# adamgreig/basebandboard

Hardware: AMD Instinct MI355X
Metric: awgn_clt_gsamples_per_s (higher is better)
Workload: dtype u32 bit-sliced GF(2) / int8 out

## Files before the change

### basebandboard_amd/_lib.py

```python
import ctypes as C
import pathlib

import torch

_HERE = pathlib.Path(__file__).resolve().parent
LIB_PATH = _HERE / "libbbb_hip.so"

SHARD_TRIALS, SHARD_SEEDS, SHARD_BITS, SHARD_GROUPS = 0, 1, 2, 3
BBB_OK, BBB_EINVAL, BBB_ENOMEM, BBB_EHIP, BBB_EIO, BBB_ENODEV, BBB_EUNSUP = 0, -1, -2, -3, -4, -5, -6

SYMBOLS = [
    "bbb_abi_version", "bbb_strerror", "bbb_last_error_detail", "bbb_device_count", "bbb_free",
    "bbb_lutopt_load_matrix_file", "bbb_lutopt_create", "bbb_lutopt_destroy", "bbb_lutopt_set_stream",
    "bbb_lutopt_is_specialised", "bbb_lutopt_set_staged", "bbb_lutopt_set_custom_fill", "bbb_lutopt_set_custom_ber", "bbb_lutopt_attach_custom_library", "bbb_lutopt_profile", "bbb_lutopt_profile_read", "bbb_lutopt_profile_read_mover", "bbb_lutopt_state_at", "bbb_lutopt_fill_words", "bbb_awgn_fill_i8", "bbb_awgn_fill_i16", "bbb_awgn_prefetch", "bbb_awgn_stream_open", "bbb_awgn_stream_next", "bbb_awgn_stream_read", "bbb_awgn_stream_seek", "bbb_awgn_stream_tell", "bbb_awgn_stream_close", "bbb_awgn_hist",
    "bbb_clt_tree_i16", "bbb_prbs_fill", "bbb_prbs_fill_hint", "bbb_prbs_check", "bbb_prbs_check_dev", "bbb_prbs_state_at",
    "bbb_prbs_detector_run", "bbb_prbs_detector_stream", "bbb_ber_trials", "bbb_ber_trials_dev", "bbb_ber_run_open", "bbb_ber_run_next", "bbb_ber_run_next_dev", "bbb_ber_run_tell", "bbb_ber_run_close", "bbb_ber_sweep_multi", "bbb_sweep_shard", "bbb_multi_last_info", "bbb_multi_release", "bbb_shaper_fill_i16", "bbb_tx_fill_i16", "bbb_tx_stream_open", "bbb_tx_stream_next", "bbb_tx_stream_read", "bbb_tx_stream_seek", "bbb_tx_stream_tell", "bbb_tx_stream_close", "bbb_rx_slice", "bbb_rx_phase_search", "bbb_eye_accumulate_i16", "bbb_tx_eye_open", "bbb_tx_eye_run", "bbb_tx_eye_close", "bbb_tx_ber_sweep_open", "bbb_tx_ber_sweep_run", "bbb_tx_ber_sweep_close", "bbb_acf_accumulate_i16", "bbb_tx_acf_open", "bbb_tx_acf_run", "bbb_tx_acf_close", "bbb_nco_rom", "bbb_nco_open", "bbb_nco_set_cfg", "bbb_nco_set_stream", "bbb_nco_run", "bbb_nco_get_state", "bbb_nco_set_state", "bbb_nco_close", "bbb_sinc_coefficients", "bbb_sinc_interpolate", "bbb_sinc_eye_open", "bbb_sinc_eye_run", "bbb_sinc_eye_close", "bbb_fir_moving_average", "bbb_fir_filter", "bbb_fir_slice", "bbb_link_sweep_open", "bbb_link_sweep_run", "bbb_link_sweep_close", "bbb_gf2_berlekamp_massey", "bbb_gf2_recur",
    "bbb_gf2_dot", "bbb_gf2_poly_is_primitive", "bbb_gf2_poly_modexp", "bbb_lutopt_charpoly", "bbb_lutopt_is_full_period",
    "bbb_lutopt_save_matrix_file", "bbb_lutopt_search_candidate", "bbb_lutopt_search",
    "bbb_errstat_open", "bbb_errstat_accumulate", "bbb_errstat_skip", "bbb_errstat_read", "bbb_errstat_reset",
    "bbb_errstat_set_stream", "bbb_errstat_geometry", "bbb_errstat_close",
    "bbb_xcorr_accumulate_i16", "bbb_tx_xcorr_open", "bbb_tx_xcorr_run", "bbb_tx_xcorr_close",
    "bbb_ddc_run", "bbb_ddc_polar_host",
    "bbb_dfe_run", "bbb_dfe_geometry", "bbb_dfe_model_host",
]


class BbbError(RuntimeError):
    def __init__(self, code, what, detail):
        super().__init__(f"{what}: {detail}" if detail else what)
        self.code = code


class TrialCfg(C.Structure):
    _fields_ = [("prbs_k", C.c_int32), ("amp", C.c_int32), ("noise_var", C.c_int32), ("reserved", C.c_int32),
                ("prbs_state", C.c_uint64), ("warmup", C.c_uint64), ("first_bit", C.c_uint64),
                ("nbits", C.c_uint64)]


class TxCfg(C.Structure):
    _fields_ = [("coeffs", C.c_int16 * 64), ("source", C.c_int32), ("prbs_k", C.c_int32), ("prbs_state", C.c_uint64),
                ("bit_en", C.c_int32), ("noise_en", C.c_int32), ("noise_var", C.c_int32), ("reserved", C.c_int32),
                ("warmup", C.c_uint64)]


class EyeCfg(C.Structure):
    _fields_ = [("ncols", C.c_uint32), ("shift", C.c_uint32), ("col_origin", C.c_uint64), ("threshold", C.c_int32),
                ("strict", C.c_int32)]


class TxSetting(C.Structure):
    _fields_ = [("coeffs", C.c_int16 * 64), ("bit_en", C.c_int32), ("noise_en", C.c_int32), ("noise_var", C.c_int32),
                ("threshold", C.c_int32), ("strict", C.c_int32), ("reserved", C.c_int32)]


class DetectorStats(C.Structure):
    _fields_ = [(n, C.c_uint64) for n in ("bits", "errors", "errors_raw", "reload_clocks", "resyncs", "chunks",
                                          "chunks_rerun", "serial_fallback")]


class SearchStats(C.Structure):
    _fields_ = [(n, C.c_uint64) for n in ("tested", "full_degree", "order_divides", "primitive", "kernel_ns")]


class MultiInfo(C.Structure):
    _fields_ = [("n_devices", C.c_int32), ("n_ranks_seen", C.c_int32), ("rccl_reused", C.c_int32), ("reserved", C.c_int32),
                ("rccl_path", C.c_char * 256)]


class NcoCfg(C.Structure):
    _fields_ = [("fcw", C.c_uint32), ("am", C.c_uint32), ("fm", C.c_int32), ("pm", C.c_int32)]


class NcoState(C.Structure):
    _fields_ = [("pa", C.c_uint32), ("q", C.c_int32), ("w", C.c_int32), ("y", C.c_int32)]


class SincCfg(C.Structure):
    _fields_ = [("in_bytes", C.c_uint32), ("out_bytes", C.c_uint32), ("shift", C.c_uint32)]


class FirCfg(C.Structure):
    _fields_ = [("ntaps", C.c_uint32), ("taps", C.c_int16 * 256), ("shift", C.c_uint32), ("decim", C.c_uint32),
                ("phase", C.c_uint32), ("out_bytes", C.c_uint32)]


DDC_IQ16, DDC_IQ32, DDC_POLAR = 0, 1, 2


class DfeCfg(C.Structure):
    _fields_ = [("ff", FirCfg), ("nfb", C.c_uint32), ("fb", C.c_int32 * 4), ("threshold", C.c_int32), ("strict", C.c_uint32),
                ("region_symbols", C.c_uint32), ("warmup_symbols", C.c_uint32)]


class DdcCfg(C.Structure):
    _fields_ = [("fcw", C.c_uint32), ("pa0", C.c_uint32), ("mode", C.c_uint32)]


ERRSTAT_NBINS = 312


class ErrstatCfg(C.Structure):
    _fields_ = [("guard", C.c_uint32), ("nblock", C.c_uint32), ("block_bits", C.c_uint64 * 4)]


class ErrstatResult(C.Structure):
    _fields_ = ([(n, C.c_uint64) for n in ("bits", "errors", "first_error", "last_error", "max_gap", "bursts", "burst_len_sum",
                                           "max_burst_len", "max_burst_weight", "open_first", "open_last", "open_weight")]
                + [("errored_blocks", C.c_uint64 * 4)]
                + [(n, C.c_uint64 * ERRSTAT_NBINS) for n in ("gap_hist", "burst_len_hist", "burst_weight_hist")])


class XcorrCfg(C.Structure):
    _fields_ = [("spb", C.c_uint32), ("nlags", C.c_uint32), ("origin", C.c_uint64)]


class Ber(C.Structure):
    _fields_ = [("bits", C.c_uint64), ("errors", C.c_uint64)]


_lib = None


def select_build(name):
    global LIB_PATH
    if _lib is not None:
        raise RuntimeError("the library is already loaded")
    LIB_PATH = _HERE / {"product": "libbbb_hip.so", "experiments": "libbbb_hip_exp.so"}[name]


def lib():
    global _lib
    if _lib is not None:
        return _lib
    if not LIB_PATH.exists():
        raise ImportError(
            f"{LIB_PATH} is missing: build it with `python -c 'import __graft_entry__ as g; g.build()'` "
            "(hipcc --offload-arch=gfx950).  basebandboard_amd has no CPU fallback.")
    l = C.CDLL(str(LIB_PATH))
    vp, u64, i32 = C.c_void_p, C.c_uint64, C.c_int
    u64p = C.POINTER(C.c_uint64)
    l.bbb_abi_version.restype = i32
    l.bbb_strerror.restype = C.c_char_p
    l.bbb_strerror.argtypes = [i32]
    l.bbb_last_error_detail.restype = C.c_char_p
    l.bbb_device_count.argtypes = [C.POINTER(i32)]
    l.bbb_free.argtypes = [vp]
    l.bbb_free.restype = None
    l.bbb_lutopt_load_matrix_file.argtypes = [C.c_char_p, C.POINTER(i32), C.POINTER(C.POINTER(C.c_uint16)),
                                              C.POINTER(C.POINTER(C.c_uint32))]
    l.bbb_lutopt_create.argtypes = [C.POINTER(vp), i32, C.POINTER(C.c_uint16), C.POINTER(C.c_uint32), u64p, i32]
    l.bbb_lutopt_destroy.argtypes = [vp]
    l.bbb_lutopt_set_stream.argtypes = [vp, vp]
    l.bbb_lutopt_is_specialised.argtypes = [vp]
    l.bbb_lutopt_set_staged.argtypes = [vp, i32]
    l.bbb_lutopt_state_at.argtypes = [vp, u64, u64p]
    l.bbb_lutopt_profile.argtypes = [vp, i32]
    l.bbb_lutopt_profile_read.argtypes = [vp, C.POINTER(C.c_double), C.POINTER(C.c_double), u64p, i32]
    l.bbb_lutopt_profile_read_mover.argtypes = [vp, C.POINTER(C.c_double), u64p, i32]
    l.bbb_lutopt_fill_words.argtypes = [vp, vp, u64, u64, i32]
    l.bbb_awgn_fill_i8.argtypes = [vp, vp, u64, u64]
    l.bbb_awgn_fill_i16.argtypes = [vp, vp, u64, u64]
    l.bbb_awgn_prefetch.argtypes = [vp, u64, u64]
    l.bbb_awgn_stream_open.argtypes = [vp, u64, u64, i32, C.POINTER(vp)]
    l.bbb_awgn_stream_next.argtypes = [vp, vp]
    l.bbb_awgn_stream_read.argtypes = [vp, vp, u64]
    l.bbb_awgn_stream_seek.argtypes = [vp, u64]
    l.bbb_awgn_stream_tell.argtypes = [vp, u64p]
    l.bbb_awgn_stream_close.argtypes = [vp]
    l.bbb_awgn_hist.argtypes = [vp, vp, u64, u64]
    l.bbb_clt_tree_i16.argtypes = [i32, vp, u64, vp, i32, vp]
    l.bbb_prbs_fill.argtypes = [i32, u64, u64, u64, vp, i32, vp]
    l.bbb_prbs_fill_hint.argtypes = [i32, u64, u64, u64, vp, C.c_uint, i32, vp]
    l.bbb_prbs_check.argtypes = [i32, u64, u64, u64, vp, u64p, i32, vp]
    l.bbb_prbs_check_dev.argtypes = [i32, u64, u64, u64, vp, vp, i32, vp]
    l.bbb_prbs_state_at.argtypes = [i32, u64, u64, u64p]
    l.bbb_prbs_detector_run.argtypes = [i32, vp, u64, u64, vp, vp, i32, vp]
    l.bbb_rx_phase_search.argtypes = [vp, u64, u64, u64, i32, i32, C.POINTER(DetectorStats), i32, vp]
    l.bbb_prbs_detector_stream.argtypes = [i32, vp, u64, vp, vp, C.POINTER(DetectorStats), u64, u64, i32, vp]
    l.bbb_ber_trials.argtypes = [vp, C.POINTER(TrialCfg), i32, C.POINTER(Ber)]
    l.bbb_ber_trials_dev.argtypes = [vp, C.POINTER(TrialCfg), i32, vp]
    l.bbb_multi_last_info.argtypes = [C.POINTER(MultiInfo)]
    l.bbb_ber_run_open.argtypes = [vp, C.POINTER(TrialCfg), i32, C.c_uint32, C.POINTER(vp)]
    l.bbb_ber_run_next.argtypes = [vp, C.POINTER(Ber)]
    l.bbb_ber_run_next_dev.argtypes = [vp, vp]
    l.bbb_ber_run_tell.argtypes = [vp, u64p, u64p]
    l.bbb_ber_run_close.argtypes = [vp]
    l.bbb_ber_sweep_multi.argtypes = [C.POINTER(vp), i32, C.POINTER(TrialCfg), i32, i32, C.POINTER(Ber)]
    l.bbb_sweep_shard.argtypes = [C.POINTER(TrialCfg), i32, i32, i32, i32, C.POINTER(TrialCfg)]
    l.bbb_multi_release.argtypes = []
    l.bbb_shaper_fill_i16.argtypes = [C.POINTER(TxCfg), vp, u64, u64, i32, vp]
    l.bbb_tx_fill_i16.argtypes = [vp, C.POINTER(TxCfg), vp, u64, u64]
    l.bbb_tx_stream_open.argtypes = [vp, C.POINTER(TxCfg), u64, u64, C.POINTER(vp)]
    l.bbb_tx_stream_next.argtypes = [vp, vp]
    l.bbb_tx_stream_read.argtypes = [vp, vp, u64]
    l.bbb_tx_stream_seek.argtypes = [vp, u64]
    l.bbb_tx_stream_tell.argtypes = [vp, u64p]
    l.bbb_tx_stream_close.argtypes = [vp]
    l.bbb_rx_slice.argtypes = [vp, u64, u64, u64, i32, vp, u64p, i32, vp]
    l.bbb_eye_accumulate_i16.argtypes = [vp, u64, u64, C.POINTER(EyeCfg), vp, i32, vp]
    l.bbb_tx_eye_open.argtypes = [vp, C.POINTER(TxCfg), C.POINTER(EyeCfg), u64, C.POINTER(vp)]
    l.bbb_tx_eye_run.argtypes = [vp, u64, u64, vp, vp]
    l.bbb_tx_eye_close.argtypes = [vp]
    l.bbb_tx_ber_sweep_open.argtypes = [vp, C.POINTER(TxCfg), C.POINTER(TxSetting), i32, u64, C.POINTER(vp)]
    l.bbb_tx_ber_sweep_run.argtypes = [vp, u64, u64, vp]
    l.bbb_tx_ber_sweep_close.argtypes = [vp]
    l.bbb_acf_accumulate_i16.argtypes = [vp, u64, u64, C.c_uint32, vp, i32, vp]
    l.bbb_tx_acf_open.argtypes = [vp, C.POINTER(TxCfg), C.c_uint32, u64, C.POINTER(vp)]
    l.bbb_tx_acf_run.argtypes = [vp, u64, u64, vp]
    l.bbb_tx_acf_close.argtypes = [vp]
    l.bbb_nco_rom.argtypes = [vp]
    l.bbb_nco_open.argtypes = [C.POINTER(NcoCfg), i32, vp, C.POINTER(vp)]
    l.bbb_nco_set_cfg.argtypes = [vp, C.POINTER(NcoCfg)]
    l.bbb_nco_set_stream.argtypes = [vp, vp]
    l.bbb_nco_run.argtypes = [vp, vp, vp, vp, u64, vp]
    l.bbb_nco_get_state.argtypes = [vp, C.POINTER(NcoState)]
    l.bbb_nco_set_state.argtypes = [vp, C.POINTER(NcoState)]
    l.bbb_nco_close.argtypes = [vp]
    l.bbb_sinc_coefficients.argtypes = [vp]
    l.bbb_sinc_interpolate.argtypes = [vp, u64, C.c_uint32, C.POINTER(SincCfg), vp, i32, vp]
    l.bbb_sinc_eye_open.argtypes = [C.POINTER(SincCfg), C.POINTER(EyeCfg), u64, i32, vp, C.POINTER(vp)]
    l.bbb_sinc_eye_run.argtypes = [vp, vp, u64, C.c_uint32, u64, vp]
    l.bbb_sinc_eye_close.argtypes = [vp]
    l.bbb_fir_moving_average.argtypes = [C.POINTER(FirCfg), i32]
    l.bbb_fir_filter.argtypes = [vp, u64, C.c_uint32, C.POINTER(FirCfg), vp, u64p, i32, vp]
    l.bbb_fir_slice.argtypes = [vp, u64, C.c_uint32, C.POINTER(FirCfg), C.c_int32, i32, vp, u64p, i32, vp]
    l.bbb_link_sweep_open.argtypes = [vp, C.POINTER(TxCfg), C.POINTER(TxSetting), i32, C.POINTER(FirCfg), C.c_uint32,
                                      C.POINTER(EyeCfg), u64, C.POINTER(vp)]
    l.bbb_link_sweep_run.argtypes = [vp, u64, u64, vp, vp]
    l.bbb_link_sweep_close.argtypes = [vp]
    l.bbb_errstat_open.argtypes = [C.POINTER(ErrstatCfg), i32, vp, C.POINTER(vp)]
    l.bbb_errstat_accumulate.argtypes = [vp, vp, vp, u64]
    l.bbb_errstat_skip.argtypes = [vp, u64]
    l.bbb_errstat_read.argtypes = [vp, C.POINTER(ErrstatResult)]
    l.bbb_errstat_reset.argtypes = [vp]
    l.bbb_errstat_set_stream.argtypes = [vp, vp]
    l.bbb_errstat_geometry.argtypes = [u64p, u64p]
    l.bbb_errstat_close.argtypes = [vp]
    l.bbb_xcorr_accumulate_i16.argtypes = [vp, u64, u64, vp, u64, u64, C.POINTER(XcorrCfg), vp, i32, vp]
    l.bbb_tx_xcorr_open.argtypes = [vp, C.POINTER(TxCfg), C.c_uint32, u64, C.POINTER(vp)]
    l.bbb_tx_xcorr_run.argtypes = [vp, u64, u64, vp]
    l.bbb_tx_xcorr_close.argtypes = [vp]
    l.bbb_ddc_run.argtypes = [vp, u64, C.c_uint32, u64, C.POINTER(DdcCfg), C.POINTER(FirCfg), vp, u64p, i32, vp]
    l.bbb_ddc_polar_host.argtypes = [C.c_int16, C.c_int16, C.POINTER(C.c_uint16), C.POINTER(C.c_int16)]
    l.bbb_dfe_run.argtypes = [vp, u64, C.c_uint32, C.POINTER(DfeCfg), vp, vp, vp, vp, u64p, i32, vp]
    l.bbb_dfe_geometry.argtypes = [C.c_uint32, u64p, u64p, u64p, u64p, u64p]
    l.bbb_dfe_model_host.argtypes = [vp, u64, C.c_uint32, C.POINTER(DfeCfg), C.POINTER(C.c_uint32), vp, vp, u64p]
    u8p = C.POINTER(C.c_uint8)
    l.bbb_gf2_berlekamp_massey.argtypes = [u8p, u64, u8p, C.POINTER(C.c_int64)]
    l.bbb_gf2_recur.argtypes = [i32, i32, u64p, u8p, i32, u8p]
    l.bbb_lutopt_set_custom_fill.argtypes = [vp, vp]
    l.bbb_lutopt_set_custom_ber.argtypes = [vp, vp]
    l.bbb_lutopt_attach_custom_library.argtypes = [vp, C.c_char_p]
    l.bbb_gf2_dot.argtypes = [i32, i32, u64p, u8p, u8p]
    u16p, u32p = C.POINTER(C.c_uint16), C.POINTER(C.c_uint32)
    l.bbb_gf2_poly_is_primitive.argtypes = [u8p, i32, C.POINTER(C.c_int)]
    l.bbb_gf2_poly_modexp.argtypes = [u8p, i32, u64p, i32, u8p]
    l.bbb_lutopt_charpoly.argtypes = [i32, u16p, u32p, u8p, C.POINTER(C.c_int)]
    l.bbb_lutopt_is_full_period.argtypes = [i32, u16p, u32p, C.POINTER(C.c_int)]
    l.bbb_lutopt_save_matrix_file.argtypes = [C.c_char_p, i32, u16p, u32p]
    l.bbb_lutopt_search_candidate.argtypes = [i32, u64, u64, u16p, u32p]
    l.bbb_lutopt_search.argtypes = [i32, u64, u64, u64, u64p, u16p, u32p, C.POINTER(SearchStats), i32, vp]
    for name in SYMBOLS:
        getattr(l, name)
    _lib = l
    return l


def check(rc, what):
    if rc == BBB_OK:
        return
    l = lib()
    detail = l.bbb_last_error_detail().decode(errors="replace")
    name = l.bbb_strerror(rc).decode()
    if rc == BBB_EINVAL:
        raise ValueError(detail or name)
    raise BbbError(rc, f"{what} failed ({name})", detail)


def cuda_tensor(name, t, dtypes, kind, device):
    if not isinstance(t, torch.Tensor) or t.dtype not in dtypes or not t.is_cuda or t.dim() != 1 or not t.is_contiguous():
        raise ValueError(f"{name} must be a contiguous 1-D {kind} CUDA tensor")
    if t.device != torch.device("cuda", device):
        raise ValueError(f"{name} must be on cuda:{device}")
    return t


class Handle:
    _handle = _close = None

    def close(self):
        p = getattr(self, self._handle, None)
        setattr(self, self._handle, None)
        if p:
            check(getattr(lib(), self._close)(p), self._close)

    def __enter__(self):
        return self

    def __exit__(self, *exc):
        self.close()

    def __del__(self):
        try:
            self.close()
        except Exception:
            pass


class StreamHandle(Handle):
    _set_stream = None

    def _open_stream(self):
        self._stream = torch.cuda.current_stream(self.device).cuda_stream if torch.cuda.is_available() else None
        return C.c_void_p(self._stream)

    def _bind_stream(self):
        s = torch.cuda.current_stream(self.device).cuda_stream
        if s != self._stream:
            check(getattr(lib(), self._set_stream)(getattr(self, self._handle), C.c_void_p(s)), self._set_stream)
            self._stream = s
```

### basebandboard_amd/csrc/bbb_api.hip

```cpp
#include "bbb_common.hpp"
#include "dev_buf.hpp"
#include "capture.hpp"
#include "awgn_launch.hpp"
#include "stage_common.hpp"
#include "gf2.hpp"
#include "rccl_loader.hpp"
#include "sweep_shard.hpp"
#include "sweep_threads.hpp"

#include <algorithm>
#include <cstdlib>
#include <cstring>
#include <map>
#include <memory>
#include <mutex>
#include <thread>
#include <utility>
#include <vector>

namespace bbb {

std::string &last_error() {
    static thread_local std::string s;
    return s;
}

int use_device(int device) {
    static std::mutex mu;
    static bool checked[64] = {false};
    bool known = false;
    if (device >= 0 && device < 64) {
        std::lock_guard<std::mutex> g(mu);
        known = checked[device];
    }
    if (!known) {
        int n = 0;
        if (hipGetDeviceCount(&n) != hipSuccess || n <= 0) return fail(BBB_ENODEV, "no HIP device visible");
        if (device < 0 || device >= n) return fail(BBB_ENODEV, "device index out of range");
        hipDeviceProp_t p;
        BBB_HIP(hipGetDeviceProperties(&p, device));
        if (std::strncmp(p.gcnArchName, "gfx950", 6) != 0)
            return fail(BBB_ENODEV, std::string("device is ") + p.gcnArchName + ", this library is built for gfx950 only");
        if (device < 64) {
            std::lock_guard<std::mutex> g(mu);
            checked[device] = true;
        }
    }
    BBB_HIP(hipSetDevice(device));
    return BBB_OK;
}

namespace {

struct Event {
    hipEvent_t e = nullptr;
    Event() = default;
    Event(Event &&o) noexcept : e(o.e) { o.e = nullptr; }
    Event &operator=(Event &&o) noexcept { std::swap(e, o.e); return *this; }
    ~Event() { if (e) (void)hipEventDestroy(e); }
    operator hipEvent_t() const { return e; }
    int create_timed() { BBB_HIP(hipEventCreate(&e)); return BBB_OK; }
    int record(hipStream_t s) {
        if (!e) BBB_HIP(hipEventCreateWithFlags(&e, hipEventDisableTiming));
        BBB_HIP(hipEventRecord(e, s));
        return BBB_OK;
    }
};

template <size_t N>
struct ReadGuarded {
    DevBuf<uint32_t> buf[N];
    Event last_read;
    bool read_pending = false;
    bool fits(const size_t (&need)[N]) const {
        for (size_t i = 0; i < N; i++)
            if (buf[i].cap < need[i]) return false;
        return true;
    }
    int grow(const size_t (&need)[N]) {
        if (fits(need)) return BBB_OK;
        if (read_pending) BBB_HIP(hipEventSynchronize(last_read));
        read_pending = false;
        for (size_t i = 0; i < N; i++)
            if (const int rc = buf[i].grow(need[i])) return rc;
        return BBB_OK;
    }
    int wait_read(hipStream_t s) const {
        if (read_pending) BBB_HIP(hipStreamWaitEvent(s, last_read, 0));
        return BBB_OK;
    }
    int mark_read(hipStream_t s) {
        if (const int rc = last_read.record(s)) return rc;
        read_pending = true;
        return BBB_OK;
    }
};
enum { kStates = 0, kPlanes = 1 };

struct StageSlot {
    DevBuf<uint32_t> stage;
    Event arith;
    Event free;
    bool busy = false;
    uint64_t gen = 0;
    DevBuf<uint32_t> bits[2];
    unsigned bits_turn = 0;

    int grow_stage(size_t words) {
        if (stage.cap >= words) return BBB_OK;
        if (busy) BBB_HIP(hipEventSynchronize(free));
        busy = false;
        return stage.grow(words);
    }
    int grow_bits(unsigned b, size_t words) {
        if (bits[b].cap >= words) return BBB_OK;
        if (busy) BBB_HIP(hipEventSynchronize(free));
        return bits[b].grow(words);
    }
    int wait_free(hipStream_t s) const { if (busy) BBB_HIP(hipStreamWaitEvent(s, free, 0)); return BBB_OK; }
    int mover_queued(hipStream_t ms) {
        if (const int rc = free.record(ms)) return rc;
        busy = true;
        gen++;
        return BBB_OK;
    }
};

struct SeededStates {
    bool valid = false;
    uint64_t first = 0, L = 0, G = 0;
    ReadGuarded<2> set;
    Event seeded;
    bool matches(uint64_t f, uint64_t l, uint64_t g) const { return valid && first == f && L == l && G == g; }
};

struct ProfEv {
    Event e0, e1, e2;
    int begin(hipStream_t s) {
        for (Event *e : {&e0, &e1, &e2})
            if (const int rc = e->create_timed()) return rc;
        return e0.record(s);
    }
};

}

struct JumpPlan {
    GF2Mat B;
    GF2Mat Bt;
    DevBuf<uint32_t> d_cols;
    DevBuf<uint32_t> d_top;
    uint32_t qcol64[32] = {0};
    int levels = 0;
};

}

using namespace bbb;

struct bbb_lutopt {
    int k = 0, W64 = 0, W32 = 0, device = 0;
    bool specialised = false;
    bbb_custom_fill_fn custom_fill = nullptr;
    bbb_custom_ber_fn custom_ber = nullptr;
    int small_fast = 0;
    bool fast512 = false;
    hipStream_t stream = nullptr;
    std::vector<uint16_t> taps;
    std::vector<uint32_t> row_off;
    uint64_t init[8] = {0};
    std::unique_ptr<GF2Powers> pw;
    std::map<uint64_t, JumpPlan> plans;
    std::map<uint64_t, JumpPlan> prbs_plans;
    ReadGuarded<2> cur;
    ReadGuarded<1> pp[2];
    int pp_idx = 0;
    DevBuf<uint16_t> d_taps;
    DevBuf<uint32_t> d_row_off;
    DevBuf<unsigned long long> d_counters;
    DevBuf<uint32_t> d_txnoise;
    DevBuf<uint32_t> d_txbits;
    ReadGuarded<1> fbits[2];
    Event fbits_ready;
    SeededStates seeds[2];
    int seeds_idx = 0;
    DevBuf<unsigned long long, true> h_counters;
    Event counters_zeroed;
    bool counters_clean = false;
    int fbits_slot = 0;
    bool planes_valid = false;
    uint64_t planes_first = 0, planes_L = 0, planes_G = 0;
    unsigned max_waves = 1024;
    SeededStates pf;
    hipStream_t side = nullptr;
    hipStream_t cs = nullptr;
    bool cs_valid = false;
    Event handover;
    bool staged_mode = false;
    bool has_stream = false;
    hipStream_t xs2[2] = {nullptr, nullptr}, ys = nullptr;
    StageSlot slots[2];
    int stage_slot = 0;
    Event ev_user;
    int pf_waited_slot = -1;
    uint64_t pf_waited_gen = 0;
    struct Ahead {
        bool valid = false; int kind = 0; uint64_t first = 0, step = 0, n = 0, win_lo = 0, L = 0, G = 0;
        unsigned nlanes = 0, left = 0; int slot = 0; bbb_tx_cfg cfg{};
        int64_t bits_m0 = 0; uint64_t bits_words64 = 0;
        unsigned bits_buf = 0;
    } ahead;
    bool last_fill_tx = false;
    bool last_staged_small = false;
    int staged_level = 0;
    bool profiling = false;
    std::vector<std::pair<Event, Event>> prof_mover_pending;
    double prof_mover_ms = 0; uint64_t prof_mover_calls = 0;
    std::vector<ProfEv> prof_pending;
    Event prof_prev_e2;
    double prof_seed_ms = 0, prof_main_ms = 0;
    uint64_t prof_calls = 0;
};

extern "C" {
static int seed_announced(bbb_lutopt *h, uint64_t first_step, uint64_t L, uint64_t G, unsigned nlanes, hipStream_t side, int seed_variant);
}

namespace {

int pad_w32(int k) {
    const int w = (k + 31) / 32;
    for (int c : {1, 2, 4, 6, 8, 12, 16})
        if (w <= c) return c;
    return 16;
}

int upload(const std::vector<uint32_t> &host, DevBuf<uint32_t> *out) {
    DevBuf<uint32_t> d;
    if (const int rc = d.grow(host.size())) return rc;
    BBB_HIP(hipMemcpy(d.p, host.data(), host.size() * sizeof(uint32_t), hipMemcpyHostToDevice));
    *out = std::move(d);
    return BBB_OK;
}

void nibble_table(const GF2Mat &M, uint32_t *out) {
    const int k = M.n, W32 = pad_w32(k), nnib = (k + 3) / 4;
    const int C = (W32 % 4 == 0) ? 4 : (W32 % 2 == 0 ? 2 : 1), NC = W32 / C;
    std::vector<uint32_t> cols((size_t)k * W32, 0u);
    for (int r = 0; r < k; r++) {
        const uint64_t *row = M.row(r);
        for (int w = 0; w < M.W; w++) {
            uint64_t bits = row[w];
            while (bits) {
                const int c = (w << 6) + __builtin_ctzll(bits);
                bits &= bits - 1;
                cols[(size_t)c * W32 + (r >> 5)] |= 1u << (r & 31);
            }
        }
    }
    std::vector<uint32_t> ent(16 * (size_t)W32);
    for (int n = 0; n < nnib; n++) {
        std::fill(ent.begin(), ent.end(), 0u);
        for (int v = 1; v < 16; v++) {
            const int c = 4 * n + __builtin_ctz((unsigned)v);
            for (int z = 0; z < W32; z++)
                ent[(size_t)v * W32 + z] = ent[(size_t)(v & (v - 1)) * W32 + z] ^ (c < k ? cols[(size_t)c * W32 + z] : 0u);
        }
        for (int v = 0; v < 16; v++)
            for (int z = 0; z < W32; z++)
                out[(((size_t)n * NC + z / C) * 16 + v) * C + z % C] = ent[(size_t)v * W32 + z];
    }
}

int build_plan(const GF2Mat &M, int levels, JumpPlan *plan) {
    const int k = M.n, W32 = pad_w32(k), nnib = (k + 3) / 4;
    const size_t nt = (size_t)nnib * 16 * W32;
    std::vector<uint32_t> host((size_t)levels * 15 * nt, 0);
    GF2Mat m1 = M;
    for (int e = 1; e < levels; e++) {
        for (int q = 0; q < 4; q++) m1 = m1.mul(m1);
        GF2Mat mj = m1;
        for (int j = 1; j <= 15; j++) {
            if (j > 1) mj = mj.mul(m1);
            nibble_table(mj, &host[((size_t)e * 15 + (j - 1)) * nt]);
        }
    }
    if (const int rc = upload(host, &plan->d_cols)) return rc;
    plan->levels = levels;
    plan->B = M;
    plan->Bt = M.transpose();
    return BBB_OK;
}

void first16(const JumpPlan &plan, const uint64_t *s0, uint32_t *out) {
    const int W = plan.B.W;
    uint64_t x[8];
    std::memcpy(x, s0, sizeof(uint64_t) * (size_t)W);
    std::memset(out, 0, sizeof(uint32_t) * 256);
    for (int i = 0; i < 16; i++) {
        if (i) plan.Bt.matvec_t(x, x);
        for (int w = 0; w < 2 * W && w < 16; w++) out[i * 16 + w] = (uint32_t)(x[w >> 1] >> (32 * (w & 1)));
    }
}

void first16_at(const bbb_lutopt *h, const JumpPlan &plan, uint64_t step, uint32_t *out) {
    uint64_t s0[8] = {0};
    h->pw->apply(step, h->init, s0);
    first16(plan, s0, out);
}

constexpr int kPlanLevels = 7;

int ensure_top_tables(JumpPlan *plan) {
    if (plan->d_top) return BBB_OK;
    const GF2Mat &M = plan->B;
    const int k = M.n, W32 = pad_w32(k), nnib = (k + 3) / 4;
    const size_t nt = (size_t)nnib * 16 * W32;
    std::vector<uint32_t> host((size_t)kSeedTopTables * nt, 0);
    GF2Mat m4 = M;
    for (int q = 0; q < 16; q++) m4 = m4.mul(m4);
    GF2Mat md = m4;
    for (int d = 1; d <= kSeedTopTables; d++) {
        if (d > 1) md = md.mul(m4);
        nibble_table(md, &host[(size_t)(d - 1) * nt]);
    }
    return upload(host, &plan->d_top);
}

int get_plan(bbb_lutopt *h, uint64_t L, JumpPlan **out) {
    auto it = h->plans.find(L);
    if (it == h->plans.end()) {
        JumpPlan p;
        int rc = build_plan(h->pw->power(L), kPlanLevels, &p);
        if (rc) return rc;
        it = h->plans.emplace(L, std::move(p)).first;
    }
    *out = &it->second;
    return BBB_OK;
}

int get_prbs_plan(bbb_lutopt *h, int k, uint64_t L, JumpPlan **out) {
    const uint64_t key = ((uint64_t)k << 56) ^ L;
    auto it = h->prbs_plans.find(key);
    if (it == h->prbs_plans.end()) {
        JumpPlan p;
        GF2Powers pw(prbs_matrix(k, prbs_tap(k)));
        int rc = build_plan(pw.power(L), kPlanLevels, &p);
        if (rc) return rc;
        {
            GF2Mat q = p.B;
            for (int i = 0; i < 6; i++) q = q.mul(q);
            const GF2Mat qt = q.transpose();
            for (int c = 0; c < k && c < 32; c++) p.qcol64[c] = (uint32_t)qt.row(c)[0];
        }
        it = h->prbs_plans.emplace(key, std::move(p)).first;
    }
    *out = &it->second;
    return BBB_OK;
}

void partition(const bbb_lutopt *h, uint64_t n, unsigned granule, uint64_t *L, uint64_t *G, unsigned *nlanes) {
    const uint64_t gmax = (uint64_t)h->max_waves * 2048;
    uint64_t l = (n + gmax - 1) / gmax;
    if (l < 64) l = 64;
    l = (l + granule - 1) / granule * granule;
    const uint64_t g = (n + l - 1) / l;
    const uint64_t waves = (g + 2047) / 2048;
    *L = l;
    *G = g;
    *nlanes = (unsigned)(waves * 64);
}

struct DevStreams { hipStream_t xs[2] = {nullptr, nullptr}, side = nullptr; };
static std::mutex g_streams_mu;
static std::map<int, DevStreams> g_streams;

int ensure_internal_streams(bbb_lutopt *h) {
    if (!h->xs2[0]) {
        std::lock_guard<std::mutex> g(g_streams_mu);
        DevStreams &d = g_streams[h->device];
        for (hipStream_t *st : {&d.xs[0], &d.xs[1]})
            if (!*st) BBB_HIP(hipStreamCreateWithFlags(st, hipStreamNonBlocking));
        h->xs2[0] = d.xs[0]; h->xs2[1] = d.xs[1];
    }
    return BBB_OK;
}

int ensure_side_stream(bbb_lutopt *h) {
    if (!h->side) {
        std::lock_guard<std::mutex> g(g_streams_mu);
        DevStreams &d = g_streams[h->device];
        if (!d.side) BBB_HIP(hipStreamCreateWithFlags(&d.side, hipStreamNonBlocking));
        h->side = d.side;
    }
    return BBB_OK;
}

int begin_op(bbb_lutopt *h, bool internal, bool independent_of_previous_internal = false) {
    if (internal) {
        const int rc = ensure_internal_streams(h);
        if (rc) return rc;
    }
    hipStream_t want = internal ? h->xs2[h->stage_slot ^ 1] : h->stream;
    if (h->cs_valid && h->cs != want) {
        const bool from_internal = h->cs == h->xs2[0] || h->cs == h->xs2[1];
        if (!(independent_of_previous_internal && internal && from_internal)) {
            const int rc = h->handover.record(h->cs);
            if (rc) return rc;
            BBB_HIP(hipStreamWaitEvent(want, h->handover, 0));
        }
    }
    h->cs = want;
    h->cs_valid = true;
    return BBB_OK;
}

int mark_planes_read(bbb_lutopt *h) { return h->cur.mark_read(h->cs); }

int prepare_planes(bbb_lutopt *h, uint64_t first, uint64_t L, uint64_t G, unsigned nlanes, int slice_mode = 0) {
    if (h->planes_valid && h->planes_first == first && h->planes_L == L && h->planes_G == G) return BBB_OK;
    JumpPlan *plan;
    int rc = get_plan(h, L, &plan);
    if (rc) return rc;
    const bool two_launch = h->k == 256 && (h->specialised || h->custom_fill) && !h->fast512 && G <= ((uint64_t)kSeedTopTables + 1) * 65536 &&
                            !env_knob("BBB_EXP_SEED_CHAIN", 0);
    const size_t states_words = two_launch && (size_t)G * h->W32 < (size_t)65536 * 8 ? (size_t)65536 * 8 : (size_t)G * h->W32;
    if ((rc = h->cur.grow({states_words, (size_t)2 * h->k * nlanes}))) return rc;
    uint32_t s16[256];
    first16_at(h, *plan, first, s16);
    h->planes_valid = false;
    if (two_launch) {
        if ((rc = ensure_top_tables(plan))) return rc;
        if ((rc = awgn_seed_head_launch(h->k, plan->d_cols, s16, G, h->cur.buf[kStates], h->cs))) return rc;
        rc = awgn_seed_tail_planes_launch(h->k, plan->d_top, G, h->cur.buf[kStates], nlanes, h->cur.buf[kPlanes], h->cs);
    } else {
        rc = awgn_seed_launch(h->k, plan->d_cols, s16, G, h->cur.buf[kStates], G, nlanes, h->cur.buf[kPlanes], h->cs, slice_mode);
    }
    if (rc || slice_mode) return rc;
    if ((rc = mark_planes_read(h))) return rc;
    h->planes_valid = true;
    h->planes_first = first; h->planes_L = L; h->planes_G = G;
    return BBB_OK;
}

int acquire_planes(bbb_lutopt *h, uint64_t first_step, uint64_t L, uint64_t G, unsigned nlanes, bool may_use_prefetch,
                   bool *from_prefetch = nullptr, int slice_mode = 0) {
    if (from_prefetch) *from_prefetch = false;
    if (may_use_prefetch && h->pf.matches(first_step, L, G)) {
        if (from_prefetch) *from_prefetch = true;
        BBB_HIP(hipStreamWaitEvent(h->cs, h->pf.seeded, 0));
        std::swap(h->cur, h->pf.set);
        h->pf.valid = false;
        h->planes_valid = slice_mode == 0;
        h->planes_first = first_step; h->planes_L = L; h->planes_G = G;
        return BBB_OK;
    }
    return prepare_planes(h, first_step, L, G, nlanes, slice_mode);
}


template <typename LaunchMover>
int queue_mover_with(bbb_lutopt *h, int slot, LaunchMover launch_mover) {
    hipStream_t ms = h->stream;
    StageSlot &sl = h->slots[slot];
    int rc;
    const bool own_stream = env_knob("BBB_EXP_MOVER_OWN_STREAM", 0) != 0;
    if (own_stream) {
        if (!h->ys) BBB_HIP(hipStreamCreateWithFlags(&h->ys, hipStreamNonBlocking));
        ms = h->ys;
        if ((rc = h->ev_user.record(h->stream))) return rc;
        BBB_HIP(hipStreamWaitEvent(ms, h->ev_user, 0));
    }
    BBB_HIP(hipStreamWaitEvent(ms, sl.arith, 0));
    if ((rc = sl.wait_free(ms))) return rc;
    Event m0, m1;
    if (h->profiling) {
        if ((rc = m0.create_timed()) || (rc = m1.create_timed())) return rc;
        BBB_HIP(hipEventRecord(m0, ms));
    }
    if ((rc = launch_mover((const void *)sl.stage.p, ms))) return rc;
    if (h->profiling) {
        BBB_HIP(hipEventRecord(m1, ms));
        h->prof_mover_pending.emplace_back(std::move(m0), std::move(m1));
    }
    if ((rc = sl.mover_queued(ms))) return rc;
    if (own_stream) BBB_HIP(hipStreamWaitEvent(h->stream, sl.free, 0));
    return BBB_OK;
}

bool tx_cfg_equal(const bbb_tx_cfg &a, const bbb_tx_cfg &b) {
    return std::memcmp(a.coeffs, b.coeffs, sizeof a.coeffs) == 0 && a.source == b.source && a.prbs_k == b.prbs_k &&
           a.prbs_state == b.prbs_state && a.bit_en == b.bit_en && a.noise_en == b.noise_en && a.noise_var == b.noise_var &&
           a.warmup == b.warmup;
}

bbb_lutopt::Ahead take_ahead(bbb_lutopt *h) {
    const bbb_lutopt::Ahead a = h->ahead;
    h->ahead.first += a.n; h->ahead.step += a.n;
    h->ahead.win_lo += a.n;
    h->ahead.valid = --h->ahead.left > 0;
    return a;
}

int take_waiting(bbb_lutopt *h, int kind, uint64_t first, uint64_t n, const bbb_tx_cfg *cfg, bool *waiting, bbb_lutopt::Ahead *a) {
    *waiting = h->ahead.valid && h->ahead.kind == kind && h->ahead.first == first && h->ahead.n == n &&
               (kind != 1 || tx_cfg_equal(h->ahead.cfg, *cfg));
    if (!*waiting) return BBB_OK;
    if (env_knob("BBB_EXP_DELIVER_HANDOVER", 0)) {
        const int rc = begin_op(h, true);
        if (rc) return rc;
    }
    *a = take_ahead(h);
    return BBB_OK;
}

uint64_t ahead_total(const bbb_lutopt *h, uint64_t n, uint64_t cap, uint64_t step, uint64_t first, uint64_t pos_bound) {
    const uint64_t m = (uint64_t)h->staged_level;
    const bool ahead = m >= 2 && (n % 16) == 0 && m * n < cap && step + m * n >= m * n && (!pos_bound || first + m * n < pos_bound);
    return ahead ? m * n : n;
}

int produce_planes(bbb_lutopt *h, uint64_t L, unsigned nlanes, ProfEv *ev, bool planes_seeded_after_mover, int *slot_out,
                   bool small_footprint = false) {
    const int slot = h->stage_slot ^= 1;
    StageSlot &sl = h->slots[slot];
    *slot_out = slot;
    if (h->ahead.valid && h->ahead.slot == slot) h->ahead.valid = false;
    int rc;
    if ((rc = sl.grow_stage(stage_words(nlanes, L)))) return rc;
    const bool seeding_saw_last_mover = planes_seeded_after_mover && h->pf_waited_slot == slot && h->pf_waited_gen == sl.gen;
    if (planes_seeded_after_mover) h->pf_waited_slot = -1;
    if (!seeding_saw_last_mover && (rc = sl.wait_free(h->cs))) return rc;
    if (ev) BBB_HIP(hipEventRecord(ev->e1, h->cs));
    rc = awgn256_planes_launch(h->cur.buf[kPlanes], (void *)sl.stage.p, (unsigned)L, nlanes, h->cs, small_footprint);
    h->last_staged_small = small_footprint;
    if (rc) return rc;
    if ((rc = mark_planes_read(h))) return rc;
    if (ev) BBB_HIP(hipEventRecord(ev->e2, h->cs));
    return sl.arith.record(h->cs);
}

struct StagedRun { uint64_t L = 0, G = 0; unsigned nlanes = 0; int slot = 0; };

template <typename Hook, typename LaunchMover>
int staged_produce(bbb_lutopt *h, uint64_t ntotal, uint64_t seed_step, bool small_form, bool timed, Hook hook, LaunchMover launch_mover,
                   StagedRun *run) {
    StagedRun &r = *run;
    uint64_t &L = r.L, &G = r.G;
    partition(h, ntotal, 16, &L, &G, &r.nlanes);
    if (L > 0xffffff00ull) return fail(BBB_EINVAL, "nsamples too large for one call (segment length must fit 32 bits): split it");
    int rc = begin_op(h, true, h->pf.matches(seed_step, L, G));
    if (rc) return rc;
    h->last_fill_tx = false;
    ProfEv ev;
    const bool prof = timed && h->profiling;
    if (prof && (rc = ev.begin(h->cs))) return rc;
    bool from_pf = false;
    if ((rc = acquire_planes(h, seed_step, L, G, r.nlanes, true, &from_pf))) return rc;
    if ((rc = hook())) return rc;
    rc = produce_planes(h, L, r.nlanes, prof ? &ev : nullptr, from_pf, &r.slot, small_form);
    if (!rc) rc = queue_mover_with(h, r.slot, [&](const void *stage, hipStream_t ms) { return launch_mover(r, stage, ms); });
    if (prof) h->prof_pending.push_back(std::move(ev));
    return rc;
}

void record_ahead(bbb_lutopt *h, int kind, uint64_t first, uint64_t step, uint64_t n, uint64_t left, const StagedRun &run) {
    bbb_lutopt::Ahead &a = h->ahead;
    a.valid = true; a.kind = kind;
    a.first = first; a.step = step; a.n = n; a.win_lo = n; a.left = (unsigned)left;
    a.L = run.L; a.G = run.G; a.nlanes = run.nlanes; a.slot = run.slot;
}

bool partition512(const bbb_lutopt *h, uint64_t nsamples, uint64_t *L, uint64_t *G, unsigned *nlanes) {
    const uint64_t gmax = (uint64_t)h->max_waves * 1024;
    uint64_t l = (nsamples + gmax - 1) / gmax;
    if (l < 64) l = 64;
    l = (l + 7) / 8 * 8;
    if (l > 0xffffff00ull) return false;
    *L = l;
    *G = (nsamples + l - 1) / l;
    *nlanes = (unsigned)((*G + 1023) / 1024 * 64);
    return true;
}

int awgn_fill(bbb_lutopt *h, void *dst, int elem_size, uint64_t nsamples, uint64_t first_step) {
    if (!h) return fail(BBB_EINVAL, "null handle");
    if (nsamples == 0) return BBB_OK;
    if (!dst || ((uintptr_t)dst & 15)) return fail(BBB_EINVAL, "dst must be a 16-byte aligned device pointer");
    if (first_step + nsamples < first_step) return fail(BBB_EINVAL, "first_step + nsamples overflows");
    if (h->k & (h->k - 1)) return fail(BBB_EUNSUP, "CLTGRNG needs k to be a power of two (rng.py:72-76)");
    if (elem_size == 1 && h->k > 256) return fail(BBB_EUNSUP, "k > 256 needs the int16 output");
    if (h->device < 0) return fail(BBB_ENODEV, "host-only handle (device -1) cannot generate samples");
    BBB_HIP(hipSetDevice(h->device));
    uint64_t L, G;
    unsigned nlanes;
    if (h->fast512 && elem_size == 2) {
        if (!partition512(h, nsamples, &L, &G, &nlanes))
            return fail(BBB_EINVAL, "nsamples too large for one call (segment length must fit 32 bits): split it");
        int rc5 = begin_op(h, false);
        if (rc5) return rc5;
        h->planes_valid = false;
        if ((rc5 = acquire_planes(h, first_step, L, G, nlanes, true, nullptr, 1))) return rc5;
        if ((rc5 = awgn512p_fill_launch(h->cur.buf[kPlanes], (int16_t *)dst, nsamples, (unsigned)L, G, nlanes, h->cs))) return rc5;
        return mark_planes_read(h);
    }
    partition(h, nsamples, 16, &L, &G, &nlanes);
    if (L > 0xffffff00ull) return fail(BBB_EINVAL, "nsamples too large for one call (segment length must fit 32 bits): split it");
    const bool fast256 = h->specialised && elem_size == 1;
    h->last_fill_tx = false;
    const bool staged = fast256 && h->staged_mode && nsamples >= (1ull << 24);
    if (staged) {
        bool waiting;
        bbb_lutopt::Ahead a;
        int rc = take_waiting(h, 0, first_step, nsamples, nullptr, &waiting, &a);
        if (rc) return rc;
        auto launch_i8 = [&](const void *stage, uint64_t win_lo, uint64_t Lk, uint64_t Gk, unsigned nl, hipStream_t ms) {
            return unplane_launch(stage, dst, win_lo, nsamples, (unsigned)Lk, Gk, nl, ms);
        };
        if (waiting)
            return queue_mover_with(h, a.slot, [&](const void *stage, hipStream_t ms) { return launch_i8(stage, a.win_lo, a.L, a.G, a.nlanes, ms); });
        const uint64_t ntotal = ahead_total(h, nsamples, 1ull << 40, first_step, first_step, 0);
        const bool small_form = h->staged_level == 1 || env_knob("BBB_EXP_NOISE_SMALL", 0);
        StagedRun run;
        rc = staged_produce(h, ntotal, first_step + (small_form ? 1 : 0), small_form, true, [] { return BBB_OK; },
                            [&](const StagedRun &r, const void *stage, hipStream_t ms) { return launch_i8(stage, 0, r.L, r.G, r.nlanes, ms); }, &run);
        if (!rc && ntotal != nsamples) record_ahead(h, 0, first_step + nsamples, first_step + nsamples, nsamples, ntotal / nsamples - 1, run);
        return rc;
    }
    int rc = begin_op(h, false);
    if (rc) return rc;
    ProfEv ev;
    if (h->profiling && (rc = ev.begin(h->cs))) return rc;
    rc = acquire_planes(h, first_step, L, G, nlanes, fast256);
    if (rc) return rc;
    if (fast256) {
        if (h->profiling) BBB_HIP(hipEventRecord(ev.e1, h->cs));
        rc = awgn256_fill_launch(h->cur.buf[kPlanes], (int8_t *)dst, nsamples, (unsigned)L, G, nlanes, h->cs);
        if (!rc) rc = mark_planes_read(h);
        if (h->profiling) {
            BBB_HIP(hipEventRecord(ev.e2, h->cs));
            h->prof_pending.push_back(std::move(ev));
        }
        return rc;
    }
    if (h->custom_fill && elem_size == 1) {
        const int e = h->custom_fill(h->cur.buf[kPlanes], (int8_t *)dst, nsamples, (uint32_t)L, G, nlanes, (void *)h->cs);
        if (e) return fail(BBB_EHIP, std::string("custom sample kernel: ") + hipGetErrorString((hipError_t)e));
        return mark_planes_read(h);
    }
    if (h->small_fast && elem_size == 1) {
        rc = awgn_small_fill_launch(h->small_fast, h->cur.buf[kPlanes], (int8_t *)dst, nsamples, (unsigned)L, G, nlanes, h->cs);
        return rc ? rc : mark_planes_read(h);
    }
    h->planes_valid = false;
    rc = awgn_generic_fill_launch(h->k, h->d_taps, h->d_row_off, h->cur.buf[kPlanes], dst, elem_size, nsamples, (unsigned)L, G,
                                  nlanes, h->cs);
    return rc ? rc : mark_planes_read(h);
}

int wrap12(int v) {
    unsigned u = (unsigned)v & 0xfffu;
    return (u & 0x800u) ? (int)u - 4096 : (int)u;
}
int channel_thresholds(int amp, int noise_var, TrialDev *t) {
    for (int bv = 0; bv < 2; bv++) {
        int n = 0, prev = 0;
        for (int T = 0; T < 256; T++) {
            const int g = T - 128;
            const int noise = wrap12(g * noise_var);
            const int x = wrap12((bv ? amp : -amp) + noise);
            const int decided = x >= 0;
            const int err = decided != bv;
            if (err != prev) {
                if (n == 4) return fail(BBB_EUNSUP, "channel needs more than 4 decision thresholds");
                t->thr[bv][n++] = T;
                prev = err;
            }
        }
        t->nthr[bv] = n;
    }
    return BBB_OK;
}

int trial_dev(const bbb_trial_cfg &c, TrialDev *t) {
    const int tap = prbs_tap(c.prbs_k);
    if (!tap) return fail(BBB_EINVAL, "k=" + std::to_string(c.prbs_k) + " invalid for PRBS");
    if (c.prbs_state == 0 || (c.prbs_state >> c.prbs_k)) return fail(BBB_EINVAL, "PRBS state must be in [1, 2^k)");
    if (c.amp < 0 || c.amp > 2047 || c.noise_var < 0 || c.noise_var > 15) return fail(BBB_EINVAL, "amp must be 0..2047 and noise_var 0..15");
    t->prbs_k = c.prbs_k;
    t->prbs_tap = tap;
    return channel_thresholds(c.amp, c.noise_var, t);
}

bool single_threshold(const TrialDev &t) {
    for (int bv = 0; bv < 2; bv++) {
        int real = 0;
        for (int j = 0; j < t.nthr[bv]; j++) real += t.thr[bv][j] > 0 && t.thr[bv][j] < 256;
        if (real != 1) return false;
    }
    return true;
}

int ber_run(bbb_lutopt *h, const bbb_trial_cfg *cfgs, int ncfg, unsigned long long *counters_dev) {
    {
        const int rc0 = begin_op(h, false);
        if (rc0) return rc0;
    }
    if (!h->specialised && !h->custom_ber)
        return fail(BBB_EUNSUP, "BER trials need the shipped n256 matrix, or a k = 256 matrix with its own kernels attached "
                                "(bbb_lutopt_attach_custom_library / LUTOPT.specialise)");
    std::vector<TrialDev> td((size_t)ncfg);
    for (int i = 0; i < ncfg; i++) {
        const bbb_trial_cfg &c = cfgs[i];
        if (c.warmup + c.first_bit < c.warmup || c.warmup + c.first_bit + c.nbits < c.nbits)
            return fail(BBB_EINVAL, "warmup + first_bit + nbits overflows");
        const int rc = trial_dev(c, &td[(size_t)i]);
        if (rc) return rc;
    }
    for (int i = 0; i < ncfg;) {
        const bbb_trial_cfg &c = cfgs[i];
        int n = 1;
        while (single_threshold(td[(size_t)i]) && i + n < ncfg && n < BBB_BER_MAX_GROUP) {
            const bbb_trial_cfg &d = cfgs[i + n];
            if (d.prbs_k != c.prbs_k || d.prbs_state != c.prbs_state || d.warmup != c.warmup ||
                d.first_bit != c.first_bit || d.nbits != c.nbits || !single_threshold(td[(size_t)(i + n)]))
                break;
            n++;
        }
        if (c.nbits == 0) { i += n; continue; }
        uint64_t L, G;
        unsigned nlanes;
        partition(h, c.nbits, 2, &L, &G, &nlanes);
        if (L >= (1ull << 27)) return fail(BBB_EINVAL, "nbits too large for one trial (about 2^47): split it with first_bit");
        for (int j = 0; j < n; j++) { td[(size_t)(i + j)].L = (uint32_t)L; td[(size_t)(i + j)].G = G; td[(size_t)(i + j)].nbits = c.nbits; }
        int rc;
        if ((rc = ensure_internal_streams(h))) return rc;
        const uint64_t gen_first = c.warmup + c.first_bit + 1;
        JumpPlan *pp, *plan = nullptr;
        if ((rc = get_prbs_plan(h, c.prbs_k, L, &pp))) return rc;
        const int pb = h->pp_idx ^= 1;
        for (int b : {pb, pb ^ 1})
            if ((rc = h->pp[b].grow({(size_t)32 * nlanes}))) return rc;
        uint32_t ps16[256], s16[256];
        {
            uint64_t ps0 = 0;
            if ((rc = prbs_state_at_host(c.prbs_k, c.prbs_state, c.first_bit, &ps0))) return rc;
            uint64_t ps64[8] = {ps0};
            first16(*pp, ps64, ps16);
        }
        int sb = -1;
        for (int b : {0, 1})
            if (h->seeds[b].matches(gen_first, L, G)) sb = b;
        const bool seed_gen = sb < 0;
        if (seed_gen) {
            sb = h->seeds_idx ^= 1;
            const size_t need[2] = {(size_t)65536 * h->W32, (size_t)h->k * nlanes};
            for (int b : {sb, sb ^ 1}) {
                if (!h->seeds[b].set.fits(need)) h->seeds[b].valid = false;
                if ((rc = h->seeds[b].set.grow(need))) return rc;
            }
            if ((rc = get_plan(h, L, &plan))) return rc;
            if ((rc = ensure_top_tables(plan))) return rc;
            first16_at(h, *plan, gen_first, s16);
        }
        const bool busy = seed_gen && hipStreamQuery(h->cs) == hipErrorNotReady;
        hipStream_t ss = busy ? h->xs2[0] : h->cs;
        ReadGuarded<1> &prbs = h->pp[pb];
        if ((rc = prbs.wait_read(seed_gen ? ss : h->cs))) return rc;
        SeededStates &gs = h->seeds[sb];
        if (seed_gen) {
            gs.valid = false;
            if ((rc = gs.set.wait_read(ss))) return rc;
            const PrbsSeedRide ride{c.prbs_k, pp->d_cols, ps16, pp->qcol64, nlanes, prbs.buf[0]};
            if ((rc = awgn_seed_head_launch(h->k, plan->d_cols, s16, G, gs.set.buf[kStates], ss, &ride))) return rc;
            if ((rc = awgn_seed_tail_planes_launch(h->k, plan->d_top, G, gs.set.buf[kStates], nlanes, gs.set.buf[kPlanes], ss))) return rc;
            if ((rc = gs.seeded.record(ss))) return rc;
            if (busy) BBB_HIP(hipStreamWaitEvent(h->cs, gs.seeded, 0));
            gs.valid = true;
            gs.first = gen_first; gs.L = L; gs.G = G;
        } else {
            BBB_HIP(hipStreamWaitEvent(h->cs, gs.seeded, 0));
            if ((rc = prbs_seed_lanes_launch(c.prbs_k, pp->d_cols, ps16, pp->qcol64, G, nlanes, prbs.buf[0], h->cs))) return rc;
        }
        if (h->specialised) {
            if ((rc = ber256_launch(gs.set.buf[kPlanes], prbs.buf[0], &td[(size_t)i], n, nlanes, counters_dev + 2 * (size_t)i, h->cs))) return rc;
        } else {
            const int e = h->custom_ber(gs.set.buf[kPlanes], prbs.buf[0], &td[(size_t)i], n, nlanes, (uint64_t *)(counters_dev + 2 * (size_t)i), (void *)h->cs);
            if (e) return fail(e < 0 ? e : BBB_EHIP, "custom BER kernel failed");
        }
        if ((rc = prbs.mark_read(h->cs))) return rc;
        if ((rc = gs.set.mark_read(h->cs))) return rc;
        i += n;
    }
    return BBB_OK;
}

}

extern "C" {

int bbb_abi_version(void) { return BBB_ABI_VERSION; }

const char *bbb_strerror(int code) {
    switch (code) {
    case BBB_OK: return "ok";
    case BBB_EINVAL: return "invalid argument";
    case BBB_ENOMEM: return "out of memory";
    case BBB_EHIP: return "HIP runtime error";
    case BBB_EIO: return "matrix file unreadable or malformed";
    case BBB_ENODEV: return "no gfx950 device";
    case BBB_EUNSUP: return "unsupported request";
    default: return "unknown error";
    }
}

const char *bbb_last_error_detail(void) { return last_error().c_str(); }

int bbb_device_count(int *count) {
    if (!count) return fail(BBB_EINVAL, "null count");
    int n = 0;
    if (hipGetDeviceCount(&n) != hipSuccess) n = 0;
    *count = n;
    return BBB_OK;
}

void bbb_free(void *p) { std::free(p); }

int bbb_lutopt_load_matrix_file(const char *path, int *k, uint16_t **taps, uint32_t **row_off) {
    if (!path || !k || !taps || !row_off) return fail(BBB_EINVAL, "null argument");
    FILE *f = std::fopen(path, "r");
    if (!f) return fail(BBB_EIO, std::string("cannot open ") + path);
    std::vector<std::string> rows;
    char line[BBB_MAX_K + 16];
    while (std::fgets(line, sizeof line, f)) {
        std::string s(line);
        while (!s.empty() && (s.back() == '\n' || s.back() == '\r' || s.back() == ' ')) s.pop_back();
        if (!s.empty()) rows.push_back(s);
    }
    std::fclose(f);
    const int n = (int)rows.size();
    if (n == 0 || n > BBB_MAX_K) return fail(BBB_EIO, "matrix must have 1..512 rows");
    std::vector<uint16_t> t;
    std::vector<uint32_t> off(1, 0);
    for (int r = 0; r < n; r++) {
        if ((int)rows[r].size() != n) return fail(BBB_EIO, "matrix is not square");
        for (int c = 0; c < n; c++) {
            if (rows[r][c] == '1') t.push_back((uint16_t)c);
            else if (rows[r][c] != '0') return fail(BBB_EIO, "matrix holds a character other than 0/1");
        }
        off.push_back((uint32_t)t.size());
    }
    *taps = (uint16_t *)std::malloc(sizeof(uint16_t) * (t.empty() ? 1 : t.size()));
    *row_off = (uint32_t *)std::malloc(sizeof(uint32_t) * off.size());
    if (!*taps || !*row_off) return fail(BBB_ENOMEM, "malloc");
    std::memcpy(*taps, t.data(), sizeof(uint16_t) * t.size());
    std::memcpy(*row_off, off.data(), sizeof(uint32_t) * off.size());
    *k = n;
    return BBB_OK;
}

int bbb_lutopt_create(bbb_lutopt **out, int k, const uint16_t *taps, const uint32_t *row_off,
                      const uint64_t *init_words, int device) {
    if (!out || !taps || !row_off || !init_words) return fail(BBB_EINVAL, "null argument");
    if (k < 2 || k > BBB_MAX_K) return fail(BBB_EINVAL, "k must be in [2, 512]");
    GF2Mat A(k);
    for (int r = 0; r < k; r++) {
        const uint32_t n = row_off[r + 1] - row_off[r];
        if (row_off[r + 1] < row_off[r] || n < 1 || n > 8) return fail(BBB_EINVAL, "every row needs 1..8 taps");
        for (uint32_t j = row_off[r]; j < row_off[r + 1]; j++) {
            if (taps[j] >= k) return fail(BBB_EINVAL, "tap index out of range");
            if (A.get(r, taps[j])) return fail(BBB_EINVAL, "duplicate tap in a row");
            A.set(r, taps[j]);
        }
    }
    if (device != -1) {
        int rc = use_device(device);
        if (rc) return rc;
    }
    std::unique_ptr<bbb_lutopt> h(new bbb_lutopt);
    h->k = k;
    h->W64 = (k + 63) / 64;
    h->W32 = pad_w32(k);
    h->device = device;
    h->taps.assign(taps, taps + row_off[k]);
    h->row_off.assign(row_off, row_off + k + 1);
    for (int w = 0; w < h->W64; w++) {
        uint64_t v = init_words[w];
        if (w == h->W64 - 1 && (k & 63)) v &= (1ull << (k & 63)) - 1ull;
        h->init[w] = v;
    }
    h->pw.reset(new GF2Powers(A));
    h->specialised = awgn256_matches(k, taps, row_off);
    h->small_fast = awgn_small_matches(k, taps, row_off);
    h->fast512 = awgn512p_matches(k, taps, row_off);
    if (device == -1) {
        *out = h.release();
        return BBB_OK;
    }
    hipDeviceProp_t p;
    BBB_HIP(hipGetDeviceProperties(&p, device));
    h->max_waves = (unsigned)p.multiProcessorCount * 4;
    int rc = h->d_taps.grow(h->taps.size());
    if (rc || (rc = h->d_row_off.grow(h->row_off.size()))) return rc;
    BBB_HIP(hipMemcpy(h->d_taps.p, h->taps.data(), sizeof(uint16_t) * h->taps.size(), hipMemcpyHostToDevice));
    BBB_HIP(hipMemcpy(h->d_row_off.p, h->row_off.data(), sizeof(uint32_t) * h->row_off.size(), hipMemcpyHostToDevice));
    *out = h.release();
    return BBB_OK;
}

int bbb_lutopt_destroy(bbb_lutopt *h) {
    if (!h) return BBB_OK;
    if (h->device < 0) { delete h; return BBB_OK; }
    (void)hipSetDevice(h->device);
    (void)hipDeviceSynchronize();
    if (h->ys) (void)hipStreamDestroy(h->ys);
    for (int s : {1, 0}) h->slots[s].stage = {};
    for (int i : {kPlanes, kStates}) h->pf.set.buf[i] = {};
    for (int i : {kPlanes, kStates})
        for (int b : {1, 0}) h->seeds[b].set.buf[i] = {};
    delete h;
    return BBB_OK;
}

int bbb_lutopt_set_stream(bbb_lutopt *h, void *hip_stream) {
    if (!h) return fail(BBB_EINVAL, "null handle");
    h->stream = (hipStream_t)hip_stream;
    return BBB_OK;
}

int bbb_lutopt_set_custom_fill(bbb_lutopt *h, bbb_custom_fill_fn fn) {
    if (!h) return fail(BBB_EINVAL, "null handle");
    if (fn && (h->k > 256 || (h->k & (h->k - 1)))) return fail(BBB_EUNSUP, "custom kernels exist for power-of-two k <= 256");
    h->custom_fill = fn;
    h->planes_valid = false;
    return BBB_OK;
}

int bbb_lutopt_set_custom_ber(bbb_lutopt *h, bbb_custom_ber_fn fn) {
    if (!h) return fail(BBB_EINVAL, "null handle");
    if (fn && h->k != 256) return fail(BBB_EUNSUP, "the fused BER kernels exist for k = 256");
    h->custom_ber = fn;
    return BBB_OK;
}

int bbb_lutopt_attach_custom_library(bbb_lutopt *h, const char *path) {
    if (!h || !path) return fail(BBB_EINVAL, "null argument");
    void *lib = dlopen(path, RTLD_NOW | RTLD_LOCAL);
    if (!lib) return fail(BBB_EIO, std::string("cannot load ") + path + ": " + dlerror());
    auto bail = [&](int code, const std::string &what) { dlclose(lib); return fail(code, what); };
    auto order = reinterpret_cast<int (*)(void)>(dlsym(lib, "bbb_custom_order"));
    auto abi = reinterpret_cast<int (*)(void)>(dlsym(lib, "bbb_custom_abi"));
    auto fill = reinterpret_cast<bbb_custom_fill_fn>(dlsym(lib, "bbb_custom_fill"));
    if (!order || !fill) return bail(BBB_EIO, std::string(path) + " does not export bbb_custom_order / bbb_custom_fill");
    if (!abi || abi() != BBB_CUSTOM_ABI)
        return bail(BBB_EINVAL, std::string(path) + " was built for another version of this library (custom ABI " +
                                    (abi ? std::to_string(abi()) : std::string("none")) + ", expected " + std::to_string(BBB_CUSTOM_ABI) + "): rebuild it");
    if (order() != h->k) return bail(BBB_EINVAL, std::string(path) + " was built for another order");
    int rc = bbb_lutopt_set_custom_fill(h, fill);
    if (rc) { dlclose(lib); return rc; }
    auto ber = reinterpret_cast<bbb_custom_ber_fn>(dlsym(lib, "bbb_custom_ber"));
    if (ber && h->k == 256) rc = bbb_lutopt_set_custom_ber(h, ber);
    return rc;
}

int bbb_lutopt_set_staged(bbb_lutopt *h, int enable) {
    if (!h) return fail(BBB_EINVAL, "null handle");
    if (enable < 0 || enable > 8) return fail(BBB_EINVAL, "0 = off, 1 = staged, 2..8 = staged with that many fills per sample kernel");
    h->staged_mode = enable != 0;
    h->staged_level = enable;
    h->ahead.valid = false;
    return BBB_OK;
}

int bbb_lutopt_is_specialised(const bbb_lutopt *h) { return h && h->specialised ? 1 : 0; }

int bbb_lutopt_profile(bbb_lutopt *h, int enable) {
    if (!h) return fail(BBB_EINVAL, "null handle");
    h->profiling = enable != 0;
    return BBB_OK;
}

int bbb_lutopt_profile_read(bbb_lutopt *h, double *seed_ms, double *kernel_ms, uint64_t *calls, int reset) {
    if (!h) return fail(BBB_EINVAL, "null handle");
    std::vector<ProfEv> pending;
    pending.swap(h->prof_pending);
    for (ProfEv &ev : pending) {
        BBB_HIP(hipEventSynchronize(ev.e2));
        float a = 0, b = 0;
        BBB_HIP(hipEventElapsedTime(&a, ev.e0, ev.e1));
        BBB_HIP(hipEventElapsedTime(&b, ev.e1, ev.e2));
        if (h->prof_prev_e2) {
            float c = 0;
            BBB_HIP(hipEventElapsedTime(&c, h->prof_prev_e2, ev.e2));
            if (c > 0 && c < b) b = c;
        }
        h->prof_prev_e2 = std::move(ev.e2);
        h->prof_seed_ms += a; h->prof_main_ms += b; h->prof_calls++;
    }
    if (seed_ms) *seed_ms = h->prof_seed_ms;
    if (kernel_ms) *kernel_ms = h->prof_main_ms;
    if (calls) *calls = h->prof_calls;
    if (reset) { h->prof_seed_ms = h->prof_main_ms = 0; h->prof_calls = 0; }
    return BBB_OK;
}

int bbb_lutopt_profile_read_mover(bbb_lutopt *h, double *mover_ms, uint64_t *calls, int reset) {
    if (!h) return fail(BBB_EINVAL, "null handle");
    std::vector<std::pair<Event, Event>> pending;
    pending.swap(h->prof_mover_pending);
    for (const auto &ev : pending) {
        BBB_HIP(hipEventSynchronize(ev.second));
        float a = 0;
        BBB_HIP(hipEventElapsedTime(&a, ev.first, ev.second));
        h->prof_mover_ms += a; h->prof_mover_calls++;
    }
    if (mover_ms) *mover_ms = h->prof_mover_ms;
    if (calls) *calls = h->prof_mover_calls;
    if (reset) { h->prof_mover_ms = 0; h->prof_mover_calls = 0; }
    return BBB_OK;
}

int bbb_lutopt_state_at(bbb_lutopt *h, uint64_t nsteps, uint64_t *state_words) {
    if (!h || !state_words) return fail(BBB_EINVAL, "null argument");
    h->pw->apply(nsteps, h->init, state_words);
    return BBB_OK;
}

static int seed_announced(bbb_lutopt *h, uint64_t first_step, uint64_t L, uint64_t G, unsigned nlanes, hipStream_t side, int seed_variant) {
    JumpPlan *plan;
    int rc = get_plan(h, L, &plan);
    if (rc) return rc;
    SeededStates &pf = h->pf;
    pf.valid = false;
    if (pf.seeded) BBB_HIP(hipStreamWaitEvent(side, pf.seeded, 0));
    if ((rc = pf.set.wait_read(side))) return rc;
    if ((rc = pf.set.grow({(size_t)G * h->W32, (size_t)2 * h->k * nlanes}))) return rc;
    pf.set.read_pending = false;
    uint32_t s16[256];
    first16_at(h, *plan, first_step, s16);
    if ((rc = awgn_seed_launch(h->k, plan->d_cols, s16, G, pf.set.buf[kStates], G, nlanes, pf.set.buf[kPlanes], side, h->fast512 ? 1 : 0, seed_variant))) return rc;
    if ((rc = pf.seeded.record(side))) return rc;
    pf.valid = true;
    pf.first = first_step; pf.L = L; pf.G = G;
    return BBB_OK;
}

static int awgn_prefetch(bbb_lutopt *h, uint64_t nsamples, uint64_t first_step, bool for_tx);

int bbb_awgn_prefetch(bbb_lutopt *h, uint64_t nsamples, uint64_t first_step) {
    return awgn_prefetch(h, nsamples, first_step, h && (h->staged_level == 1 || h->last_staged_small || env_knob("BBB_EXP_NOISE_SMALL", 0)));
}

static int awgn_prefetch(bbb_lutopt *h, uint64_t nsamples, uint64_t first_step, bool for_tx) {
    if (!h) return fail(BBB_EINVAL, "null handle");
    if (h->device < 0) return fail(BBB_ENODEV, "host-only handle (device -1)");
    if ((!h->specialised && !h->fast512) || nsamples == 0) return BBB_OK;
    BBB_HIP(hipSetDevice(h->device));
    uint64_t L, G;
    unsigned nlanes;
    const bool staged_size = nsamples >= (1ull << 24);
    if (h->staged_level >= 2 && nsamples >= (1ull << 24) && (nsamples % 16) == 0) {
        const uint64_t m = (uint64_t)h->staged_level;
        if (h->ahead.valid && h->ahead.step == first_step && h->ahead.n == nsamples) {
            const uint64_t skip = (uint64_t)h->ahead.left * nsamples;
            if (first_step + skip < first_step) return BBB_OK;
            first_step += skip;
        }
        if (m * nsamples < (1ull << 40) && first_step + m * nsamples > first_step) nsamples *= m;
    }
    if (for_tx && h->staged_mode && h->specialised && staged_size) {
        if (first_step + 1 == 0) return BBB_OK;
        first_step += 1;
    }
    if (h->fast512) {
        if (!partition512(h, nsamples, &L, &G, &nlanes)) return BBB_OK;
    } else {
        partition(h, nsamples, 16, &L, &G, &nlanes);
    }
    if (L > 0xffffff00ull) return BBB_OK;
    if (h->pf.matches(first_step, L, G)) return BBB_OK;
    hipStream_t side = nullptr;
    int rc;
    if (h->staged_mode && h->specialised) {
        if ((rc = ensure_internal_streams(h))) return rc;
        side = h->xs2[h->stage_slot ^ 1];
    } else {
        if ((rc = ensure_side_stream(h))) return rc;
        side = h->side;
    }
    h->pf_waited_slot = -1;
    h->pf.valid = false;
    const StageSlot &next = h->slots[h->stage_slot ^ 1];
    if (h->staged_mode && next.busy && !h->last_staged_small) {
        if ((rc = next.wait_free(side))) return rc;
        h->pf_waited_slot = h->stage_slot ^ 1;
        h->pf_waited_gen = next.gen;
    }
    return seed_announced(h, first_step, L, G, nlanes, side, h->last_fill_tx ? 4 : 2);
}

int bbb_awgn_fill_i8(bbb_lutopt *h, int8_t *dst_dev, uint64_t nsamples, uint64_t first_step) {
    return awgn_fill(h, dst_dev, 1, nsamples, first_step);
}

int bbb_awgn_fill_i16(bbb_lutopt *h, int16_t *dst_dev, uint64_t nsamples, uint64_t first_step) {
    if (h && h->specialised && h->device >= 0 && nsamples && dst_dev && !((uintptr_t)dst_dev & 15) && (nsamples % 16) == 0) {
        BBB_HIP(hipSetDevice(h->device));
        int rc = h->d_txnoise.grow((size_t)(nsamples + 15) / 4 + 4);
        if (rc) return rc;
        if ((rc = awgn_fill(h, h->d_txnoise, 1, nsamples, first_step))) return rc;
        return widen_i8_i16_launch((const int8_t *)h->d_txnoise.p, dst_dev, nsamples, h->stream);
    }
    return awgn_fill(h, dst_dev, 2, nsamples, first_step);
}


struct SeqStream {
    bbb_lutopt *h = nullptr;
    uint64_t n = 0, pos = 0;
    int saved_level = 0;
    virtual ~SeqStream() = default;
    virtual int fill(void *dst_dev, uint64_t nsamples) = 0;
    virtual int hint() = 0;
    static int overflows(const char *what) { return fail(BBB_EINVAL, std::string(what) + " + nsamples_per_call overflows"); }

    int open(bbb_lutopt *handle, uint64_t nsamples_per_call, uint64_t first, const char *what, bool level2) {
        if (handle->has_stream) return fail(BBB_EINVAL, "the handle already has an open stream");
        if (first + nsamples_per_call < first) return overflows(what);
        h = handle; n = nsamples_per_call; pos = first;
        saved_level = h->staged_level;
        int rc;
        if (h->staged_level == 0 && level2 && (rc = bbb_lutopt_set_staged(h, 2))) return rc;
        if ((rc = hint())) return rc;
        h->has_stream = true;
        return BBB_OK;
    }
    int read(void *dst_dev, uint64_t nsamples) {
        if (pos + nsamples < pos) return fail(BBB_EINVAL, "the stream position overflows");
        const int rc = fill(dst_dev, nsamples);
        if (rc) return rc;
        pos += nsamples;
        return hint();
    }
    int seek(uint64_t first, const char *what) {
        if (first + n < first) return overflows(what);
        pos = first;
        h->ahead.valid = false;
        return hint();
    }
};

static int seq_read(SeqStream *s, void *dst_dev, uint64_t nsamples) { return s && s->h ? s->read(dst_dev, nsamples) : fail(BBB_EINVAL, "null stream"); }
static int seq_next(SeqStream *s, void *dst_dev) { return s ? seq_read(s, dst_dev, s->n) : fail(BBB_EINVAL, "null stream"); }
static int seq_seek(SeqStream *s, uint64_t first, const char *what) { return s && s->h ? s->seek(first, what) : fail(BBB_EINVAL, "null stream"); }
static int seq_tell(const SeqStream *s, uint64_t *next) {
    if (!s || !next) return fail(BBB_EINVAL, "null argument");
    *next = s->pos;
    return BBB_OK;
}
static int seq_close(SeqStream *s) {
    if (!s) return BBB_OK;
    int rc = BBB_OK;
    if (s->h) {
        s->h->has_stream = false;
        if (s->h->staged_level != s->saved_level) rc = bbb_lutopt_set_staged(s->h, s->saved_level);
    }
    delete s;
    return rc;
}

struct bbb_awgn_stream : SeqStream {
    int elem = 1;
    int fill(void *dst_dev, uint64_t nsamples) override {
        return elem == 1 ? bbb_awgn_fill_i8(h, (int8_t *)dst_dev, nsamples, pos) : bbb_awgn_fill_i16(h, (int16_t *)dst_dev, nsamples, pos);
    }
    int hint() override { return pos + n >= pos ? bbb_awgn_prefetch(h, n, pos) : BBB_OK; }
};

int bbb_awgn_stream_open(bbb_lutopt *h, uint64_t nsamples_per_call, uint64_t first_step, int elem_bytes, bbb_awgn_stream **out) {
    if (!h || !out) return fail(BBB_EINVAL, "null argument");
    if (nsamples_per_call == 0) return fail(BBB_EINVAL, "nsamples_per_call must be positive");
    if (elem_bytes != 1 && elem_bytes != 2) return fail(BBB_EINVAL, "elem_bytes must be 1 (int8) or 2 (int16)");
    if (h->device < 0) return fail(BBB_ENODEV, "host-only handle (device -1) cannot generate samples");
    if (h->k & (h->k - 1)) return fail(BBB_EUNSUP, "CLTGRNG needs k to be a power of two (rng.py:72-76)");
    if (elem_bytes == 1 && h->k > 256) return fail(BBB_EUNSUP, "k > 256 needs the int16 output");
    std::unique_ptr<bbb_awgn_stream> s(new bbb_awgn_stream);
    s->elem = elem_bytes;
    const int rc = s->open(h, nsamples_per_call, first_step, "first_step", true);
    if (!rc) *out = s.release();
    return rc;
}

int bbb_awgn_stream_read(bbb_awgn_stream *s, void *dst_dev, uint64_t nsamples) { return seq_read(s, dst_dev, nsamples); }
int bbb_awgn_stream_next(bbb_awgn_stream *s, void *dst_dev) { return seq_next(s, dst_dev); }
int bbb_awgn_stream_seek(bbb_awgn_stream *s, uint64_t first_step) { return seq_seek(s, first_step, "first_step"); }
int bbb_awgn_stream_tell(const bbb_awgn_stream *s, uint64_t *next_step) { return seq_tell(s, next_step); }
int bbb_awgn_stream_close(bbb_awgn_stream *s) { return seq_close(s); }

int bbb_lutopt_fill_words(bbb_lutopt *h, uint32_t *dst_dev, uint64_t nstates, uint64_t first_step, int msb_first) {
    if (!h) return fail(BBB_EINVAL, "null handle");
    if (h->k % 32) return fail(BBB_EUNSUP, "the word stream is defined for k a multiple of 32 (util/verify.py:41,50)");
    if (nstates == 0) return BBB_OK;
    if (!dst_dev || ((uintptr_t)dst_dev & 3)) return fail(BBB_EINVAL, "dst must be a 4-byte aligned device pointer");
    if (first_step + nstates < first_step) return fail(BBB_EINVAL, "first_step + nstates overflows");
    if (nstates > (1ull << 48)) return fail(BBB_EINVAL, "nstates must be <= 2^48 per call");
    if (h->device < 0) return fail(BBB_ENODEV, "host-only handle (device -1) cannot generate words");
    BBB_HIP(hipSetDevice(h->device));
    uint64_t L, G;
    unsigned nlanes;
    const bool fast = h->specialised && !((uintptr_t)dst_dev & 7);
    partition(h, nstates, fast ? 2 : 1, &L, &G, &nlanes);
    int rc = begin_op(h, false);
    if (rc) return rc;
    rc = prepare_planes(h, first_step, L, G, nlanes);
    if (rc) return rc;
    if (fast) {
        rc = lutopt_words256_launch(h->cur.buf[kPlanes], dst_dev, nstates, (unsigned)L, G, nlanes, msb_first != 0, h->cs);
        return rc ? rc : mark_planes_read(h);
    }
    h->planes_valid = false;
    rc = lutopt_words_launch(h->k, h->d_taps, h->d_row_off, h->cur.buf[kPlanes], dst_dev, nstates, (unsigned)L, G, nlanes,
                             msb_first != 0, h->cs);
    if (!rc) rc = mark_planes_read(h);
    return rc;
}

int bbb_clt_tree_i16(int k, const uint64_t *states_dev, uint64_t nstates, int16_t *out_dev, int device,
                     void *hip_stream) {
    if (k < 2 || k > BBB_MAX_K || (k & (k - 1)) || (k & 63)) return fail(BBB_EINVAL, "k must be 64, 128, 256 or 512");
    if (nstates && (!states_dev || !out_dev)) return fail(BBB_EINVAL, "null device pointer");
    int rc = use_device(device);
    if (rc) return rc;
    return clt_tree_launch(k, states_dev, nstates, out_dev, (hipStream_t)hip_stream);
}

int bbb_prbs_fill(int k, uint64_t init_state, uint64_t first_bit, uint64_t nbits, uint64_t *dst_packed_dev,
                  int device, void *hip_stream) {
    if (nbits && !dst_packed_dev) return fail(BBB_EINVAL, "null device pointer");
    if (!prbs_tap(k)) return fail(BBB_EINVAL, "k=" + std::to_string(k) + " invalid for PRBS");
    int rc = use_device(device);
    if (rc) return rc;
    return prbs_fill_launch(k, init_state, first_bit, nbits, dst_packed_dev, (hipStream_t)hip_stream);
}

int bbb_prbs_fill_hint(int k, uint64_t init_state, uint64_t first_bit, uint64_t nbits, uint64_t *dst_packed_dev,
                       unsigned flags, int device, void *hip_stream) {
    if (flags & ~(unsigned)BBB_PRBS_WILL_READ_BACK) return fail(BBB_EINVAL, "unknown flag");
    if (nbits && !dst_packed_dev) return fail(BBB_EINVAL, "null device pointer");
    if (!prbs_tap(k)) return fail(BBB_EINVAL, "k=" + std::to_string(k) + " invalid for PRBS");
    int rc = use_device(device);
    if (rc) return rc;
    return prbs_fill_launch(k, init_state, first_bit, nbits, dst_packed_dev, (hipStream_t)hip_stream, (flags & BBB_PRBS_WILL_READ_BACK) ? 1 : 0);
}

int bbb_prbs_check_dev(int k, uint64_t init_state, uint64_t first_bit, uint64_t nbits,
                       const uint64_t *src_packed_dev, uint64_t *nerr_dev, int device, void *hip_stream) {
    if ((nbits && !src_packed_dev) || !nerr_dev) return fail(BBB_EINVAL, "null device pointer");
    if (!prbs_tap(k)) return fail(BBB_EINVAL, "k=" + std::to_string(k) + " invalid for PRBS");
    int rc = use_device(device);
    if (rc) return rc;
    return prbs_check_launch(k, init_state, first_bit, nbits, src_packed_dev, nerr_dev, (hipStream_t)hip_stream);
}

int bbb_prbs_check(int k, uint64_t init_state, uint64_t first_bit, uint64_t nbits, const uint64_t *src_packed_dev,
                   uint64_t *nerr, int device, void *hip_stream) {
    if (!nerr) return fail(BBB_EINVAL, "null nerr");
    if (!prbs_tap(k)) return fail(BBB_EINVAL, "k=" + std::to_string(k) + " invalid for PRBS");
    int rc = use_device(device);
    if (rc) return rc;
    hipStream_t st = (hipStream_t)hip_stream;
    {
        CallScratch<uint64_t> d;
        if ((rc = d.alloc(1, st))) return rc;
        BBB_HIP(hipMemsetAsync(d, 0, sizeof(uint64_t), st));
        if ((rc = bbb_prbs_check_dev(k, init_state, first_bit, nbits, src_packed_dev, d, device, hip_stream))) return rc;
        BBB_HIP(hipMemcpyAsync(nerr, d, sizeof(uint64_t), hipMemcpyDeviceToHost, st));
    }
    BBB_HIP(hipStreamSynchronize(st));
    return BBB_OK;
}

int bbb_prbs_state_at(int k, uint64_t init_state, uint64_t nbits, uint64_t *state) {
    if (!state) return fail(BBB_EINVAL, "null state");
    if (init_state >> (k > 0 && k < 64 ? k : 63)) return fail(BBB_EINVAL, "PRBS state must be < 2^k");
    return prbs_state_at_host(k, init_state, nbits, state);
}

int bbb_prbs_detector_run(int k, const uint8_t *bits_dev, uint64_t nstreams, uint64_t n, uint8_t *err_dev,
                          uint8_t *reload_dev, int device, void *hip_stream) {
    if (!prbs_tap(k)) return fail(BBB_EINVAL, "k=" + std::to_string(k) + " invalid for PRBS");
    if (nstreams && n && !bits_dev) return fail(BBB_EINVAL, "null device pointer");
    int rc = use_device(device);
    if (rc) return rc;
    return prbs_detector_launch(k, bits_dev, nstreams, n, err_dev, reload_dev, (hipStream_t)hip_stream);
}

int bbb_prbs_detector_stream(int k, const uint64_t *bits_packed_dev, uint64_t nbits, uint64_t *err_packed_dev,
                             uint64_t *reload_packed_dev, bbb_detector_stats *stats, uint64_t chunk_bits, uint64_t warm_bits,
                             int device, void *hip_stream) {
    if (!prbs_tap(k)) return fail(BBB_EINVAL, "k=" + std::to_string(k) + " invalid for PRBS");
    if (nbits && !bits_packed_dev) return fail(BBB_EINVAL, "null device pointer");
    int rc = use_device(device);
    if (rc) return rc;
    return prbs_detector_stream_launch(k, bits_packed_dev, nbits, err_packed_dev, reload_packed_dev, stats, chunk_bits,
                                       warm_bits, (hipStream_t)hip_stream);
}

static void tx_bit_range(uint64_t first, uint64_t n, int64_t *m0, uint64_t *nbits) {
    const int64_t lo = ((int64_t)first - 17 >= 0 ? ((int64_t)first - 17) / 8 : -1) - 7;
    const int64_t hi = (int64_t)(first + n - 1) - 17 >= 0 ? ((int64_t)(first + n - 1) - 17) / 8 : -1;
    *m0 = lo < 0 ? 0 : lo;
    *nbits = hi >= *m0 ? (uint64_t)(hi - *m0 + 1) : 0;
}

static int tx_check(const bbb_tx_cfg *cfg) {
    if (!cfg) return fail(BBB_EINVAL, "null cfg");
    if (cfg->source != 0 && cfg->source != 1) return fail(BBB_EINVAL, "source must be 0 (PRBS) or 1 (pulse)");
    if (cfg->source == 0) {
        if (!prbs_tap(cfg->prbs_k)) return fail(BBB_EINVAL, "k=" + std::to_string(cfg->prbs_k) + " invalid for PRBS");
        if (cfg->prbs_state == 0 || (cfg->prbs_state >> cfg->prbs_k)) return fail(BBB_EINVAL, "PRBS state must be in [1, 2^k)");
    }
    if (cfg->noise_var < 0 || cfg->noise_var > 15) return fail(BBB_EINVAL, "noise_var must be 0..15");
    for (int i = 0; i < 64; i++)
        if (cfg->coeffs[i] <= -256 || cfg->coeffs[i] > 255) return fail(BBB_EINVAL, "coefficients must be in (-256, 255]");
    return BBB_OK;
}

int bbb_shaper_fill_i16(const bbb_tx_cfg *cfg, int16_t *out_dev, uint64_t nsamples, uint64_t first_sample, int device,
                        void *hip_stream) {
    int rc = tx_check(cfg);
    if (rc) return rc;
    if (nsamples == 0) return BBB_OK;
    if (!out_dev || ((uintptr_t)out_dev & 15)) return fail(BBB_EINVAL, "out must be a 16-byte aligned device pointer");
    if ((rc = use_device(device))) return rc;
    hipStream_t st = (hipStream_t)hip_stream;
    int64_t m0;
    uint64_t nbits;
    tx_bit_range(first_sample, nsamples, &m0, &nbits);
    CallScratch<uint64_t> d_bits;
    if (cfg->source == 0 && nbits) {
        if ((rc = d_bits.alloc((nbits + 63) / 64 + 2, st))) return rc;
        if ((rc = prbs_fill_launch(cfg->prbs_k, cfg->prbs_state, (uint64_t)m0, nbits, d_bits, st))) return rc;
    }
    return tx_waveform_launch(cfg->coeffs, d_bits, m0, d_bits ? nbits : 0, cfg->source, nullptr, 0, 1, 0, first_sample, nsamples, out_dev, st);
}

int bbb_tx_fill_i16(bbb_lutopt *h, const bbb_tx_cfg *cfg, int16_t *out_dev, uint64_t nsamples, uint64_t first_sample) {
    if (!h) return fail(BBB_EINVAL, "null handle");
    int rc = tx_check(cfg);
    if (rc) return rc;
    if (nsamples == 0) return BBB_OK;
    if (!out_dev || ((uintptr_t)out_dev & 15)) return fail(BBB_EINVAL, "out must be a 16-byte aligned device pointer");
    if (h->device < 0) return fail(BBB_ENODEV, "host-only handle (device -1) cannot generate samples");
    if (cfg->noise_en && (!h->specialised && h->k > 256)) return fail(BBB_EUNSUP, "TX noise needs an 8-bit CLT generator (k <= 256)");
    BBB_HIP(hipSetDevice(h->device));
    int64_t m0;
    uint64_t nbits;
    if (cfg->noise_en && h->specialised && first_sample + nsamples < (1ull << 62) && nsamples < (1ull << 31)) {
        if (cfg->warmup + first_sample + nsamples < nsamples) return fail(BBB_EINVAL, "warmup + first_sample + nsamples overflows");
        uint64_t L, G;
        unsigned nlanes;
        const bool staged = h->staged_mode && nsamples >= (1ull << 24);
        tx_bit_range(first_sample, nsamples, &m0, &nbits);
        const int64_t F = (int64_t)first_sample - 17, FM = F >> 3;
        const bool use_bits = cfg->bit_en && nbits;
        const uint32_t rel_base = (uint32_t)(FM - 7 - (m0 - 128));
        if (staged) {
            if ((rc = ensure_internal_streams(h))) return rc;
            uint64_t words64 = 0;
            uint32_t *d_bits = nullptr;
            unsigned bits_buf = 0;
            uint32_t rel = rel_base;
            bool bits_on = use_bits;
            auto make_bits = [&](int slot, uint64_t nbits_all) -> int {
                words64 = 2 + (nbits_all + 63) / 64 + 3;
                StageSlot &sl = h->slots[slot];
                bits_buf = sl.bits_turn ^= 1u;
                if (const int rcg = sl.grow_bits(bits_buf, (size_t)words64 * 2)) return rcg;
                d_bits = sl.bits[bits_buf];
                if (!cfg->bit_en || !nbits_all) return BBB_OK;
                BBB_HIP(hipMemsetAsync(d_bits, 0, 16, h->cs));
                uint64_t *bits64 = (uint64_t *)d_bits + 2;
                return cfg->source == 0 ? prbs_fill_launch(cfg->prbs_k, cfg->prbs_state, (uint64_t)m0, nbits_all, bits64, h->cs)
                                        : pulse_bits_launch(bits64, m0, (nbits_all + 63) / 64, h->cs);
            };
            auto launch_tx = [&](const void *stage, uint64_t win_lo, uint64_t Lk, uint64_t Gk, unsigned nl, hipStream_t ys) {
                return unplane_tx_launch(stage, out_dev, win_lo, nsamples, (unsigned)Lk, Gk, nl, cfg->coeffs, d_bits, (uint32_t)(words64 * 2),
                                         rel, (uint32_t)(F & 7), cfg->noise_var, cfg->bit_en, bits_on ? 1 : 0, ys);
            };
            bool waiting;
            bbb_lutopt::Ahead a;
            if ((rc = take_waiting(h, 1, first_sample, nsamples, cfg, &waiting, &a))) return rc;
            if (waiting) {
                d_bits = h->slots[a.slot].bits[a.bits_buf]; words64 = a.bits_words64;
                rel = (uint32_t)(FM - 7 - (a.bits_m0 - 128));
                bits_on = cfg->bit_en != 0;
                return queue_mover_with(h, a.slot, [&](const void *stage, hipStream_t ys) {
                    return launch_tx(stage, a.win_lo, a.L, a.G, a.nlanes, ys);
                });
            }
            const uint64_t step0 = cfg->warmup + first_sample;
            const uint64_t ntotal = ahead_total(h, nsamples, 1ull << 34, step0, first_sample, 1ull << 62);
            int64_t m0_all;
            uint64_t nbits_all;
            tx_bit_range(first_sample, ntotal, &m0_all, &nbits_all);
            bits_on = cfg->bit_en && nbits_all;
            StagedRun run;
            rc = staged_produce(h, ntotal, step0 + 1, true, false,
                                [&] { return make_bits(h->stage_slot ^ 1, nbits_all); },
                                [&](const StagedRun &r, const void *stage, hipStream_t ys) { return launch_tx(stage, 0, r.L, r.G, r.nlanes, ys); },
                                &run);
            if (rc) return rc;
            if (ntotal != nsamples) {
                record_ahead(h, 1, first_sample + nsamples, step0 + nsamples, nsamples, ntotal / nsamples - 1, run);
                h->ahead.cfg = *cfg;
                h->ahead.bits_m0 = m0; h->ahead.bits_words64 = words64; h->ahead.bits_buf = bits_buf;
            }
            return BBB_OK;
        }
        partition(h, nsamples, 16, &L, &G, &nlanes);
        if ((rc = begin_op(h, false))) return rc;
        h->last_fill_tx = true;
        const uint64_t words64 = 2 + (nbits + 63) / 64 + (L / 8 + 63) / 64 + 2;
        const int bs = h->fbits_slot ^= 1;
        { const int rcs_ = ensure_side_stream(h); if (rcs_) return rcs_; }
        ReadGuarded<1> &fb = h->fbits[bs];
        if ((rc = fb.grow({(size_t)words64 * 2}))) return rc;
        uint32_t *const d_bits = fb.buf[0];
        if (use_bits) {
            if ((rc = fb.wait_read(h->side))) return rc;
            BBB_HIP(hipMemsetAsync(d_bits, 0, 16, h->side));
            uint64_t *bits64 = (uint64_t *)d_bits + 2;
            if (cfg->source == 0) rc = prbs_fill_launch(cfg->prbs_k, cfg->prbs_state, (uint64_t)m0, nbits, bits64, h->side);
            else rc = pulse_bits_launch(bits64, m0, (nbits + 63) / 64, h->side);
            if (rc || (rc = h->fbits_ready.record(h->side))) return rc;
            BBB_HIP(hipStreamWaitEvent(h->cs, h->fbits_ready, 0));
        }
        if ((rc = acquire_planes(h, cfg->warmup + first_sample, L, G, nlanes, true))) return rc;
        rc = awgn256_tx_launch(h->cur.buf[kPlanes], out_dev, nsamples, (unsigned)L, G, nlanes, cfg->coeffs, d_bits, (uint32_t)(words64 * 2), rel_base,
                               (uint32_t)(F & 7), cfg->noise_var, cfg->bit_en, use_bits ? 1 : 0, h->cs);
        if (!rc) rc = mark_planes_read(h);
        return rc ? rc : fb.mark_read(h->cs);
    }
    if ((rc = begin_op(h, false))) return rc;
    tx_bit_range(first_sample, nsamples, &m0, &nbits);
    const bool have_bits = cfg->source == 0 && nbits && cfg->bit_en;
    if (have_bits) {
        if ((rc = h->d_txbits.grow((size_t)((nbits + 63) / 64 + 2) * 2))) return rc;
        if ((rc = prbs_fill_launch(cfg->prbs_k, cfg->prbs_state, (uint64_t)m0, nbits, (uint64_t *)h->d_txbits.p, h->stream))) return rc;
    }
    if (cfg->noise_en) {
        if ((rc = h->d_txnoise.grow((size_t)(nsamples + 15) / 4 + 4))) return rc;
        if ((rc = awgn_fill(h, h->d_txnoise, 1, nsamples, cfg->warmup + first_sample))) return rc;
    }
    return tx_waveform_launch(cfg->coeffs, have_bits ? (const uint64_t *)h->d_txbits.p : nullptr, m0, have_bits ? nbits : 0,
                              cfg->bit_en ? cfg->source : 1, (const int8_t *)h->d_txnoise.p, cfg->noise_var, cfg->bit_en,
                              cfg->noise_en, first_sample, nsamples, out_dev, h->stream);
}


struct bbb_tx_stream : SeqStream {
    bbb_tx_cfg cfg{};
    int fill(void *dst_dev, uint64_t nsamples) override { return bbb_tx_fill_i16(h, &cfg, (int16_t *)dst_dev, nsamples, pos); }
    int hint() override {
        if (!cfg.noise_en) return BBB_OK;
        const uint64_t step = cfg.warmup + pos;
        if (step < pos || step + n < step) return BBB_OK;
        return awgn_prefetch(h, n, step, true);
    }
};

int bbb_tx_stream_open(bbb_lutopt *h, const bbb_tx_cfg *cfg, uint64_t nsamples_per_call, uint64_t first_sample, bbb_tx_stream **out) {
    if (!h || !out) return fail(BBB_EINVAL, "null argument");
    int rc = tx_check(cfg);
    if (rc) return rc;
    if (nsamples_per_call == 0) return fail(BBB_EINVAL, "nsamples_per_call must be positive");
    if (h->device < 0) return fail(BBB_ENODEV, "host-only handle (device -1) cannot generate samples");
    std::unique_ptr<bbb_tx_stream> s(new bbb_tx_stream);
    s->cfg = *cfg;
    rc = s->open(h, nsamples_per_call, first_sample, "first_sample", cfg->noise_en != 0);
    if (!rc) *out = s.release();
    return rc;
}

int bbb_tx_stream_read(bbb_tx_stream *s, int16_t *out_dev, uint64_t nsamples) { return seq_read(s, out_dev, nsamples); }
int bbb_tx_stream_next(bbb_tx_stream *s, int16_t *out_dev) { return seq_next(s, out_dev); }
int bbb_tx_stream_seek(bbb_tx_stream *s, uint64_t first_sample) { return seq_seek(s, first_sample, "first_sample"); }
int bbb_tx_stream_tell(const bbb_tx_stream *s, uint64_t *next_sample) { return seq_tell(s, next_sample); }
int bbb_tx_stream_close(bbb_tx_stream *s) { return seq_close(s); }

int bbb_rx_slice(const int16_t *samples_dev, uint64_t nsamples, uint64_t stride, uint64_t phase, int strict,
                 uint64_t *bits_packed_dev, uint64_t *nbits_out, int device, void *hip_stream) {
    if (stride == 0) return fail(BBB_EINVAL, "stride must be >= 1");
    const uint64_t nbits = phase < nsamples ? (nsamples - phase + stride - 1) / stride : 0;
    if (nbits_out) *nbits_out = nbits;
    if (nbits == 0) return BBB_OK;
    if (!samples_dev || !bits_packed_dev) return fail(BBB_EINVAL, "null device pointer");
    int rc = use_device(device);
    if (rc) return rc;
    return rx_slice_launch(samples_dev, nbits, stride, phase, strict, bits_packed_dev, (hipStream_t)hip_stream);
}

int bbb_rx_phase_search(const int16_t *samples_dev, uint64_t nsamples, uint64_t stride, uint64_t nphases, int strict, int k,
                        bbb_detector_stats *stats_out, int device, void *hip_stream) {
    if (stride == 0) return fail(BBB_EINVAL, "stride must be >= 1");
    if (!prbs_tap(k)) return fail(BBB_EINVAL, "k=" + std::to_string(k) + " invalid for PRBS");
    if (nphases == 0) return BBB_OK;
    if (!stats_out || (nsamples && !samples_dev)) return fail(BBB_EINVAL, "null argument");
    int rc = use_device(device);
    if (rc) return rc;
    hipStream_t st = (hipStream_t)hip_stream;
    const uint64_t maxbits = nsamples ? (nsamples + stride - 1) / stride : 0;
    uint64_t *bits = nullptr;
    if (maxbits) BBB_HIP(hipMalloc(&bits, ((maxbits + 63) / 64) * sizeof(uint64_t)));
    for (uint64_t p = 0; p < nphases && rc == BBB_OK; p++) {
        const uint64_t nbits = p < nsamples ? (nsamples - p + stride - 1) / stride : 0;
        stats_out[p] = bbb_detector_stats{};
        if (nbits == 0) continue;
        rc = rx_slice_launch(samples_dev, nbits, stride, p, strict, bits, st);
        if (rc == BBB_OK) rc = prbs_detector_stream_launch(k, bits, nbits, nullptr, nullptr, &stats_out[p], 0, 0, st);
    }
    if (bits) (void)hipFree(bits);
    return rc;
}

int bbb_lutopt_search(int k, uint64_t seed, uint64_t first_candidate, uint64_t ncandidates, uint64_t *found_index,
                      uint16_t *taps_out, uint32_t *row_off_out, bbb_search_stats *stats, int device, void *hip_stream) {
    if (!found_index) return fail(BBB_EINVAL, "null argument");
    int rc = use_device(device);
    if (rc) return rc;
    return lutopt_search_launch(k, seed, first_candidate, ncandidates, found_index, taps_out, row_off_out, stats,
                                (hipStream_t)hip_stream);
}

int bbb_ber_trials_dev(bbb_lutopt *h, const bbb_trial_cfg *cfgs, int ncfg, uint64_t *counters_dev) {
    if (!h || (ncfg && (!cfgs || !counters_dev)) || ncfg < 0) return fail(BBB_EINVAL, "null argument");
    if (h->device < 0) return fail(BBB_ENODEV, "host-only handle (device -1) cannot run trials");
    BBB_HIP(hipSetDevice(h->device));
    return ber_run(h, cfgs, ncfg, (unsigned long long *)counters_dev);
}

static int ensure_counters(bbb_lutopt *h, size_t need) {
    const size_t cap = need < 64 ? 64 : need;
    if (h->d_counters.cap < cap) h->counters_clean = false;
    int rc = h->d_counters.grow(cap);
    return rc ? rc : h->h_counters.grow(cap);
}

static int take_clean_counters(bbb_lutopt *h, size_t need) {
    if (h->counters_clean && h->counters_zeroed) {
        BBB_HIP(hipStreamWaitEvent(h->stream, h->counters_zeroed, 0));
    } else {
        BBB_HIP(hipMemsetAsync(h->d_counters, 0, need * sizeof(unsigned long long), h->stream));
    }
    h->counters_clean = false;
    return BBB_OK;
}

static int read_back_counters(bbb_lutopt *h, size_t need) {
    BBB_HIP(hipMemcpyAsync(h->h_counters, h->d_counters, need * sizeof(unsigned long long), hipMemcpyDeviceToHost, h->stream));
    BBB_HIP(hipMemsetAsync(h->d_counters, 0, h->d_counters.cap * sizeof(unsigned long long), h->stream));
    if (const int rc = h->counters_zeroed.record(h->stream)) return rc;
    h->counters_clean = true;
    return BBB_OK;
}

int bbb_ber_trials(bbb_lutopt *h, const bbb_trial_cfg *cfgs, int ncfg, bbb_ber *out) {
    if (!h || (ncfg && (!cfgs || !out)) || ncfg < 0) return fail(BBB_EINVAL, "null argument");
    if (ncfg == 0) return BBB_OK;
    if (h->device < 0) return fail(BBB_ENODEV, "host-only handle (device -1) cannot run trials");
    BBB_HIP(hipSetDevice(h->device));
    const size_t need = 2 * (size_t)ncfg;
    int rc = ensure_counters(h, need);
    if (rc) return rc;
    if ((rc = take_clean_counters(h, need))) return rc;
    rc = ber_run(h, cfgs, ncfg, h->d_counters);
    if (rc) return rc;
    if ((rc = read_back_counters(h, need))) return rc;
    BBB_HIP(hipStreamSynchronize(h->stream));
    for (int i = 0; i < ncfg; i++) {
        out[i].bits = h->h_counters[2 * (size_t)i];
        out[i].errors = h->h_counters[2 * (size_t)i + 1];
    }
    return BBB_OK;
}


struct bbb_ber_run {
    bbb_lutopt *h = nullptr;
    std::vector<bbb_trial_cfg> cfgs;
    std::vector<TrialDev> td;
    uint32_t m = 1, call = 0;
    uint64_t n = 0, block = 0, Lb = 0, G = 0;
    unsigned nlanes = 0;
    DevBuf<uint32_t> d_states, d_planes, d_pplanes;
    DevBuf<unsigned long long> d_totals;
    Event fork, join;
};

int bbb_ber_run_open(bbb_lutopt *h, const bbb_trial_cfg *cfgs, int ncfg, uint32_t calls_per_block, bbb_ber_run **out) {
    if (!h || !cfgs || !out || ncfg < 1) return fail(BBB_EINVAL, "null argument");
    if (ncfg > BBB_BER_MAX_GROUP) return fail(BBB_EINVAL, "a continued trial group holds at most BBB_BER_MAX_GROUP settings");
    if (calls_per_block < 1 || calls_per_block > 4096) return fail(BBB_EINVAL, "calls_per_block must be in 1..4096");
    if (h->device < 0) return fail(BBB_ENODEV, "host-only handle (device -1) cannot run trials");
    if (!h->specialised && !h->custom_ber)
        return fail(BBB_EUNSUP, "BER trials need the shipped n256 matrix, or a k = 256 matrix with its own kernels attached");
    BBB_HIP(hipSetDevice(h->device));
    const bbb_trial_cfg &c0 = cfgs[0];
    if (c0.nbits == 0) return fail(BBB_EINVAL, "nbits (bits per call) must be positive");
    std::unique_ptr<bbb_ber_run> r(new bbb_ber_run);
    r->h = h;
    r->cfgs.assign(cfgs, cfgs + ncfg);
    r->td.resize((size_t)ncfg);
    for (int i = 0; i < ncfg; i++) {
        const bbb_trial_cfg &c = cfgs[i];
        if (c.prbs_k != c0.prbs_k || c.prbs_state != c0.prbs_state || c.warmup != c0.warmup || c.first_bit != c0.first_bit || c.nbits != c0.nbits)
            return fail(BBB_EINVAL, "the settings of a continued trial group must share the PRBS, the offsets and nbits (they read one noise stream)");
        const int rc = trial_dev(c, &r->td[(size_t)i]);
        if (rc) return rc;
        if (ncfg > 1 && !single_threshold(r->td[(size_t)i]))
            return fail(BBB_EINVAL, "grouped trials must be single-threshold (a wrap-around setting runs alone)");
    }
    r->m = calls_per_block;
    r->n = c0.nbits;
    const uint64_t nblock = r->n * (uint64_t)r->m;
    if (nblock / r->m != r->n || c0.warmup + c0.first_bit + nblock < nblock) return fail(BBB_EINVAL, "bits per block overflow");
    partition(h, nblock, 2 * r->m, &r->Lb, &r->G, &r->nlanes);
    if (r->Lb / r->m >= (1ull << 27)) return fail(BBB_EINVAL, "nbits too large for one call (about 2^47): lower it");
    const int rc = r->d_totals.grow(2 * (size_t)ncfg);
    if (rc) return rc;
    if (hipMemset(r->d_totals, 0, 2 * (size_t)ncfg * sizeof(unsigned long long)) != hipSuccess)
        return fail(BBB_EHIP, "hipMemset of the run's totals failed");
    *out = r.release();
    return BBB_OK;
}

static int ber_run_step(bbb_ber_run *r, unsigned long long *counters_dev) {
    bbb_lutopt *h = r->h;
    BBB_HIP(hipSetDevice(h->device));
    int rc = begin_op(h, false);
    if (rc) return rc;
    const bbb_trial_cfg &c = r->cfgs[0];
    const int ncfg = (int)r->cfgs.size();
    const uint64_t nblock = r->n * (uint64_t)r->m, block_first = c.first_bit + r->block * nblock;
    if (block_first + nblock < block_first || c.warmup + block_first + nblock + 1 < nblock) return fail(BBB_EINVAL, "stream position overflows");
    if (r->call == 0) {
        JumpPlan *plan, *pp;
        if ((rc = get_plan(h, r->Lb, &plan))) return rc;
        if ((rc = get_prbs_plan(h, c.prbs_k, r->Lb, &pp))) return rc;
        if ((rc = ensure_top_tables(plan))) return rc;
        if ((rc = r->d_states.grow((size_t)65536 * h->W32))) return rc;
        if ((rc = r->d_planes.grow((size_t)h->k * r->nlanes))) return rc;
        if ((rc = r->d_pplanes.grow((size_t)32 * r->nlanes))) return rc;
        uint32_t s16[256];
        first16_at(h, *plan, c.warmup + block_first + 1, s16);
        uint64_t ps0 = 0;
        if ((rc = prbs_state_at_host(c.prbs_k, c.prbs_state, block_first, &ps0))) return rc;
        uint64_t ps64[8] = {ps0};
        uint32_t ps16[256];
        first16(*pp, ps64, ps16);
        { const int rcs_ = ensure_side_stream(h); if (rcs_) return rcs_; }
        if ((rc = r->fork.record(h->cs))) return rc;
        BBB_HIP(hipStreamWaitEvent(h->side, r->fork, 0));
        if ((rc = prbs_seed_lanes_launch(c.prbs_k, pp->d_cols, ps16, pp->qcol64, r->G, r->nlanes, r->d_pplanes, h->side))) return rc;
        if ((rc = r->join.record(h->side))) return rc;
        if ((rc = awgn_seed_head_launch(h->k, plan->d_cols, s16, r->G, r->d_states, h->cs))) return rc;
        if ((rc = awgn_seed_tail_planes_launch(h->k, plan->d_top, r->G, r->d_states, r->nlanes, r->d_planes, h->cs))) return rc;
        BBB_HIP(hipStreamWaitEvent(h->cs, r->join, 0));
    }
    const uint64_t Lc = r->Lb / r->m;
    const uint64_t last_total = nblock - (r->G - 1) * r->Lb, lo = (uint64_t)r->call * Lc;
    const uint64_t last_len = last_total <= lo ? 0 : (last_total - lo < Lc ? last_total - lo : Lc);
    const uint64_t bits_now = (r->G - 1) * Lc + last_len;
    for (int i = 0; i < ncfg; i++) {
        TrialDev &t = r->td[(size_t)i];
        t.L = (uint32_t)Lc; t.G = r->G; t.nbits = bits_now;
        t.flags = kTrialLastLen | kTrialSaveState; t.last_len = (uint32_t)last_len;
    }
    if (h->specialised) {
        if ((rc = ber256_launch(r->d_planes, r->d_pplanes, r->td.data(), ncfg, r->nlanes, counters_dev, h->cs))) return rc;
    } else {
        const int e = h->custom_ber(r->d_planes, r->d_pplanes, r->td.data(), ncfg, r->nlanes, (uint64_t *)counters_dev, (void *)h->cs);
        if (e) return fail(e < 0 ? e : BBB_EHIP, "custom BER kernel failed");
    }
    if (++r->call == r->m) { r->call = 0; r->block++; }
    return BBB_OK;
}

int bbb_ber_run_next_dev(bbb_ber_run *r, uint64_t *counters_dev) {
    if (!r || !counters_dev) return fail(BBB_EINVAL, "null argument");
    return ber_run_step(r, (unsigned long long *)counters_dev);
}

int bbb_ber_run_next(bbb_ber_run *r, bbb_ber *totals) {
    if (!r) return fail(BBB_EINVAL, "null argument");
    int rc = ber_run_step(r, r->d_totals);
    if (rc || !totals) return rc;
    const size_t need = 2 * r->cfgs.size();
    std::vector<unsigned long long> host(need);
    BBB_HIP(hipMemcpyAsync(host.data(), r->d_totals, need * sizeof(unsigned long long), hipMemcpyDeviceToHost, r->h->stream));
    BBB_HIP(hipStreamSynchronize(r->h->stream));
    for (size_t i = 0; i < r->cfgs.size(); i++) {
        totals[i].bits = host[2 * i];
        totals[i].errors = host[2 * i + 1];
    }
    return BBB_OK;
}

int bbb_ber_run_tell(const bbb_ber_run *r, uint64_t *calls_done, uint64_t *next_block_first_bit) {
    if (!r) return fail(BBB_EINVAL, "null argument");
    if (calls_done) *calls_done = r->block * r->m + r->call;
    if (next_block_first_bit) *next_block_first_bit = r->cfgs[0].first_bit + (r->block + (r->call ? 1 : 0)) * r->n * (uint64_t)r->m;
    return BBB_OK;
}

int bbb_ber_run_close(bbb_ber_run *r) {
    if (!r) return BBB_OK;
    if (r->h && r->h->device >= 0) (void)hipSetDevice(r->h->device);
    if (r->h && r->h->stream) (void)hipStreamSynchronize(r->h->stream);
    if (r->h && r->h->cs_valid) (void)hipStreamSynchronize(r->h->cs);
    if (r->h && r->h->side) (void)hipStreamSynchronize(r->h->side);
    delete r;
    return BBB_OK;
}


int bbb_sweep_shard(const bbb_trial_cfg *cfgs, int ncfg, int ndev, int rank, int mode, bbb_trial_cfg *mine) {
    const int e = sweep_shard(cfgs, ncfg, ndev, rank, mode, mine);
    if (e == -2) return fail(BBB_EINVAL, "first_bit + nbits overflows");
    if (e) return fail(BBB_EINVAL, "bad shard arguments (ndev >= 1, 0 <= rank < ndev, mode BBB_SHARD_TRIALS / _SEEDS / _BITS)");
    return BBB_OK;
}

namespace {

struct CommSet { std::vector<int> devs; std::vector<ncclComm_t> comms; };
std::mutex g_comm_mu;
std::vector<CommSet> g_comm_sets;

int get_comms(const std::vector<int> &devs, std::vector<ncclComm_t> *out) {
    const Rccl &r = rccl();
    if (!r.ok) return fail(BBB_EUNSUP, r.error);
    std::lock_guard<std::mutex> g(g_comm_mu);
    for (const CommSet &c : g_comm_sets)
        if (c.devs == devs) { *out = c.comms; return BBB_OK; }
    CommSet c;
    c.devs = devs;
    c.comms.resize(devs.size());
    const ncclResult_t e = r.CommInitAll(c.comms.data(), (int)devs.size(), devs.data());
    if (e != ncclSuccess) return fail(BBB_EHIP, std::string("ncclCommInitAll: ") + r.GetErrorString(e));
    g_comm_sets.push_back(c);
    *out = c.comms;
    return BBB_OK;
}

}

namespace {
std::mutex g_multi_info_mu;
bbb_multi_info g_multi_info{};
}

int bbb_multi_last_info(bbb_multi_info *out) {
    if (!out) return fail(BBB_EINVAL, "null argument");
    std::lock_guard<std::mutex> g(g_multi_info_mu);
    *out = g_multi_info;
    return BBB_OK;
}

int bbb_multi_release(void) {
    {
        std::lock_guard<std::mutex> gs(g_streams_mu);
        for (auto &kv : g_streams) {
            if (hipSetDevice(kv.first) != hipSuccess) continue;
            for (hipStream_t st : {kv.second.xs[0], kv.second.xs[1], kv.second.side})
                if (st) (void)hipStreamDestroy(st);
        }
        g_streams.clear();
    }
    std::lock_guard<std::mutex> g(g_comm_mu);
    const Rccl &r = rccl();
    for (CommSet &c : g_comm_sets)
        for (ncclComm_t comm : c.comms)
            if (r.ok && comm) (void)r.CommDestroy(comm);
    g_comm_sets.clear();
    return BBB_OK;
}

int bbb_ber_sweep_multi(bbb_lutopt *const *handles, int ndev, const bbb_trial_cfg *cfgs, int ncfg, int mode, bbb_ber *out) {
    if (!handles || ndev < 1 || ncfg < 0 || (ncfg && (!cfgs || !out))) return fail(BBB_EINVAL, "null argument");
    if (ncfg == 0) return BBB_OK;
    struct DeviceGuard {
        int dev = -1;
        DeviceGuard() { if (hipGetDevice(&dev) != hipSuccess) dev = -1; }
        ~DeviceGuard() { if (dev >= 0) (void)hipSetDevice(dev); }
    } device_guard;
    const bool rehearsal = env_knob("BBB_MULTI_REHEARSAL", 0) != 0;
    std::vector<int> devs((size_t)ndev);
    for (int r = 0; r < ndev; r++) {
        if (!handles[r]) return fail(BBB_EINVAL, "null handle");
        if (handles[r]->device < 0) return fail(BBB_ENODEV, "host-only handle (device -1) cannot run trials");
        devs[(size_t)r] = handles[r]->device;
        for (int q = 0; q < r; q++) {
            if (handles[q] == handles[r]) return fail(BBB_EINVAL, "the same handle twice");
            if (devs[(size_t)q] == devs[(size_t)r] && !rehearsal) return fail(BBB_EINVAL, "every handle must live on its own device");
        }
    }
    {
        std::vector<bbb_trial_cfg> probe((size_t)ncfg);
        const int e = bbb_sweep_shard(cfgs, ncfg, ndev, 0, mode, probe.data());
        if (e) return e;
    }
    std::vector<ncclComm_t> comms;
    int rc = rehearsal ? BBB_OK : get_comms(devs, &comms);
    if (rc) return rc;
    const size_t nwords = 2 * (size_t)ncfg;
    {
        std::string err;
        int bad = 0;
        rc = run_shares_on_threads(cfgs, ncfg, ndev, mode, [&](int r, const bbb_trial_cfg *mine, std::string *etext) -> int {
            bbb_lutopt *h = handles[r];
            auto body = [&]() -> int {
                BBB_HIP(hipSetDevice(h->device));
                int e = ensure_counters(h, nwords);
                if (e) return e;
                if ((e = take_clean_counters(h, nwords))) return e;
                return ber_run(h, mine, ncfg, h->d_counters);
            };
            const int e = body();
            if (e) *etext = last_error();
            return e;
        }, &err, &bad);
        if (rc) return fail(rc, "device " + std::to_string(devs[(size_t)bad]) + ": " + err);
    }
    if (!rehearsal) {
        const Rccl &nccl = rccl();
        if (ndev > 1) {
            ncclResult_t e = nccl.GroupStart();
            for (int r = 0; r < ndev && e == ncclSuccess; r++)
                e = nccl.AllReduce(handles[r]->d_counters, handles[r]->d_counters, nwords, ncclUint64, ncclSum, comms[(size_t)r],
                                   handles[r]->stream);
            const ncclResult_t e2 = nccl.GroupEnd();
            if (e == ncclSuccess) e = e2;
            if (e != ncclSuccess) return fail(BBB_EHIP, std::string("ncclAllReduce: ") + nccl.GetErrorString(e));
        }
        int seen = 0;
        if (nccl.CommCount(comms[0], &seen) != ncclSuccess) seen = -1;
        std::lock_guard<std::mutex> gi(g_multi_info_mu);
        g_multi_info = bbb_multi_info{};
        g_multi_info.n_devices = ndev;
        g_multi_info.n_ranks_seen = seen;
        g_multi_info.rccl_reused = nccl.reused ? 1 : 0;
        std::snprintf(g_multi_info.rccl_path, sizeof g_multi_info.rccl_path, "%s", nccl.path.c_str());
    } else {
        std::lock_guard<std::mutex> gi(g_multi_info_mu);
        g_multi_info = bbb_multi_info{};
        g_multi_info.n_devices = ndev;
        g_multi_info.n_ranks_seen = 0;
    }
    for (int r = 0; r < ndev; r++) {
        BBB_HIP(hipSetDevice(handles[r]->device));
        if ((rc = read_back_counters(handles[r], nwords))) return rc;
    }
    for (int r = 0; r < ndev; r++) {
        BBB_HIP(hipSetDevice(handles[r]->device));
        BBB_HIP(hipStreamSynchronize(handles[r]->stream));
    }
    std::vector<std::vector<unsigned long long>> host((size_t)ndev);
    for (int r = 0; r < ndev; r++) host[(size_t)r].assign(handles[r]->h_counters.p, handles[r]->h_counters.p + nwords);
    if (rehearsal) {
        for (int r = 1; r < ndev; r++)
            for (size_t i = 0; i < nwords; i++) host[0][i] += host[(size_t)r][i];
    } else {
        for (int r = 1; r < ndev; r++)
            if (host[(size_t)r] != host[0]) return fail(BBB_EHIP, "ranks disagree after the all-reduce");
    }
    for (int i = 0; i < ncfg; i++) {
        out[i].bits = host[0][2 * (size_t)i];
        out[i].errors = host[0][2 * (size_t)i + 1];
    }
    return BBB_OK;
}

}

namespace bbb {
int lutopt_device(const bbb_lutopt *h) { return h->device; }
hipStream_t lutopt_stream(const bbb_lutopt *h) { return h->stream; }
int tx_cfg_check(const bbb_tx_cfg *cfg) { return tx_check(cfg); }

int lutopt_k(const bbb_lutopt *h) { return h->k; }
int lutopt_staged_level(const bbb_lutopt *h) { return h->staged_level; }

int lutopt_stage_visit(bbb_lutopt *h, uint64_t nsamples, uint64_t first_step, lutopt_stage_visitor visit, void *ctx) {
    if (!h || !visit) return fail(BBB_EINVAL, "null argument");
    if (!h->specialised || h->device < 0) return fail(BBB_EUNSUP, "the staged sample kernel exists for the shipped n256 matrix on a device");
    if (nsamples == 0 || first_step + nsamples < first_step) return fail(BBB_EINVAL, "empty range, or first_step + nsamples overflows");
    BBB_HIP(hipSetDevice(h->device));
    StagedRun run;
    return staged_produce(h, nsamples, first_step + 1, true, false, [] { return BBB_OK; },
                          [&](const StagedRun &r, const void *stage, hipStream_t ms) {
                              return visit(ctx, stage, nsamples, (unsigned)r.L, r.G, r.nlanes, ms);
                          }, &run);
}
}
```

### basebandboard_amd/csrc/prbs_kernels.hip

```cpp
#include "bbb_common.hpp"
#include "gf2.hpp"

#include <cstdlib>
#include <mutex>
#include <vector>

namespace bbb {

typedef unsigned long long u64;
typedef u64 u64x2 __attribute__((ext_vector_type(2)));

__host__ __device__ constexpr int tap_of(int k) {
    return k == 7 ? 6 : k == 9 ? 5 : k == 11 ? 9 : k == 15 ? 14 : k == 20 ? 3 : k == 23 ? 18 : k == 31 ? 28 : 0;
}
static int k_index(int k) {
    switch (k) { case 7: return 0; case 9: return 1; case 11: return 2; case 15: return 3;
                 case 20: return 4; case 23: return 5; case 31: return 6; default: return -1; }
}

struct PrbsPowTable { uint32_t rows[64][32]; };
__device__ PrbsPowTable d_prbs_pow[7];

static const PrbsPowTable &host_pow_table(int k) {
    static PrbsPowTable tabs[7];
    static std::once_flag once[7];
    const int ki = k_index(k);
    std::call_once(once[ki], [&] {
        GF2Powers pw(prbs_matrix(k, tap_of(k)));
        for (int i = 0; i < 64; i++) {
            const GF2Mat &m = pw.pow2(i);
            for (int r = 0; r < 32; r++) tabs[ki].rows[i][r] = r < k ? (uint32_t)m.row(r)[0] : 0u;
        }
    });
    return tabs[ki];
}

static int upload_pow_table(int k) {
    static std::mutex mu;
    static bool done[64][7];
    int dev = 0;
    BBB_HIP(hipGetDevice(&dev));
    std::lock_guard<std::mutex> g(mu);
    const int ki = k_index(k);
    if (dev < 64 && done[dev][ki]) return BBB_OK;
    const PrbsPowTable &t = host_pow_table(k);
    BBB_HIP(hipMemcpyToSymbol(HIP_SYMBOL(d_prbs_pow), &t, sizeof t, sizeof(PrbsPowTable) * (size_t)ki));
    if (dev < 64) done[dev][ki] = true;
    return BBB_OK;
}

int prbs_state_at_host(int k, uint64_t init_state, uint64_t nbits, uint64_t *state) {
    if (!tap_of(k)) return fail(BBB_EINVAL, "k=" + std::to_string(k) + " invalid for PRBS");
    const PrbsPowTable &t = host_pow_table(k);
    uint32_t s = (uint32_t)init_state;
    for (int i = 0; nbits; i++, nbits >>= 1) {
        if (!(nbits & 1)) continue;
        uint32_t ns = 0;
        for (int r = 0; r < k; r++) ns |= (uint32_t)(__builtin_popcount(t.rows[i][r] & s) & 1) << r;
        s = ns;
    }
    *state = s;
    return BBB_OK;
}

template <int K>
__device__ __forceinline__ uint32_t lfsr_matvec(const uint32_t *__restrict rows, uint32_t s) {
    uint32_t ns = 0;
#pragma unroll
    for (int r = 0; r < K; r++) ns |= (uint32_t)(__builtin_popcount(rows[r] & s) & 1) << r;
    return ns;
}

typedef uint32_t u32x2 __attribute__((ext_vector_type(2)));
typedef uint32_t u32x4 __attribute__((ext_vector_type(4)));
template <int WPL> struct LaneWords;
template <> struct LaneWords<1> { typedef u32x2 type; };
template <> struct LaneWords<2> { typedef u32x4 type; };
__device__ __forceinline__ uint32_t popc_words(u32x2 v) { return (uint32_t)(__builtin_popcount(v.x) + __builtin_popcount(v.y)); }
__device__ __forceinline__ uint32_t popc_words(u32x4 v) {
    return (uint32_t)(__builtin_popcount(v.x) + __builtin_popcount(v.y) + __builtin_popcount(v.z) + __builtin_popcount(v.w));
}
__device__ __forceinline__ void xor_inplace(u32x2 &a, const u32x2 &b) {
    asm("v_xor_b32 %0, %0, %1" : "+v"(a.x) : "v"(b.x));
    asm("v_xor_b32 %0, %0, %1" : "+v"(a.y) : "v"(b.y));
}
__device__ __forceinline__ void xor_inplace(u32x4 &a, const u32x4 &b) {
    asm("v_xor_b32 %0, %0, %1" : "+v"(a.x) : "v"(b.x));
    asm("v_xor_b32 %0, %0, %1" : "+v"(a.y) : "v"(b.y));
    asm("v_xor_b32 %0, %0, %1" : "+v"(a.z) : "v"(b.z));
    asm("v_xor_b32 %0, %0, %1" : "+v"(a.w) : "v"(b.w));
}

template <typename T>
__device__ __forceinline__ T check_load(const T *p) {
    return __builtin_nontemporal_load(p);
}
template <typename T>
__device__ __forceinline__ void fill_store(T *p, const T &v) {
    *p = v;
}

template <int K, bool CHECK, int WPL, bool LW>
__global__ void __launch_bounds__(64, 2)
prbs_stream_kernel(int ki, u64 init_state, u64 first_bit, u64 nbits, u64 nwords, u64 rows_per_wave,
                   u64 *__restrict buf, u64 *__restrict nerr, int nt_stores) {
    typedef typename LaneWords<WPL>::type lw_t;
    constexpr int TAP = tap_of(K);
    constexpr int RW = 64 * WPL;
    constexpr int LEVELS = WPL == 2 ? 7 : 6;
    constexpr uint32_t SMASK = (uint32_t)((1ull << K) - 1ull);
    __shared__ __attribute__((aligned(16))) u64 X[K * RW];
    const int lane = threadIdx.x;
    const u64 row0 = (u64)blockIdx.x * rows_per_wave;
    const u64 word0 = row0 * RW;
    if (word0 >= nwords) return;
    const PrbsPowTable &pw = d_prbs_pow[ki];

    {
    constexpr u64 PERIOD = (1ull << K) - 1ull;
    constexpr u64 BACK = (u64)K * RW * 64;
    constexpr u64 WRAP = ((BACK + PERIOD - 1) / PERIOD) * PERIOD;
    const u64 t0 = (first_bit % PERIOD) + (word0 * 64) % PERIOD + (WRAP - BACK);
    uint32_t s = (uint32_t)init_state;
#pragma unroll 1
    for (int i0 = 0; i0 < 64; i0 += 16) {
        if (((t0 >> i0) & 0xffffull) == 0) continue;
        uint32_t myrow[16];
#pragma unroll
        for (int i = 0; i < 16; i++) myrow[i] = pw.rows[i0 + i][lane & 31];
#pragma unroll
        for (int i = 0; i < 16; i++) {
            if ((t0 >> (i0 + i)) & 1) s = (uint32_t)__ballot(lane < K && (__builtin_popcount(myrow[i] & s) & 1));
        }
    }
    if (lane < K) {
        uint32_t si = s;
#pragma unroll
        for (int m = 0; m < 5; m++) {
            const uint32_t sj = lfsr_matvec<K>(pw.rows[6 + m], si);
            si = ((lane >> m) & 1) ? sj : si;
        }
        u64 w = 0;
        for (int j = 0; j < 64; j++) {
            const uint32_t bit = ((si >> (K - 1)) ^ (si >> (TAP - 1))) & 1u;
            si = ((si << 1) | bit) & SMASK;
            w |= (u64)bit << j;
        }
        X[lane] = w;
    }
    }
    __syncthreads();
    {
        int known = K;
#pragma unroll 1
        for (int j = 0; j < LEVELS; j++) {
            const int lagk = K << j, lagt = TAP << j, target = K << (j + 1);
            while (known < target) {
                const int cnt = min(lagt, target - known);
                for (int base = 0; base < cnt; base += 64) {
                    const int o = base + lane;
                    if (o < cnt) X[known + o] = X[known + o - lagk] ^ X[known + o - lagt];
                }
                known += cnt;
                __syncthreads();
            }
        }
    }
    lw_t *Xv = reinterpret_cast<lw_t *>(X);
    lw_t V[LW ? 1 : K];
    if (!LW) {
#pragma unroll
        for (int q = 0; q < K; q++) V[q] = Xv[q * 64 + lane];
    }

    const u64 rows_total = (nwords - word0 + RW - 1) / RW;
    const u64 nrows = rows_total < rows_per_wave ? rows_total : rows_per_wave;
    const u64 last_word = nwords - 1;
    const u64 last_mask = (nbits & 63) ? ((1ull << (nbits & 63)) - 1ull) : ~0ull;
    u64 errs = 0;

    constexpr int DB = WPL == 2 ? 8 : 16;
    constexpr int NB = (K + DB - 1) / DB;
    for (u64 q0 = 0; q0 < nrows; q0 += K) {
        const u64 wbase = word0 + q0 * RW + (u64)(WPL * lane);
        u64 *rowp = buf + (word0 + q0 * RW);
        if (q0 + K <= nrows && word0 + (q0 + K) * RW <= last_word) {
            if (CHECK) {
                lw_t D[2][DB];
#pragma unroll
                for (int i = 0; i < DB && i < K; i++) D[0][i] = check_load(reinterpret_cast<const lw_t *>(rowp + (u64)i * RW) + lane);
                if (!LW) {
#pragma unroll
                    for (int i = 0; i < K; i++) xor_inplace(V[i], V[(i - TAP + K) % K]);
                }
                uint32_t e32 = 0;
                constexpr int PD = 6;
                constexpr int LAG = K - TAP;
                lw_t O[LW ? K : 1], N[LW ? K : 1];
                if (LW) {
#pragma unroll
                    for (int j = 0; j < K; j++)
                        if ((j >= LAG ? j - LAG : j) < PD) O[j] = Xv[j * 64 + lane];
                }
#pragma unroll
                for (int bidx = 0; bidx < NB; bidx++) {
                    if (bidx + 1 < NB) {
#pragma unroll
                        for (int i = 0; i < DB; i++)
                            if ((bidx + 1) * DB + i < K)
                                D[(bidx + 1) & 1][i] = check_load(reinterpret_cast<const lw_t *>(rowp + (u64)((bidx + 1) * DB + i) * RW) + lane);
                    }
#pragma unroll
                    for (int i = 0; i < DB; i++) {
                        const int r = bidx * DB + i;
                        if (r < K) {
                            if (LW) {
#pragma unroll
                                for (int j = 0; j < K; j++)
                                    if ((j >= LAG ? j - LAG : j) == r + PD) O[j] = Xv[j * 64 + lane];
                                N[r] = O[r] ^ (r < TAP ? O[(r + LAG) % K] : N[(r - TAP + K) % K]);
                                Xv[r * 64 + lane] = N[r];
                                e32 += popc_words(D[bidx & 1][i] ^ N[r]);
                            } else {
                                e32 += popc_words(D[bidx & 1][i] ^ V[r]);
                            }
                        }
                    }
                }
                errs += e32;
            } else if (LW) {
                lw_t W[K];
#pragma unroll
                for (int i = 0; i < K; i++) W[i] = Xv[i * 64 + lane];
#pragma unroll
                for (int i = 0; i < K; i++) W[i] ^= W[(i - TAP + K) % K];
#pragma unroll
                for (int i = 0; i < K; i++) Xv[i * 64 + lane] = W[i];
                if (nt_stores) {
#pragma unroll
                    for (int i = 0; i < K; i++) __builtin_nontemporal_store(W[i], reinterpret_cast<lw_t *>(rowp + (u64)i * RW) + lane);
                } else {
#pragma unroll
                    for (int i = 0; i < K; i++) fill_store(reinterpret_cast<lw_t *>(rowp + (u64)i * RW) + lane, W[i]);
                }
            } else {
#pragma unroll
                for (int i = 0; i < K; i++) xor_inplace(V[i], V[(i - TAP + K) % K]);
                if (nt_stores) {
#pragma unroll
                    for (int i = 0; i < K; i++) __builtin_nontemporal_store(V[i], reinterpret_cast<lw_t *>(rowp + (u64)i * RW) + lane);
                } else {
#pragma unroll
                    for (int i = 0; i < K; i++) fill_store(reinterpret_cast<lw_t *>(rowp + (u64)i * RW) + lane, V[i]);
                }
            }
            continue;
        }
        if (LW) {
#pragma unroll
            for (int i = 0; i < K; i++) Xv[i * 64 + lane] = Xv[i * 64 + lane] ^ Xv[((i - TAP + K) % K) * 64 + lane];
        } else {
#pragma unroll
            for (int i = 0; i < K; i++) xor_inplace(V[i], V[(i - TAP + K) % K]);
#pragma unroll
            for (int q = 0; q < K; q++) Xv[q * 64 + lane] = V[q];
        }
#pragma unroll 1
        for (int i = 0; i < K && q0 + i < nrows; i++) {
#pragma unroll
            for (int e = 0; e < WPL; e++) {
                const u64 w = wbase + (u64)i * RW + e;
                if (w > last_word) continue;
                u64 v = X[i * RW + WPL * lane + e];
                if (w == last_word) v &= last_mask;
                if (CHECK) {
                    u64 d = buf[w] ^ v;
                    if (w == last_word) d &= last_mask;
                    errs += (u64)__builtin_popcountll(d);
                } else {
                    buf[w] = v;
                }
            }
        }
    }
    if (CHECK) {
#pragma unroll
        for (int off = 32; off > 0; off >>= 1) errs += __shfl_xor(errs, off, 64);
        if (lane == 0 && errs) atomicAdd(nerr, errs);
    }
}

template <int K>
__global__ void __launch_bounds__(64, 2)
prbs_check_rev_kernel(int ki, u64 init_state, u64 first_bit, u64 nbits, u64 nwords, u64 rows_per_wave,
                      const u64 *__restrict buf, u64 *__restrict nerr) {
    constexpr int TAP = tap_of(K);
    constexpr int RW = 64;
    constexpr int LEVELS = 6;
    constexpr uint32_t SMASK = (uint32_t)((1ull << K) - 1ull);
    __shared__ __attribute__((aligned(16))) u64 X[K * RW];
    const int lane = threadIdx.x;
    const u64 row0 = (u64)blockIdx.x * rows_per_wave;
    const u64 word0 = row0 * RW;
    if (word0 >= nwords) return;
    const PrbsPowTable &pw = d_prbs_pow[ki];
    const u64 rows_total = (nwords - word0 + RW - 1) / RW;
    const long long nrows = (long long)(rows_total < rows_per_wave ? rows_total : rows_per_wave);

    {
    constexpr u64 PERIOD = (1ull << K) - 1ull;
    const u64 wtop = word0 + (u64)nrows * RW;
    const u64 t0 = (first_bit % PERIOD) + ((wtop % PERIOD) * 64) % PERIOD;
    uint32_t s = (uint32_t)init_state;
#pragma unroll 1
    for (int i0 = 0; i0 < 64; i0 += 16) {
        if (((t0 >> i0) & 0xffffull) == 0) continue;
        uint32_t myrow[16];
#pragma unroll
        for (int i = 0; i < 16; i++) myrow[i] = pw.rows[i0 + i][lane & 31];
#pragma unroll
        for (int i = 0; i < 16; i++) {
            if ((t0 >> (i0 + i)) & 1) s = (uint32_t)__ballot(lane < K && (__builtin_popcount(myrow[i] & s) & 1));
        }
    }
    if (lane < K) {
        uint32_t si = s;
#pragma unroll
        for (int m = 0; m < 5; m++) {
            const uint32_t sj = lfsr_matvec<K>(pw.rows[6 + m], si);
            si = ((lane >> m) & 1) ? sj : si;
        }
        u64 w = 0;
        for (int j = 0; j < 64; j++) {
            const uint32_t bit = ((si >> (K - 1)) ^ (si >> (TAP - 1))) & 1u;
            si = ((si << 1) | bit) & SMASK;
            w |= (u64)bit << j;
        }
        X[lane] = w;
    }
    }
    __syncthreads();
    {
        int known = K;
#pragma unroll 1
        for (int j = 0; j < LEVELS; j++) {
            const int lagk = K << j, lagt = TAP << j, target = K << (j + 1);
            while (known < target) {
                const int cnt = min(lagt, target - known);
                for (int base = 0; base < cnt; base += 64) {
                    const int o = base + lane;
                    if (o < cnt) X[known + o] = X[known + o - lagk] ^ X[known + o - lagt];
                }
                known += cnt;
                __syncthreads();
            }
        }
    }
    u32x2 *Xv = reinterpret_cast<u32x2 *>(X);
    u32x2 V[K];
#pragma unroll
    for (int q = 0; q < K; q++) V[q] = Xv[q * 64 + lane];

    const u64 last_word = nwords - 1;
    const u64 last_mask = (nbits & 63) ? ((1ull << (nbits & 63)) - 1ull) : ~0ull;
    u64 errs = 0;
    constexpr int DB = 16;
    constexpr int NB = (K + DB - 1) / DB;
    for (long long q0 = nrows - K; q0 > -(long long)K; q0 -= K) {
#pragma unroll
        for (int i = K - 1; i >= 0; i--) xor_inplace(V[i], V[(i - TAP + K) % K]);
        if (q0 >= 0 && word0 + (u64)(q0 + K) * RW <= last_word) {
            const u64 *rowp = buf + (word0 + (u64)q0 * RW);
            u32x2 D[2][DB];
#pragma unroll
            for (int i = 0; i < DB && i < K; i++) D[0][i] = check_load(reinterpret_cast<const u32x2 *>(rowp + (u64)i * RW) + lane);
            uint32_t e32 = 0;
#pragma unroll
            for (int bidx = 0; bidx < NB; bidx++) {
                if (bidx + 1 < NB) {
#pragma unroll
                    for (int i = 0; i < DB; i++)
                        if ((bidx + 1) * DB + i < K)
                            D[(bidx + 1) & 1][i] = check_load(reinterpret_cast<const u32x2 *>(rowp + (u64)((bidx + 1) * DB + i) * RW) + lane);
                }
#pragma unroll
                for (int i = 0; i < DB; i++) {
                    const int r = bidx * DB + i;
                    if (r < K) e32 += popc_words(D[bidx & 1][i] ^ V[r]);
                }
            }
            errs += e32;
            continue;
        }
        __syncthreads();
#pragma unroll
        for (int q = 0; q < K; q++) Xv[q * 64 + lane] = V[q];
        __syncthreads();
#pragma unroll 1
        for (int i = 0; i < K; i++) {
            const long long r = q0 + i;
            if (r < 0 || r >= nrows) continue;
            const u64 w = word0 + (u64)r * RW + (u64)lane;
            if (w > last_word) continue;
            u64 d = buf[w] ^ X[i * RW + lane];
            if (w == last_word) d &= last_mask;
            errs += (u64)__builtin_popcountll(d);
        }
    }
#pragma unroll
    for (int off = 32; off > 0; off >>= 1) errs += __shfl_xor(errs, off, 64);
    if (lane == 0 && errs) atomicAdd(nerr, errs);
}

static int launch_check_rev(int k, int ki, u64 init_state, u64 first_bit, u64 nbits, const u64 *buf, u64 *nerr, hipStream_t st) {
    const u64 nwords = (nbits + 63) / 64;
    const u64 RW = 64;
    const u64 rows = (nwords + RW - 1) / RW;
    int dev = 0, ncu = 256, per_cu = 4;
    BBB_HIP(hipGetDevice(&dev));
    BBB_HIP(hipDeviceGetAttribute(&ncu, hipDeviceAttributeMultiprocessorCount, dev));
    const void *fn = nullptr;
#define BBB_PRBS_FN(KK) case KK: fn = (const void *)prbs_check_rev_kernel<KK>; break;
    switch (k) { BBB_PRBS_FN(7) BBB_PRBS_FN(9) BBB_PRBS_FN(11) BBB_PRBS_FN(15) BBB_PRBS_FN(20) BBB_PRBS_FN(23) BBB_PRBS_FN(31) }
#undef BBB_PRBS_FN
    {
        static std::mutex mu;
        static int cached_per_cu[8] = {0};
        std::lock_guard<std::mutex> g(mu);
        int &slot = cached_per_cu[ki];
        if (slot == 0) {
            if (hipOccupancyMaxActiveBlocksPerMultiprocessor(&per_cu, fn, 64, 0) != hipSuccess || per_cu < 1) per_cu = 4;
            slot = per_cu;
        }
        per_cu = slot;
    }
    static const int cap_env = env_knob("BBB_PRBS_WAVES_PER_CU", -1);
    const int cap = cap_env > 0 ? cap_env : 4;
    if (per_cu > cap) per_cu = cap;
    const u64 target_waves = (u64)ncu * (u64)per_cu;
    u64 rpw = (rows + target_waves - 1) / target_waves;
    const u64 min_rpw = 8 * (u64)k;
    if (rpw < min_rpw) rpw = min_rpw;
    const u64 nblocks = (rows + rpw - 1) / rpw;
    if (nblocks > 0x7fffffffull) return fail(BBB_EINVAL, "nbits too large");
    dim3 grid((unsigned)nblocks), block(64);
#define BBB_PRBS_CASE(KK)                                                                                          \
    case KK:                                                                                                       \
        hipLaunchKernelGGL((prbs_check_rev_kernel<KK>), grid, block, 0, st, ki, init_state, first_bit, nbits, nwords, \
                           rpw, buf, nerr);                                                                        \
        break;
    switch (k) {
        BBB_PRBS_CASE(7) BBB_PRBS_CASE(9) BBB_PRBS_CASE(11) BBB_PRBS_CASE(15)
        BBB_PRBS_CASE(20) BBB_PRBS_CASE(23) BBB_PRBS_CASE(31)
    }
#undef BBB_PRBS_CASE
    BBB_HIP(hipGetLastError());
    return BBB_OK;
}

static int prbs_wpl(bool check) {
    static const int fill = env_knob("BBB_PRBS_FILL_WPL", 1);
    static const int chk = env_knob("BBB_PRBS_CHECK_WPL", 1);
    const int v = check ? chk : fill;
    return v == 1 ? 1 : 2;
}

template <bool CHECK, int WPL, bool LW>
static int launch_stream_w(int k, int ki, u64 init_state, u64 first_bit, u64 nbits, u64 *buf, u64 *nerr, hipStream_t st, int nt_stores) {
    const u64 nwords = (nbits + 63) / 64;
    const u64 RW = 64 * WPL;
    const u64 rows = (nwords + RW - 1) / RW;
    int dev = 0, ncu = 256, per_cu = 4;
    BBB_HIP(hipGetDevice(&dev));
    BBB_HIP(hipDeviceGetAttribute(&ncu, hipDeviceAttributeMultiprocessorCount, dev));
    const void *fn = nullptr;
#define BBB_PRBS_FN(KK) case KK: fn = (const void *)prbs_stream_kernel<KK, CHECK, WPL, LW>; break;
    switch (k) { BBB_PRBS_FN(7) BBB_PRBS_FN(9) BBB_PRBS_FN(11) BBB_PRBS_FN(15) BBB_PRBS_FN(20) BBB_PRBS_FN(23) BBB_PRBS_FN(31) }
#undef BBB_PRBS_FN
    {
        static std::mutex mu;
        static int cached_per_cu[8] = {0};
        std::lock_guard<std::mutex> g(mu);
        int &slot = cached_per_cu[ki];
        if (slot == 0) {
            if (hipOccupancyMaxActiveBlocksPerMultiprocessor(&per_cu, fn, 64, 0) != hipSuccess || per_cu < 1) per_cu = 4;
            slot = per_cu;
        }
        per_cu = slot;
    }
    static const int cap_env = env_knob("BBB_PRBS_WAVES_PER_CU", -1);
    const int cap = cap_env >= 0 ? cap_env : (CHECK ? 0 : 4);
    if (cap > 0 && per_cu > cap) per_cu = cap;
    const u64 target_waves = (u64)ncu * (u64)per_cu;
    u64 rpw = (rows + target_waves - 1) / target_waves;
    const u64 min_rpw = 8 * (u64)k;
    if (rpw < min_rpw) rpw = min_rpw;
    const u64 nblocks = (rows + rpw - 1) / rpw;
    if (nblocks > 0x7fffffffull) return fail(BBB_EINVAL, "nbits too large");
    dim3 grid((unsigned)nblocks), block(64);
#define BBB_PRBS_CASE(KK)                                                                                       \
    case KK:                                                                                                    \
        hipLaunchKernelGGL((prbs_stream_kernel<KK, CHECK, WPL, LW>), grid, block, 0, st, ki, init_state, first_bit, \
                           nbits, nwords, rpw, buf, nerr, nt_stores);                                           \
        break;
    switch (k) {
        BBB_PRBS_CASE(7) BBB_PRBS_CASE(9) BBB_PRBS_CASE(11) BBB_PRBS_CASE(15)
        BBB_PRBS_CASE(20) BBB_PRBS_CASE(23) BBB_PRBS_CASE(31)
    }
#undef BBB_PRBS_CASE
    BBB_HIP(hipGetLastError());
    return BBB_OK;
}

template <bool CHECK>
static int launch_stream(int k, u64 init_state, u64 first_bit, u64 nbits, u64 *buf, u64 *nerr, hipStream_t st, int nt_stores = 0) {
    const int ki = k_index(k);
    if (ki < 0) return fail(BBB_EINVAL, "k=" + std::to_string(k) + " invalid for PRBS");
    if (init_state == 0 || init_state >> k) return fail(BBB_EINVAL, "PRBS state must be in [1, 2^k)");
    if (nbits == 0) return BBB_OK;
    if ((uintptr_t)buf & 15) return fail(BBB_EINVAL, "packed PRBS buffer must be 16-byte aligned");
    if (first_bit + nbits < first_bit) return fail(BBB_EINVAL, "first_bit + nbits overflows");
    int rc = upload_pow_table(k);
    if (rc) return rc;
    static const int lw_fill = env_knob("BBB_PRBS_FILL_LW", 0);
    static const int lw_chk = env_knob("BBB_PRBS_CHECK_LW", 0);
    const bool lw = CHECK ? lw_chk != 0 : lw_fill != 0;
    static const int rev = env_knob("BBB_PRBS_CHECK_REV", 1);
    if (CHECK && rev && !lw && prbs_wpl(true) == 1) return launch_check_rev(k, ki, init_state, first_bit, nbits, buf, nerr, st);
    if (prbs_wpl(CHECK) == 1)
        return lw ? launch_stream_w<CHECK, 1, true>(k, ki, init_state, first_bit, nbits, buf, nerr, st, nt_stores)
                  : launch_stream_w<CHECK, 1, false>(k, ki, init_state, first_bit, nbits, buf, nerr, st, nt_stores);
    return lw ? launch_stream_w<CHECK, 2, true>(k, ki, init_state, first_bit, nbits, buf, nerr, st, nt_stores)
              : launch_stream_w<CHECK, 2, false>(k, ki, init_state, first_bit, nbits, buf, nerr, st, nt_stores);
}

int prbs_fill_launch(int k, uint64_t init_state, uint64_t first_bit, uint64_t nbits, uint64_t *dst, hipStream_t st, int nt_stores) {
    return launch_stream<false>(k, init_state, first_bit, nbits, (u64 *)dst, nullptr, st, nt_stores);
}
int prbs_check_launch(int k, uint64_t init_state, uint64_t first_bit, uint64_t nbits, const uint64_t *src,
                      uint64_t *nerr_dev, hipStream_t st) {
    return launch_stream<true>(k, init_state, first_bit, nbits, (u64 *)const_cast<uint64_t *>(src), (u64 *)nerr_dev, st);
}

__global__ void __launch_bounds__(256)
prbs_detector_kernel(int k, int tap, const uint8_t *__restrict bits, u64 nstreams, u64 n,
                     uint8_t *__restrict err, uint8_t *__restrict reload) {
    const u64 sidx = (u64)blockIdx.x * blockDim.x + threadIdx.x;
    if (sidx >= nstreams) return;
    const u64 mask = (1ull << k) - 1ull;
    u64 prbs = 1, err_sr = mask;
    int bit_in = 0, reload_ctr = 0;
    const uint8_t *in = bits + sidx * n;
    for (u64 i = 0; i < n; i++) {
        const int feedback = (int)(((prbs >> (k - 1)) ^ (prbs >> (tap - 1))) & 1ull);
        const int rl = reload_ctr != 0;
        const int prbs_in = rl ? bit_in : feedback;
        const int e = bit_in != feedback;
        const int err_count = __builtin_popcountll(err_sr);
        prbs = ((prbs << 1) | (u64)prbs_in) & mask;
        u64 esr = ((err_sr << 1) | (u64)e) & mask;
        if (err_count > k / 2) {
            reload_ctr = k + k / 2;
            esr = 0;
        } else if (rl) {
            reload_ctr -= 1;
        }
        err_sr = esr;
        bit_in = in[i] & 1;
        if (err) err[sidx * n + i] = (uint8_t)(bit_in != (int)(((prbs >> (k - 1)) ^ (prbs >> (tap - 1))) & 1ull));
        if (reload) reload[sidx * n + i] = (uint8_t)(reload_ctr != 0);
    }
}

int prbs_detector_launch(int k, const uint8_t *bits, uint64_t nstreams, uint64_t n, uint8_t *err,
                         uint8_t *reload, hipStream_t st) {
    const int tap = tap_of(k);
    if (!tap) return fail(BBB_EINVAL, "k=" + std::to_string(k) + " invalid for PRBS");
    if (nstreams == 0 || n == 0) return BBB_OK;
    const u64 nblocks = (nstreams + 255) / 256;
    if (nblocks > 0x7fffffffull) return fail(BBB_EINVAL, "too many streams");
    hipLaunchKernelGGL(prbs_detector_kernel, dim3((unsigned)nblocks), dim3(256), 0, st, k, tap, bits,
                       (u64)nstreams, (u64)n, err, reload);
    BBB_HIP(hipGetLastError());
    return BBB_OK;
}

}
```

### basebandboard_amd/prbs.py

```python
import ctypes as C

import torch

from . import _lib

TAPS = {7: 6, 9: 5, 11: 9, 15: 14, 20: 3, 23: 18, 31: 28}


def _stream_ptr(device):
    return C.c_void_p(torch.cuda.current_stream(device).cuda_stream)


def _check_k(k):
    if k not in TAPS.keys():
        raise ValueError("k={} invalid for PRBS".format(k))


class PRBS:

    def __init__(self, k, init=1, device=0):
        _check_k(k)
        if not 0 < init < (1 << k):
            raise ValueError("PRBS state must be in [1, 2^k)")
        self.k, self.init, self.device = k, int(init), int(device)

    def state_at(self, nbits):
        s = C.c_uint64()
        _lib.check(_lib.lib().bbb_prbs_state_at(self.k, self.init, int(nbits), C.byref(s)), "bbb_prbs_state_at")
        return s.value

    def generate(self, nbits, first_bit=0, out=None, will_read_back=False):
        nwords = (int(nbits) + 63) // 64
        dev = torch.device("cuda", self.device)
        if out is None:
            out = torch.empty(nwords, dtype=torch.int64, device=dev)
        if out.dtype != torch.int64 or out.numel() < nwords or not out.is_contiguous() or out.device != dev:
            raise ValueError("out must be a contiguous int64 CUDA tensor with >= ceil(nbits/64) words")
        _lib.check(_lib.lib().bbb_prbs_fill_hint(self.k, self.init, int(first_bit), int(nbits), C.c_void_p(out.data_ptr()),
                                                 1 if will_read_back else 0, self.device, _stream_ptr(self.device)), "bbb_prbs_fill")
        return out[:nwords]


class PRBSErrorDetector:

    def __init__(self, k, device=0):
        _check_k(k)
        self.k, self.device = k, int(device)

    def run(self, bits):
        if bits.dtype != torch.uint8 or bits.dim() != 2 or not bits.is_cuda:
            raise ValueError("bits must be a uint8 CUDA tensor [nstreams, n]")
        bits = bits.contiguous()
        err = torch.empty_like(bits)
        reload = torch.empty_like(bits)
        _lib.check(_lib.lib().bbb_prbs_detector_run(self.k, C.c_void_p(bits.data_ptr()), bits.shape[0], bits.shape[1],
                                                    C.c_void_p(err.data_ptr()), C.c_void_p(reload.data_ptr()),
                                                    self.device, _stream_ptr(self.device)), "bbb_prbs_detector_run")
        return err, reload

    def run_stream(self, packed, nbits, want_err=False, want_reload=False, chunk_bits=0, warm_bits=0, error_stats=None):
        if error_stats is not None:
            want_e, want_r = want_err, want_reload
            out = self.run_stream(packed, nbits, True, True, chunk_bits, warm_bits)
            error_stats.accumulate(out["err"], out["reload"], int(nbits))
            if not want_e:
                del out["err"]
            if not want_r:
                del out["reload"]
            return out
        if packed.dtype != torch.int64 or not packed.is_cuda or not packed.is_contiguous():
            raise ValueError("packed must be a contiguous int64 CUDA tensor")
        if packed.numel() * 64 < nbits:
            raise ValueError("packed holds fewer than nbits bits")
        nw = (int(nbits) + 63) // 64
        err = torch.empty(nw, dtype=torch.int64, device=packed.device) if want_err else None
        rl = torch.empty(nw, dtype=torch.int64, device=packed.device) if want_reload else None
        st = _lib.DetectorStats()
        _lib.check(_lib.lib().bbb_prbs_detector_stream(
            self.k, C.c_void_p(packed.data_ptr()), int(nbits), C.c_void_p(err.data_ptr() if want_err else None),
            C.c_void_p(rl.data_ptr() if want_reload else None), C.byref(st), int(chunk_bits), int(warm_bits),
            self.device, _stream_ptr(self.device)), "bbb_prbs_detector_stream")
        out = {n: int(getattr(st, n)) for n, _ in _lib.DetectorStats._fields_}
        if want_err:
            out["err"] = err
        if want_reload:
            out["reload"] = rl
        return out

    def count_errors(self, packed, nbits, first_bit=0, init=1):
        if packed.dtype != torch.int64 or not packed.is_cuda or not packed.is_contiguous():
            raise ValueError("packed must be a contiguous int64 CUDA tensor")
        if packed.numel() * 64 < nbits:
            raise ValueError("packed holds fewer than nbits bits")
        n = C.c_uint64()
        _lib.check(_lib.lib().bbb_prbs_check(self.k, int(init), int(first_bit), int(nbits), C.c_void_p(packed.data_ptr()),
                                             C.byref(n), self.device, _stream_ptr(self.device)), "bbb_prbs_check")
        return n.value
```

### experiments/prbs_sweep.py

```python
import os, subprocess, sys, json
if len(sys.argv) > 1:
    import torch, ctypes as C
    sys.path.insert(0, os.path.dirname(os.path.dirname(os.path.abspath(__file__))))
    import basebandboard_amd as bbb
    bbb._lib.select_build("experiments")
    nbits = 10_000_000_000
    p = bbb.PRBS(31); det = bbb.PRBSErrorDetector(31)
    buf = torch.empty((nbits + 63)//64, dtype=torch.int64, device="cuda")
    p.generate(nbits, out=buf); n0 = det.count_errors(buf, nbits)
    torch.cuda.synchronize()
    e = [torch.cuda.Event(enable_timing=True) for _ in range(3)]
    g = c = 0.0
    for _ in range(5):
        e[0].record(); p.generate(nbits, out=buf); e[1].record(); n = det.count_errors(buf, nbits); e[2].record()
        torch.cuda.synchronize(); g += e[0].elapsed_time(e[1]); c += e[1].elapsed_time(e[2])
    print(json.dumps({"cfg": sys.argv[1], "errors": n0, "gen_TBs": nbits/8*5/g/1e9, "chk_TBs": nbits/8*5/c/1e9}))
else:
    def run(tag, **kv):
        env = dict(os.environ, **{k: str(v) for k, v in kv.items()})
        subprocess.run([sys.executable, __file__, tag + " " + " ".join(f"{k[9:]}={v}" for k, v in kv.items())], env=env)
    for cap in (0, 4, 8):
        for wpl in (1, 2):
            for lw in (0, 1):
                if wpl == 2 and lw == 0:
                    continue
                run("FILL ", BBB_PRBS_FILL_WPL=wpl, BBB_PRBS_FILL_LW=lw, BBB_PRBS_WAVES_PER_CU=cap)
                run("CHECK", BBB_PRBS_CHECK_WPL=wpl, BBB_PRBS_CHECK_LW=lw, BBB_PRBS_WAVES_PER_CU=cap)
```

### include/bbb.h

```cpp
#ifndef BBB_H
#define BBB_H

#include <stddef.h>
#include <stdint.h>

#ifdef __cplusplus
extern "C" {
#endif

#define BBB_OK        0
#define BBB_EINVAL   -1
#define BBB_ENOMEM   -2
#define BBB_EHIP     -3
#define BBB_EIO      -4
#define BBB_ENODEV   -5
#define BBB_EUNSUP   -6

#define BBB_ABI_VERSION 1
#define BBB_MAX_K 512

int bbb_abi_version(void);
const char *bbb_strerror(int code);
const char *bbb_last_error_detail(void);
int bbb_device_count(int *count);
void bbb_free(void *p);


typedef struct bbb_lutopt bbb_lutopt;

int bbb_lutopt_load_matrix_file(const char *path, int *k, uint16_t **taps, uint32_t **row_off);

int bbb_lutopt_create(bbb_lutopt **h, int k, const uint16_t *taps, const uint32_t *row_off,
                      const uint64_t *init_words, int device);
int bbb_lutopt_destroy(bbb_lutopt *h);
int bbb_lutopt_set_stream(bbb_lutopt *h, void *hip_stream);
int bbb_lutopt_is_specialised(const bbb_lutopt *h);

int bbb_lutopt_profile(bbb_lutopt *h, int enable);
int bbb_lutopt_profile_read(bbb_lutopt *h, double *seed_ms, double *kernel_ms, uint64_t *calls, int reset);
int bbb_lutopt_profile_read_mover(bbb_lutopt *h, double *mover_ms, uint64_t *calls, int reset);

int bbb_lutopt_state_at(bbb_lutopt *h, uint64_t nsteps, uint64_t *state_words);

int bbb_lutopt_fill_words(bbb_lutopt *h, uint32_t *dst_dev, uint64_t nstates, uint64_t first_step, int msb_first);

int bbb_awgn_fill_i8(bbb_lutopt *h, int8_t *dst_dev, uint64_t nsamples, uint64_t first_step);
int bbb_awgn_prefetch(bbb_lutopt *h, uint64_t nsamples, uint64_t first_step);
int bbb_lutopt_set_staged(bbb_lutopt *h, int enable);
int bbb_awgn_fill_i16(bbb_lutopt *h, int16_t *dst_dev, uint64_t nsamples, uint64_t first_step);

typedef struct bbb_awgn_stream bbb_awgn_stream;
int bbb_awgn_stream_open(bbb_lutopt *h, uint64_t nsamples_per_call, uint64_t first_step, int elem_bytes, bbb_awgn_stream **s);
int bbb_awgn_stream_next(bbb_awgn_stream *s, void *dst_dev);
int bbb_awgn_stream_read(bbb_awgn_stream *s, void *dst_dev, uint64_t nsamples);
int bbb_awgn_stream_seek(bbb_awgn_stream *s, uint64_t first_step);
int bbb_awgn_stream_tell(const bbb_awgn_stream *s, uint64_t *next_step);
int bbb_awgn_stream_close(bbb_awgn_stream *s);

int bbb_awgn_hist(bbb_lutopt *h, uint64_t *hist_dev, uint64_t nsamples, uint64_t first_step);

int bbb_clt_tree_i16(int k, const uint64_t *states_dev, uint64_t nstates, int16_t *out_dev,
                     int device, void *hip_stream);


int bbb_prbs_fill(int k, uint64_t init_state, uint64_t first_bit, uint64_t nbits,
                  uint64_t *dst_packed_dev, int device, void *hip_stream);
#define BBB_PRBS_WILL_READ_BACK 1u
int bbb_prbs_fill_hint(int k, uint64_t init_state, uint64_t first_bit, uint64_t nbits,
                       uint64_t *dst_packed_dev, unsigned flags, int device, void *hip_stream);
int bbb_prbs_check(int k, uint64_t init_state, uint64_t first_bit, uint64_t nbits,
                   const uint64_t *src_packed_dev, uint64_t *nerr, int device, void *hip_stream);
int bbb_prbs_check_dev(int k, uint64_t init_state, uint64_t first_bit, uint64_t nbits,
                       const uint64_t *src_packed_dev, uint64_t *nerr_dev, int device,
                       void *hip_stream);
int bbb_prbs_state_at(int k, uint64_t init_state, uint64_t nbits, uint64_t *state);

int bbb_prbs_detector_run(int k, const uint8_t *bits_dev, uint64_t nstreams, uint64_t n,
                          uint8_t *err_dev, uint8_t *reload_dev, int device, void *hip_stream);

typedef struct {
    uint64_t bits;
    uint64_t errors;
    uint64_t errors_raw;
    uint64_t reload_clocks;
    uint64_t resyncs;
    uint64_t chunks;
    uint64_t chunks_rerun;
    uint64_t serial_fallback;
} bbb_detector_stats;
int bbb_prbs_detector_stream(int k, const uint64_t *bits_packed_dev, uint64_t nbits, uint64_t *err_packed_dev,
                             uint64_t *reload_packed_dev, bbb_detector_stats *stats, uint64_t chunk_bits,
                             uint64_t warm_bits, int device, void *hip_stream);

typedef int (*bbb_custom_fill_fn)(const uint32_t *planes_dev, int8_t *dst_dev, uint64_t nsamples, uint32_t L, uint64_t G,
                                  uint32_t nlanes, void *hip_stream);
int bbb_lutopt_set_custom_fill(bbb_lutopt *h, bbb_custom_fill_fn fn);
typedef int (*bbb_custom_ber_fn)(uint32_t *planes_dev, uint32_t *prbs_planes_dev, const void *trials, int ncfg,
                                 uint32_t nlanes, uint64_t *counters_dev, void *hip_stream);
int bbb_lutopt_set_custom_ber(bbb_lutopt *h, bbb_custom_ber_fn fn);
int bbb_lutopt_attach_custom_library(bbb_lutopt *h, const char *path);


typedef struct {
    int32_t  prbs_k;
    int32_t  amp;
    int32_t  noise_var;
    int32_t  reserved;
    uint64_t prbs_state;
    uint64_t warmup;
    uint64_t first_bit;
    uint64_t nbits;
} bbb_trial_cfg;

typedef struct { uint64_t bits, errors; } bbb_ber;

int bbb_ber_trials(bbb_lutopt *h, const bbb_trial_cfg *cfgs, int ncfg, bbb_ber *out);
int bbb_ber_trials_dev(bbb_lutopt *h, const bbb_trial_cfg *cfgs, int ncfg, uint64_t *counters_dev);

typedef struct bbb_ber_run bbb_ber_run;
int bbb_ber_run_open(bbb_lutopt *h, const bbb_trial_cfg *cfgs, int ncfg, uint32_t calls_per_block, bbb_ber_run **out);
int bbb_ber_run_next(bbb_ber_run *r, bbb_ber *totals);
int bbb_ber_run_next_dev(bbb_ber_run *r, uint64_t *counters_dev);
int bbb_ber_run_tell(const bbb_ber_run *r, uint64_t *calls_done, uint64_t *next_block_first_bit);
int bbb_ber_run_close(bbb_ber_run *r);

#define BBB_SHARD_TRIALS 0
#define BBB_SHARD_SEEDS 1
#define BBB_SHARD_BITS 2
#define BBB_SHARD_GROUPS 3
int bbb_ber_sweep_multi(bbb_lutopt *const *handles, int ndev, const bbb_trial_cfg *cfgs, int ncfg, int mode,
                        bbb_ber *out);
int bbb_sweep_shard(const bbb_trial_cfg *cfgs, int ncfg, int ndev, int rank, int mode, bbb_trial_cfg *mine);
typedef struct {
    int32_t n_devices;
    int32_t n_ranks_seen;
    int32_t rccl_reused;
    int32_t reserved;
    char    rccl_path[256];
} bbb_multi_info;
int bbb_multi_last_info(bbb_multi_info *out);
int bbb_multi_release(void);


typedef struct {
    int16_t  coeffs[64];
    int32_t  source;
    int32_t  prbs_k;
    uint64_t prbs_state;
    int32_t  bit_en, noise_en, noise_var, reserved;
    uint64_t warmup;
} bbb_tx_cfg;

int bbb_shaper_fill_i16(const bbb_tx_cfg *cfg, int16_t *out_dev, uint64_t nsamples, uint64_t first_sample,
                        int device, void *hip_stream);
int bbb_tx_fill_i16(bbb_lutopt *h, const bbb_tx_cfg *cfg, int16_t *out_dev, uint64_t nsamples,
                    uint64_t first_sample);
typedef struct bbb_tx_stream bbb_tx_stream;
int bbb_tx_stream_open(bbb_lutopt *h, const bbb_tx_cfg *cfg, uint64_t nsamples_per_call, uint64_t first_sample, bbb_tx_stream **s);
int bbb_tx_stream_next(bbb_tx_stream *s, int16_t *out_dev);
int bbb_tx_stream_read(bbb_tx_stream *s, int16_t *out_dev, uint64_t nsamples);
int bbb_tx_stream_seek(bbb_tx_stream *s, uint64_t first_sample);
int bbb_tx_stream_tell(const bbb_tx_stream *s, uint64_t *next_sample);
int bbb_tx_stream_close(bbb_tx_stream *s);

int bbb_rx_slice(const int16_t *samples_dev, uint64_t nsamples, uint64_t stride, uint64_t phase, int strict,
                 uint64_t *bits_packed_dev, uint64_t *nbits_out, int device, void *hip_stream);

int bbb_rx_phase_search(const int16_t *samples_dev, uint64_t nsamples, uint64_t stride, uint64_t nphases, int strict,
                        int k, bbb_detector_stats *stats_out, int device, void *hip_stream);


#define BBB_TX_BIT_SAMPLE0 45
typedef struct {
    uint32_t ncols;
    uint32_t shift;
    uint64_t col_origin;
    int32_t  threshold;
    int32_t  strict;
} bbb_eye_cfg;

int bbb_eye_accumulate_i16(const int16_t *samples_dev, uint64_t nsamples, uint64_t first_sample, const bbb_eye_cfg *eye,
                           uint64_t *hist_dev, int device, void *hip_stream);
typedef struct bbb_tx_eye bbb_tx_eye;
int bbb_tx_eye_open(bbb_lutopt *h, const bbb_tx_cfg *cfg, const bbb_eye_cfg *eye, uint64_t chunk_samples, bbb_tx_eye **out);
int bbb_tx_eye_run(bbb_tx_eye *e, uint64_t first_sample, uint64_t nsamples, uint64_t *hist_dev, uint64_t *bathtub_dev);
int bbb_tx_eye_close(bbb_tx_eye *e);


typedef struct {
    int16_t coeffs[64];
    int32_t bit_en, noise_en, noise_var;
    int32_t threshold, strict;
    int32_t reserved;
} bbb_tx_setting;
typedef struct bbb_tx_ber_sweep bbb_tx_ber_sweep;
int bbb_tx_ber_sweep_open(bbb_lutopt *h, const bbb_tx_cfg *base, const bbb_tx_setting *settings, int nset,
                          uint64_t chunk_samples, bbb_tx_ber_sweep **out);
int bbb_tx_ber_sweep_run(bbb_tx_ber_sweep *s, uint64_t first_sample, uint64_t nsamples, uint64_t *counters_dev);
int bbb_tx_ber_sweep_close(bbb_tx_ber_sweep *s);


#define BBB_ACF_MAX_LAGS 4096
int bbb_acf_accumulate_i16(const int16_t *samples_dev, uint64_t nfirst, uint64_t navail, uint32_t nlags,
                           int64_t *acf_dev, int device, void *hip_stream);
typedef struct bbb_tx_acf bbb_tx_acf;
int bbb_tx_acf_open(bbb_lutopt *h, const bbb_tx_cfg *cfg, uint32_t nlags, uint64_t chunk_samples, bbb_tx_acf **out);
int bbb_tx_acf_run(bbb_tx_acf *a, uint64_t first_sample, uint64_t nsamples, int64_t *acf_dev);
int bbb_tx_acf_close(bbb_tx_acf *a);


#define BBB_XCORR_MAX_LAGS 1024
#define BBB_TX_BIT_ORIGIN 17
typedef struct { uint32_t spb; uint32_t nlags; uint64_t origin; } bbb_xcorr_cfg;
int bbb_xcorr_accumulate_i16(const int16_t *samples_dev, uint64_t nsamples, uint64_t first_sample,
                             const uint64_t *bits_packed_dev, uint64_t bit0, uint64_t nbits,
                             const bbb_xcorr_cfg *cfg, int64_t *xc_dev, int device, void *hip_stream);
typedef struct bbb_tx_xcorr bbb_tx_xcorr;
int bbb_tx_xcorr_open(bbb_lutopt *h, const bbb_tx_cfg *cfg, uint32_t nlags, uint64_t chunk_samples, bbb_tx_xcorr **out);
int bbb_tx_xcorr_run(bbb_tx_xcorr *x, uint64_t first_sample, uint64_t nsamples, int64_t *xc_dev);
int bbb_tx_xcorr_close(bbb_tx_xcorr *x);


typedef struct { uint32_t fcw; uint32_t am; int32_t fm; int32_t pm; } bbb_nco_cfg;
typedef struct { uint32_t pa; int32_t q, w, y; } bbb_nco_state;
typedef struct bbb_nco bbb_nco;
int bbb_nco_rom(int16_t rom[1024]);
int bbb_nco_open(const bbb_nco_cfg *cfg, int device, void *hip_stream, bbb_nco **out);
int bbb_nco_set_cfg(bbb_nco *o, const bbb_nco_cfg *cfg);
int bbb_nco_set_stream(bbb_nco *o, void *hip_stream);
int bbb_nco_run(bbb_nco *o, const int32_t *fm_dev, const uint16_t *am_dev, const int16_t *pm_dev, uint64_t nsamples,
                int16_t *x_dev);
int bbb_nco_get_state(bbb_nco *o, bbb_nco_state *st);
int bbb_nco_set_state(bbb_nco *o, const bbb_nco_state *st);
int bbb_nco_close(bbb_nco *o);


#define BBB_SINC_UP   16
#define BBB_SINC_TAPS 8
int bbb_sinc_coefficients(int8_t h[128]);

typedef struct {
    uint32_t in_bytes;
    uint32_t out_bytes;
    uint32_t shift;
} bbb_sinc_cfg;

int bbb_sinc_interpolate(const void *in_dev, uint64_t nin, uint32_t nbefore, const bbb_sinc_cfg *cfg, void *out_dev,
                         int device, void *hip_stream);

typedef struct bbb_sinc_eye bbb_sinc_eye;
int bbb_sinc_eye_open(const bbb_sinc_cfg *cfg, const bbb_eye_cfg *eye, uint64_t chunk_in, int device, void *hip_stream,
                      bbb_sinc_eye **out);
int bbb_sinc_eye_run(bbb_sinc_eye *e, const void *in_dev, uint64_t nin, uint32_t nbefore, uint64_t first_sample,
                     uint64_t *hist_dev);
int bbb_sinc_eye_close(bbb_sinc_eye *e);


#define BBB_FIR_MAX_TAPS 256
typedef struct {
    uint32_t ntaps;
    int16_t  taps[256];
    uint32_t shift;
    uint32_t decim;
    uint32_t phase;
    uint32_t out_bytes;
} bbb_fir_cfg;

int bbb_fir_moving_average(bbb_fir_cfg *cfg, int pipeline);

int bbb_fir_filter(const int16_t *in_dev, uint64_t nin, uint32_t nbefore, const bbb_fir_cfg *cfg, void *out_dev,
                   uint64_t *nout_out, int device, void *hip_stream);

int bbb_fir_slice(const int16_t *in_dev, uint64_t nin, uint32_t nbefore, const bbb_fir_cfg *cfg, int32_t threshold,
                  int strict, uint64_t *bits_packed_dev, uint64_t *nbits_out, int device, void *hip_stream);


#define BBB_DDC_IQ16  0
#define BBB_DDC_IQ32  1
#define BBB_DDC_POLAR 2
typedef struct { uint32_t fcw; uint32_t pa0; uint32_t mode;  } bbb_ddc_cfg;
int bbb_ddc_run(const int16_t *in_dev, uint64_t nin, uint32_t nbefore, uint64_t first_sample,
                const bbb_ddc_cfg *ddc, const bbb_fir_cfg *fir ,
                void *out_dev, uint64_t *nout_out, int device, void *hip_stream);
int bbb_ddc_polar_host(int16_t i, int16_t q, uint16_t *mag, int16_t *phase);


#define BBB_DFE_MAX_FB 4
typedef struct {
    bbb_fir_cfg ff;
    uint32_t nfb;
    int32_t  fb[4];
    int32_t  threshold;
    uint32_t strict;
    uint32_t region_symbols;
    uint32_t warmup_symbols;
} bbb_dfe_cfg;

int bbb_dfe_run(const int16_t *in_dev, uint64_t nin, uint32_t nbefore, const bbb_dfe_cfg *cfg, uint32_t *state_dev,
                uint64_t *bits_packed_dev, void *soft_dev, uint64_t *stats_dev, uint64_t *nbits_out, int device,
                void *hip_stream);
int bbb_dfe_geometry(uint32_t decim, uint64_t *step_samples, uint64_t *step_symbols, uint64_t *wave_symbols,
                     uint64_t *region_symbols, uint64_t *warmup_symbols);
int bbb_dfe_model_host(const int16_t *in, uint64_t nin, uint32_t nbefore, const bbb_dfe_cfg *cfg, uint32_t *state,
                       uint64_t *bits_packed, void *soft, uint64_t *nbits_out);


typedef struct bbb_link_sweep bbb_link_sweep;
int bbb_link_sweep_open(bbb_lutopt *h, const bbb_tx_cfg *base, const bbb_tx_setting *settings, int nset, const bbb_fir_cfg *fir,
                        uint32_t delay, const bbb_eye_cfg *eye , uint64_t chunk_samples,
                        bbb_link_sweep **out);
int bbb_link_sweep_run(bbb_link_sweep *s, uint64_t first_sample, uint64_t nsamples,
                       uint64_t *counters_dev ,
                       uint64_t *hist_dev );
int bbb_link_sweep_close(bbb_link_sweep *s);


int bbb_gf2_berlekamp_massey(const uint8_t *bits, uint64_t n, uint8_t *coeffs_out, int64_t *degree);
int bbb_gf2_recur(int nrows, int ncols, const uint64_t *col_words, const uint8_t *x_bits, int nsteps,
                  uint8_t *out_bits);

int bbb_gf2_dot(int nrows, int ncols, const uint64_t *col_words, const uint8_t *x_bits, uint8_t *out_bits);
int bbb_gf2_poly_is_primitive(const uint8_t *coeffs, int ncoeffs, int *result);
int bbb_gf2_poly_modexp(const uint8_t *coeffs, int ncoeffs, const uint64_t *exponent_words, int nwords,
                        uint8_t *out_coeffs);
int bbb_lutopt_charpoly(int k, const uint16_t *taps, const uint32_t *row_off, uint8_t *coeffs_out, int *degree);
int bbb_lutopt_is_full_period(int k, const uint16_t *taps, const uint32_t *row_off, int *result);
int bbb_lutopt_save_matrix_file(const char *path, int k, const uint16_t *taps, const uint32_t *row_off);


int bbb_lutopt_search_candidate(int k, uint64_t seed, uint64_t candidate, uint16_t *taps_out, uint32_t *row_off_out);
typedef struct {
    uint64_t tested;
    uint64_t full_degree;
    uint64_t order_divides;
    uint64_t primitive;
    uint64_t kernel_ns;
} bbb_search_stats;
int bbb_lutopt_search(int k, uint64_t seed, uint64_t first_candidate, uint64_t ncandidates, uint64_t *found_index,
                      uint16_t *taps_out, uint32_t *row_off_out, bbb_search_stats *stats, int device, void *hip_stream);


#define BBB_ERRSTAT_NBINS 312
typedef struct { uint32_t guard; uint32_t nblock; uint64_t block_bits[4]; } bbb_errstat_cfg;
typedef struct {
    uint64_t bits, errors, first_error, last_error, max_gap;
    uint64_t bursts, burst_len_sum, max_burst_len, max_burst_weight;
    uint64_t open_first, open_last, open_weight;
    uint64_t errored_blocks[4];
    uint64_t gap_hist[BBB_ERRSTAT_NBINS], burst_len_hist[BBB_ERRSTAT_NBINS], burst_weight_hist[BBB_ERRSTAT_NBINS];
} bbb_errstat_result;
typedef struct bbb_errstat bbb_errstat;
int bbb_errstat_open(const bbb_errstat_cfg *cfg, int device, void *hip_stream, bbb_errstat **out);
int bbb_errstat_accumulate(bbb_errstat *e, const uint64_t *err_packed_dev, const uint64_t *mask_packed_dev ,
                           uint64_t nbits);
int bbb_errstat_skip(bbb_errstat *e, uint64_t nbits);
int bbb_errstat_read(bbb_errstat *e, bbb_errstat_result *out);
int bbb_errstat_reset(bbb_errstat *e);
int bbb_errstat_set_stream(bbb_errstat *e, void *hip_stream);
int bbb_errstat_geometry(uint64_t *tile_bits, uint64_t *wave_bits);
int bbb_errstat_close(bbb_errstat *e);

#ifdef __cplusplus
}
#endif
#endif
```

Before: 966.7.

## Interleave PRBS rows across waves with strided recurrence and new partition planner

```diff
diff --git a/basebandboard_amd/_lib.py b/basebandboard_amd/_lib.py
--- a/basebandboard_amd/_lib.py
+++ b/basebandboard_amd/_lib.py
@@ -13,7 +13,7 @@
     "bbb_abi_version", "bbb_strerror", "bbb_last_error_detail", "bbb_device_count", "bbb_free",
     "bbb_lutopt_load_matrix_file", "bbb_lutopt_create", "bbb_lutopt_destroy", "bbb_lutopt_set_stream",
     "bbb_lutopt_is_specialised", "bbb_lutopt_set_staged", "bbb_lutopt_set_custom_fill", "bbb_lutopt_set_custom_ber", "bbb_lutopt_attach_custom_library", "bbb_lutopt_profile", "bbb_lutopt_profile_read", "bbb_lutopt_profile_read_mover", "bbb_lutopt_state_at", "bbb_lutopt_fill_words", "bbb_awgn_fill_i8", "bbb_awgn_fill_i16", "bbb_awgn_prefetch", "bbb_awgn_stream_open", "bbb_awgn_stream_next", "bbb_awgn_stream_read", "bbb_awgn_stream_seek", "bbb_awgn_stream_tell", "bbb_awgn_stream_close", "bbb_awgn_hist",
-    "bbb_clt_tree_i16", "bbb_prbs_fill", "bbb_prbs_fill_hint", "bbb_prbs_check", "bbb_prbs_check_dev", "bbb_prbs_state_at",
+    "bbb_clt_tree_i16", "bbb_prbs_fill", "bbb_prbs_fill_hint", "bbb_prbs_check", "bbb_prbs_check_dev", "bbb_prbs_state_at", "bbb_prbs_partition_info",
     "bbb_prbs_detector_run", "bbb_prbs_detector_stream", "bbb_ber_trials", "bbb_ber_trials_dev", "bbb_ber_run_open", "bbb_ber_run_next", "bbb_ber_run_next_dev", "bbb_ber_run_tell", "bbb_ber_run_close", "bbb_ber_sweep_multi", "bbb_sweep_shard", "bbb_multi_last_info", "bbb_multi_release", "bbb_shaper_fill_i16", "bbb_tx_fill_i16", "bbb_tx_stream_open", "bbb_tx_stream_next", "bbb_tx_stream_read", "bbb_tx_stream_seek", "bbb_tx_stream_tell", "bbb_tx_stream_close", "bbb_rx_slice", "bbb_rx_phase_search", "bbb_eye_accumulate_i16", "bbb_tx_eye_open", "bbb_tx_eye_run", "bbb_tx_eye_close", "bbb_tx_ber_sweep_open", "bbb_tx_ber_sweep_run", "bbb_tx_ber_sweep_close", "bbb_acf_accumulate_i16", "bbb_tx_acf_open", "bbb_tx_acf_run", "bbb_tx_acf_close", "bbb_nco_rom", "bbb_nco_open", "bbb_nco_set_cfg", "bbb_nco_set_stream", "bbb_nco_run", "bbb_nco_get_state", "bbb_nco_set_state", "bbb_nco_close", "bbb_sinc_coefficients", "bbb_sinc_interpolate", "bbb_sinc_eye_open", "bbb_sinc_eye_run", "bbb_sinc_eye_close", "bbb_fir_moving_average", "bbb_fir_filter", "bbb_fir_slice", "bbb_link_sweep_open", "bbb_link_sweep_run", "bbb_link_sweep_close", "bbb_gf2_berlekamp_massey", "bbb_gf2_recur",
     "bbb_gf2_dot", "bbb_gf2_poly_is_primitive", "bbb_gf2_poly_modexp", "bbb_lutopt_charpoly", "bbb_lutopt_is_full_period",
     "bbb_lutopt_save_matrix_file", "bbb_lutopt_search_candidate", "bbb_lutopt_search",
@@ -174,6 +174,7 @@
     l.bbb_prbs_check.argtypes = [i32, u64, u64, u64, vp, u64p, i32, vp]
     l.bbb_prbs_check_dev.argtypes = [i32, u64, u64, u64, vp, vp, i32, vp]
     l.bbb_prbs_state_at.argtypes = [i32, u64, u64, u64p]
+    l.bbb_prbs_partition_info.argtypes = [i32, u64, i32, i32, C.POINTER(C.c_uint32), C.POINTER(C.c_uint32)]
     l.bbb_prbs_detector_run.argtypes = [i32, vp, u64, u64, vp, vp, i32, vp]
     l.bbb_rx_phase_search.argtypes = [vp, u64, u64, u64, i32, i32, C.POINTER(DetectorStats), i32, vp]
     l.bbb_prbs_detector_stream.argtypes = [i32, vp, u64, vp, vp, C.POINTER(DetectorStats), u64, u64, i32, vp]
diff --git a/basebandboard_amd/csrc/bbb_api.hip b/basebandboard_amd/csrc/bbb_api.hip
--- a/basebandboard_amd/csrc/bbb_api.hip
+++ b/basebandboard_amd/csrc/bbb_api.hip
@@ -4,6 +4,7 @@
 #include "awgn_launch.hpp"
 #include "stage_common.hpp"
 #include "gf2.hpp"
+#include "prbs_partition.hpp"
 #include "rccl_loader.hpp"
 #include "sweep_shard.hpp"
 #include "sweep_threads.hpp"
@@ -1284,6 +1285,18 @@
     if (!state) return fail(BBB_EINVAL, "null state");
     if (init_state >> (k > 0 && k < 64 ? k : 63)) return fail(BBB_EINVAL, "PRBS state must be < 2^k");
     return prbs_state_at_host(k, init_state, nbits, state);
+}
+
+int bbb_prbs_partition_info(int k, uint64_t nbits, int pass, int device, uint32_t *waves, uint32_t *row_words) {
+    if (!waves || !row_words) return fail(BBB_EINVAL, "null output");
+    if (!prbs_tap(k)) return fail(BBB_EINVAL, "k=" + std::to_string(k) + " invalid for PRBS");
+    if (pass != BBB_PRBS_PASS_FILL && pass != BBB_PRBS_PASS_CHECK && pass != BBB_PRBS_PASS_FILL_READ_BACK) return fail(BBB_EINVAL, "unknown pass");
+    int ncu = 256;
+    if (device >= 0) BBB_HIP(hipDeviceGetAttribute(&ncu, hipDeviceAttributeMultiprocessorCount, device));
+    const PrbsPartition p = prbs_partition(k, nbits, pass, ncu);
+    *waves = p.rows_per_wave ? 1u : 1u << p.lg_w;
+    *row_words = 64u * (uint32_t)p.wpl;
+    return BBB_OK;
 }
 
 int bbb_prbs_detector_run(int k, const uint8_t *bits_dev, uint64_t nstreams, uint64_t n, uint8_t *err_dev,
diff --git a/basebandboard_amd/csrc/prbs_kernels.hip b/basebandboard_amd/csrc/prbs_kernels.hip
--- a/basebandboard_amd/csrc/prbs_kernels.hip
+++ b/basebandboard_amd/csrc/prbs_kernels.hip
@@ -1,5 +1,6 @@
 #include "bbb_common.hpp"
 #include "gf2.hpp"
+#include "prbs_partition.hpp"
 
 #include <cstdlib>
 #include <mutex>
@@ -90,6 +91,8 @@
     asm("v_xor_b32 %0, %0, %1" : "+v"(a.z) : "v"(b.z));
     asm("v_xor_b32 %0, %0, %1" : "+v"(a.w) : "v"(b.w));
 }
+template <typename T>
+__device__ __forceinline__ u64 lane_word(const T &v, int e) { return (u64)v[2 * e] | ((u64)v[2 * e + 1] << 32); }
 
 template <typename T>
 __device__ __forceinline__ T check_load(const T *p) {
@@ -100,27 +103,58 @@
     *p = v;
 }
 
-template <int K, bool CHECK, int WPL, bool LW>
-__global__ void __launch_bounds__(64, 2)
-prbs_stream_kernel(int ki, u64 init_state, u64 first_bit, u64 nbits, u64 nwords, u64 rows_per_wave,
-                   u64 *__restrict buf, u64 *__restrict nerr, int nt_stores) {
+typedef __attribute__((address_space(1))) char gchar;
+__device__ __forceinline__ gchar *uniform_ptr(const u64 *p) {
+    const u64 a = (u64)p;
+    const uint32_t lo = __builtin_amdgcn_readfirstlane((uint32_t)a), hi = __builtin_amdgcn_readfirstlane((uint32_t)(a >> 32));
+    return (gchar *)(((u64)hi << 32) | lo);
+}
+__device__ __forceinline__ uint32_t pass_lane_off(uint32_t lane_off) {
+    asm volatile("" : "+v"(lane_off));
+    return lane_off;
+}
+template <typename T>
+__device__ __forceinline__ T *lane_ptr(gchar *row_base, uint32_t lane_off, int i, int sh) {
+    return (T *)(__attribute__((address_space(1))) T *)(row_base + (lane_off + ((uint32_t)i << sh)));
+}
+
+template <int K, int WPL>
+__device__ __forceinline__ uint32_t check_pass(gchar *rowp, uint32_t lane_off, int sh, const typename LaneWords<WPL>::type (&V)[K]) {
     typedef typename LaneWords<WPL>::type lw_t;
+    constexpr int DB = WPL == 2 ? 8 : 16;
+    constexpr int NB = (K + DB - 1) / DB;
+    lw_t D[2][DB];
+#pragma unroll
+    for (int i = 0; i < DB && i < K; i++) D[0][i] = check_load(lane_ptr<const lw_t>(rowp, lane_off, i, sh));
+    __builtin_amdgcn_sched_barrier(0);
+    uint32_t e32 = 0;
+#pragma unroll
+    for (int bidx = 0; bidx < NB; bidx++) {
+        if (bidx + 1 < NB) {
+#pragma unroll
+            for (int i = 0; i < DB; i++)
+                if ((bidx + 1) * DB + i < K) D[(bidx + 1) & 1][i] = check_load(lane_ptr<const lw_t>(rowp, lane_off, (bidx + 1) * DB + i, sh));
+            __builtin_amdgcn_sched_barrier(0);
+        }
+#pragma unroll
+        for (int i = 0; i < DB; i++) {
+            const int r = bidx * DB + i;
+            if (r < K) e32 += popc_words(D[bidx & 1][i] ^ V[r]);
+        }
+        asm volatile("" : "+v"(lane_off), "+v"(e32));
+        __builtin_amdgcn_sched_barrier(0);
+    }
+    return e32;
+}
+
+template <int K, int WPL>
+__device__ __forceinline__ void prbs_window(const PrbsPowTable &pw, u64 init_state, u64 t0, int lg_s, u64 *X,
+                                            typename LaneWords<WPL>::type (&V)[K]) {
     constexpr int TAP = tap_of(K);
     constexpr int RW = 64 * WPL;
-    constexpr int LEVELS = WPL == 2 ? 7 : 6;
+    constexpr int NX = RW + K - 1;
     constexpr uint32_t SMASK = (uint32_t)((1ull << K) - 1ull);
-    __shared__ __attribute__((aligned(16))) u64 X[K * RW];
     const int lane = threadIdx.x;
-    const u64 row0 = (u64)blockIdx.x * rows_per_wave;
-    const u64 word0 = row0 * RW;
-    if (word0 >= nwords) return;
-    const PrbsPowTable &pw = d_prbs_pow[ki];
-
-    {
-    constexpr u64 PERIOD = (1ull << K) - 1ull;
-    constexpr u64 BACK = (u64)K * RW * 64;
-    constexpr u64 WRAP = ((BACK + PERIOD - 1) / PERIOD) * PERIOD;
-    const u64 t0 = (first_bit % PERIOD) + (word0 * 64) % PERIOD + (WRAP - BACK);
     uint32_t s = (uint32_t)init_state;
 #pragma unroll 1
     for (int i0 = 0; i0 < 64; i0 += 16) {
@@ -148,13 +182,12 @@
         }
         X[lane] = w;
     }
-    }
     __syncthreads();
     {
         int known = K;
 #pragma unroll 1
-        for (int j = 0; j < LEVELS; j++) {
-            const int lagk = K << j, lagt = TAP << j, target = K << (j + 1);
+        for (int j = 0; known < NX; j++) {
+            const int lagk = K << j, lagt = TAP << j, target = min(K << (j + 1), NX);
             while (known < target) {
                 const int cnt = min(lagt, target - known);
                 for (int base = 0; base < cnt; base += 64) {
@@ -166,112 +199,97 @@
             }
         }
     }
-    lw_t *Xv = reinterpret_cast<lw_t *>(X);
-    lw_t V[LW ? 1 : K];
-    if (!LW) {
-#pragma unroll
-        for (int q = 0; q < K; q++) V[q] = Xv[q * 64 + lane];
-    }
-
-    const u64 rows_total = (nwords - word0 + RW - 1) / RW;
-    const u64 nrows = rows_total < rows_per_wave ? rows_total : rows_per_wave;
+#pragma unroll
+    for (int e = 0; e < WPL; e++) {
+        u64 c[2 * K - 1];
+#pragma unroll
+        for (int i = 0; i < K; i++) c[i] = X[WPL * lane + e + i];
+#pragma unroll 1
+        for (int d = 0; d < lg_s; d++) {
+#pragma unroll
+            for (int i = K; i < 2 * K - 1; i++) c[i] = c[i - K] ^ c[i - TAP];
+#pragma unroll
+            for (int i = 1; i < K; i++) c[i] = c[2 * i];
+        }
+#pragma unroll
+        for (int i = 0; i < K; i++) {
+            V[i][2 * e] = (uint32_t)c[i];
+            V[i][2 * e + 1] = (uint32_t)(c[i] >> 32);
+        }
+    }
+}
+
+template <int RW>
+__device__ __forceinline__ bool prbs_class(u64 nwords, unsigned lg_w, u64 rows_per_wave, u64 &base_row, u64 &nrows) {
+    const u64 rows = (nwords + RW - 1) / RW;
+    if (rows_per_wave) {
+        base_row = (u64)blockIdx.x * rows_per_wave;
+        if (base_row >= rows) return false;
+        nrows = rows - base_row < rows_per_wave ? rows - base_row : rows_per_wave;
+    } else {
+        base_row = blockIdx.x;
+        if (base_row >= rows) return false;
+        nrows = (rows - base_row + ((1ull << lg_w) - 1ull)) >> lg_w;
+    }
+    return true;
+}
+
+template <int K, bool CHECK, int WPL>
+__global__ void __launch_bounds__(64, 2)
+prbs_stream_kernel(int ki, u64 init_state, u64 first_bit, u64 nbits, u64 nwords, unsigned lg_w, u64 rows_per_wave,
+                   u64 *__restrict buf, u64 *__restrict nerr, int nt_stores) {
+    typedef typename LaneWords<WPL>::type lw_t;
+    constexpr int TAP = tap_of(K);
+    constexpr int RW = 64 * WPL;
+    constexpr int LG_RW = WPL == 2 ? 7 : 6;
+    constexpr u64 PERIOD = (1ull << K) - 1ull;
+    __shared__ u64 X[RW + K - 1];
+    const int lane = threadIdx.x;
+    u64 base_row, nrows;
+    if (!prbs_class<RW>(nwords, lg_w, rows_per_wave, base_row, nrows)) return;
+    const int lg_s = LG_RW + (int)lg_w;
+    const u64 stride = 1ull << lg_s;
+
+    lw_t V[K];
+    {
+        const u64 back = (((u64)K << lg_s) * 64ull) % PERIOD;
+        const u64 t0 = (first_bit % PERIOD) + ((((base_row * RW) % PERIOD) * 64ull) % PERIOD) + (PERIOD - back);
+        prbs_window<K, WPL>(d_prbs_pow[ki], init_state, t0, lg_s, X, V);
+    }
+
     const u64 last_word = nwords - 1;
     const u64 last_mask = (nbits & 63) ? ((1ull << (nbits & 63)) - 1ull) : ~0ull;
     u64 errs = 0;
 
-    constexpr int DB = WPL == 2 ? 8 : 16;
-    constexpr int NB = (K + DB - 1) / DB;
+    const int sh = lg_s + 3;
     for (u64 q0 = 0; q0 < nrows; q0 += K) {
-        const u64 wbase = word0 + q0 * RW + (u64)(WPL * lane);
-        u64 *rowp = buf + (word0 + q0 * RW);
-        if (q0 + K <= nrows && word0 + (q0 + K) * RW <= last_word) {
+        const u64 row_word = (base_row + (q0 << lg_w)) * RW;
+        gchar *rowp = uniform_ptr(buf + row_word);
+        const uint32_t lane_off = pass_lane_off((uint32_t)(lane * (int)sizeof(lw_t)));
+#pragma unroll
+        for (int i = 0; i < K; i++) xor_inplace(V[i], V[(i - TAP + K) % K]);
+        if (q0 + K <= nrows && row_word + (u64)(K - 1) * stride + RW <= last_word) {
             if (CHECK) {
-                lw_t D[2][DB];
-#pragma unroll
-                for (int i = 0; i < DB && i < K; i++) D[0][i] = check_load(reinterpret_cast<const lw_t *>(rowp + (u64)i * RW) + lane);
-                if (!LW) {
-#pragma unroll
-                    for (int i = 0; i < K; i++) xor_inplace(V[i], V[(i - TAP + K) % K]);
-                }
-                uint32_t e32 = 0;
-                constexpr int PD = 6;
-                constexpr int LAG = K - TAP;
-                lw_t O[LW ? K : 1], N[LW ? K : 1];
-                if (LW) {
-#pragma unroll
-                    for (int j = 0; j < K; j++)
-                        if ((j >= LAG ? j - LAG : j) < PD) O[j] = Xv[j * 64 + lane];
-                }
-#pragma unroll
-                for (int bidx = 0; bidx < NB; bidx++) {
-                    if (bidx + 1 < NB) {
-#pragma unroll
-                        for (int i = 0; i < DB; i++)
-                            if ((bidx + 1) * DB + i < K)
-                                D[(bidx + 1) & 1][i] = check_load(reinterpret_cast<const lw_t *>(rowp + (u64)((bidx + 1) * DB + i) * RW) + lane);
-                    }
-#pragma unroll
-                    for (int i = 0; i < DB; i++) {
-                        const int r = bidx * DB + i;
-                        if (r < K) {
-                            if (LW) {
-#pragma unroll
-                                for (int j = 0; j < K; j++)
-                                    if ((j >= LAG ? j - LAG : j) == r + PD) O[j] = Xv[j * 64 + lane];
-                                N[r] = O[r] ^ (r < TAP ? O[(r + LAG) % K] : N[(r - TAP + K) % K]);
-                                Xv[r * 64 + lane] = N[r];
-                                e32 += popc_words(D[bidx & 1][i] ^ N[r]);
-                            } else {
-                                e32 += popc_words(D[bidx & 1][i] ^ V[r]);
-                            }
-                        }
-                    }
-                }
-                errs += e32;
-            } else if (LW) {
-                lw_t W[K];
-#pragma unroll
-                for (int i = 0; i < K; i++) W[i] = Xv[i * 64 + lane];
-#pragma unroll
-                for (int i = 0; i < K; i++) W[i] ^= W[(i - TAP + K) % K];
-#pragma unroll
-                for (int i = 0; i < K; i++) Xv[i * 64 + lane] = W[i];
+                errs += check_pass<K, WPL>(rowp, lane_off, sh, V);
+            } else {
                 if (nt_stores) {
 #pragma unroll
-                    for (int i = 0; i < K; i++) __builtin_nontemporal_store(W[i], reinterpret_cast<lw_t *>(rowp + (u64)i * RW) + lane);
+                    for (int i = 0; i < K; i++) __builtin_nontemporal_store(V[i], lane_ptr<lw_t>(rowp, lane_off, i, sh));
                 } else {
 #pragma unroll
-                    for (int i = 0; i < K; i++) fill_store(reinterpret_cast<lw_t *>(rowp + (u64)i * RW) + lane, W[i]);
-                }
-            } else {
-#pragma unroll
-                for (int i = 0; i < K; i++) xor_inplace(V[i], V[(i - TAP + K) % K]);
-                if (nt_stores) {
-#pragma unroll
-                    for (int i = 0; i < K; i++) __builtin_nontemporal_store(V[i], reinterpret_cast<lw_t *>(rowp + (u64)i * RW) + lane);
-                } else {
-#pragma unroll
-                    for (int i = 0; i < K; i++) fill_store(reinterpret_cast<lw_t *>(rowp + (u64)i * RW) + lane, V[i]);
+                    for (int i = 0; i < K; i++) fill_store(lane_ptr<lw_t>(rowp, lane_off, i, sh), V[i]);
                 }
             }
             continue;
         }
-        if (LW) {
-#pragma unroll
-            for (int i = 0; i < K; i++) Xv[i * 64 + lane] = Xv[i * 64 + lane] ^ Xv[((i - TAP + K) % K) * 64 + lane];
-        } else {
-#pragma unroll
-            for (int i = 0; i < K; i++) xor_inplace(V[i], V[(i - TAP + K) % K]);
-#pragma unroll
-            for (int q = 0; q < K; q++) Xv[q * 64 + lane] = V[q];
-        }
-#pragma unroll 1
-        for (int i = 0; i < K && q0 + i < nrows; i++) {
+#pragma unroll
+        for (int i = 0; i < K; i++) {
+            if (q0 + i >= nrows) continue;
 #pragma unroll
             for (int e = 0; e < WPL; e++) {
-                const u64 w = wbase + (u64)i * RW + e;
+                const u64 w = row_word + (u64)i * stride + (u64)(WPL * lane + e);
                 if (w > last_word) continue;
-                u64 v = X[i * RW + WPL * lane + e];
+                u64 v = lane_word(V[i], e);
                 if (w == last_word) v &= last_mask;
                 if (CHECK) {
                     u64 d = buf[w] ^ v;
@@ -281,6 +299,7 @@
                     buf[w] = v;
                 }
             }
+            __builtin_amdgcn_sched_barrier(0);
         }
     }
     if (CHECK) {
@@ -290,121 +309,54 @@
     }
 }
 
-template <int K>
+template <int K, int WPL>
 __global__ void __launch_bounds__(64, 2)
-prbs_check_rev_kernel(int ki, u64 init_state, u64 first_bit, u64 nbits, u64 nwords, u64 rows_per_wave,
+prbs_check_rev_kernel(int ki, u64 init_state, u64 first_bit, u64 nbits, u64 nwords, unsigned lg_w, u64 rows_per_wave,
                       const u64 *__restrict buf, u64 *__restrict nerr) {
+    typedef typename LaneWords<WPL>::type lw_t;
     constexpr int TAP = tap_of(K);
-    constexpr int RW = 64;
-    constexpr int LEVELS = 6;
-    constexpr uint32_t SMASK = (uint32_t)((1ull << K) - 1ull);
-    __shared__ __attribute__((aligned(16))) u64 X[K * RW];
+    constexpr int RW = 64 * WPL;
+    constexpr int LG_RW = WPL == 2 ? 7 : 6;
+    constexpr u64 PERIOD = (1ull << K) - 1ull;
+    __shared__ u64 X[RW + K - 1];
     const int lane = threadIdx.x;
-    const u64 row0 = (u64)blockIdx.x * rows_per_wave;
-    const u64 word0 = row0 * RW;
-    if (word0 >= nwords) return;
-    const PrbsPowTable &pw = d_prbs_pow[ki];
-    const u64 rows_total = (nwords - word0 + RW - 1) / RW;
-    const long long nrows = (long long)(rows_total < rows_per_wave ? rows_total : rows_per_wave);
-
+    u64 base_row, nrows_u;
+    if (!prbs_class<RW>(nwords, lg_w, rows_per_wave, base_row, nrows_u)) return;
+    const long long nrows = (long long)nrows_u;
+    const int lg_s = LG_RW + (int)lg_w;
+    const u64 stride = 1ull << lg_s;
+
+    lw_t V[K];
     {
-    constexpr u64 PERIOD = (1ull << K) - 1ull;
-    const u64 wtop = word0 + (u64)nrows * RW;
-    const u64 t0 = (first_bit % PERIOD) + ((wtop % PERIOD) * 64) % PERIOD;
-    uint32_t s = (uint32_t)init_state;
-#pragma unroll 1
-    for (int i0 = 0; i0 < 64; i0 += 16) {
-        if (((t0 >> i0) & 0xffffull) == 0) continue;
-        uint32_t myrow[16];
-#pragma unroll
-        for (int i = 0; i < 16; i++) myrow[i] = pw.rows[i0 + i][lane & 31];
-#pragma unroll
-        for (int i = 0; i < 16; i++) {
-            if ((t0 >> (i0 + i)) & 1) s = (uint32_t)__ballot(lane < K && (__builtin_popcount(myrow[i] & s) & 1));
-        }
-    }
-    if (lane < K) {
-        uint32_t si = s;
-#pragma unroll
-        for (int m = 0; m < 5; m++) {
-            const uint32_t sj = lfsr_matvec<K>(pw.rows[6 + m], si);
-            si = ((lane >> m) & 1) ? sj : si;
-        }
-        u64 w = 0;
-        for (int j = 0; j < 64; j++) {
-            const uint32_t bit = ((si >> (K - 1)) ^ (si >> (TAP - 1))) & 1u;
-            si = ((si << 1) | bit) & SMASK;
-            w |= (u64)bit << j;
-        }
-        X[lane] = w;
-    }
-    }
-    __syncthreads();
-    {
-        int known = K;
-#pragma unroll 1
-        for (int j = 0; j < LEVELS; j++) {
-            const int lagk = K << j, lagt = TAP << j, target = K << (j + 1);
-            while (known < target) {
-                const int cnt = min(lagt, target - known);
-                for (int base = 0; base < cnt; base += 64) {
-                    const int o = base + lane;
-                    if (o < cnt) X[known + o] = X[known + o - lagk] ^ X[known + o - lagt];
-                }
-                known += cnt;
-                __syncthreads();
-            }
-        }
-    }
-    u32x2 *Xv = reinterpret_cast<u32x2 *>(X);
-    u32x2 V[K];
-#pragma unroll
-    for (int q = 0; q < K; q++) V[q] = Xv[q * 64 + lane];
+        const u64 wtop = (base_row + (nrows_u << lg_w)) * RW;
+        const u64 t0 = (first_bit % PERIOD) + (((wtop % PERIOD) * 64ull) % PERIOD);
+        prbs_window<K, WPL>(d_prbs_pow[ki], init_state, t0, lg_s, X, V);
+    }
 
     const u64 last_word = nwords - 1;
     const u64 last_mask = (nbits & 63) ? ((1ull << (nbits & 63)) - 1ull) : ~0ull;
     u64 errs = 0;
-    constexpr int DB = 16;
-    constexpr int NB = (K + DB - 1) / DB;
+    const int sh = lg_s + 3;
     for (long long q0 = nrows - K; q0 > -(long long)K; q0 -= K) {
 #pragma unroll
         for (int i = K - 1; i >= 0; i--) xor_inplace(V[i], V[(i - TAP + K) % K]);
-        if (q0 >= 0 && word0 + (u64)(q0 + K) * RW <= last_word) {
-            const u64 *rowp = buf + (word0 + (u64)q0 * RW);
-            u32x2 D[2][DB];
-#pragma unroll
-            for (int i = 0; i < DB && i < K; i++) D[0][i] = check_load(reinterpret_cast<const u32x2 *>(rowp + (u64)i * RW) + lane);
-            uint32_t e32 = 0;
-#pragma unroll
-            for (int bidx = 0; bidx < NB; bidx++) {
-                if (bidx + 1 < NB) {
-#pragma unroll
-                    for (int i = 0; i < DB; i++)
-                        if ((bidx + 1) * DB + i < K)
-                            D[(bidx + 1) & 1][i] = check_load(reinterpret_cast<const u32x2 *>(rowp + (u64)((bidx + 1) * DB + i) * RW) + lane);
-                }
-#pragma unroll
-                for (int i = 0; i < DB; i++) {
-                    const int r = bidx * DB + i;
-                    if (r < K) e32 += popc_words(D[bidx & 1][i] ^ V[r]);
-                }
-            }
-            errs += e32;
+        if (q0 >= 0 && (base_row + ((u64)q0 << lg_w)) * RW + (u64)(K - 1) * stride + RW <= last_word) {
+            errs += check_pass<K, WPL>(uniform_ptr(buf + (base_row + ((u64)q0 << lg_w)) * RW), pass_lane_off((uint32_t)(lane * (int)sizeof(lw_t))), sh, V);
             continue;
         }
-        __syncthreads();
-#pragma unroll
-        for (int q = 0; q < K; q++) Xv[q * 64 + lane] = V[q];
-        __syncthreads();
-#pragma unroll 1
+#pragma unroll
         for (int i = 0; i < K; i++) {
             const long long r = q0 + i;
             if (r < 0 || r >= nrows) continue;
-            const u64 w = word0 + (u64)r * RW + (u64)lane;
-            if (w > last_word) continue;
-            u64 d = buf[w] ^ X[i * RW + lane];
-            if (w == last_word) d &= last_mask;
-            errs += (u64)__builtin_popcountll(d);
+#pragma unroll
+            for (int e = 0; e < WPL; e++) {
+                const u64 w = (base_row + ((u64)r << lg_w)) * RW + (u64)(WPL * lane + e);
+                if (w > last_word) continue;
+                u64 d = buf[w] ^ lane_word(V[i], e);
+                if (w == last_word) d &= last_mask;
+                errs += (u64)__builtin_popcountll(d);
+            }
+            __builtin_amdgcn_sched_barrier(0);
         }
     }
 #pragma unroll
@@ -412,42 +364,24 @@
     if (lane == 0 && errs) atomicAdd(nerr, errs);
 }
 
-static int launch_check_rev(int k, int ki, u64 init_state, u64 first_bit, u64 nbits, const u64 *buf, u64 *nerr, hipStream_t st) {
+template <int WPL>
+static int launch_prbs(int pass, bool rev, const PrbsPartition &p, int k, int ki, u64 init_state, u64 first_bit, u64 nbits,
+                       u64 *buf, u64 *nerr, hipStream_t st) {
     const u64 nwords = (nbits + 63) / 64;
-    const u64 RW = 64;
-    const u64 rows = (nwords + RW - 1) / RW;
-    int dev = 0, ncu = 256, per_cu = 4;
-    BBB_HIP(hipGetDevice(&dev));
-    BBB_HIP(hipDeviceGetAttribute(&ncu, hipDeviceAttributeMultiprocessorCount, dev));
-    const void *fn = nullptr;
-#define BBB_PRBS_FN(KK) case KK: fn = (const void *)prbs_check_rev_kernel<KK>; break;
-    switch (k) { BBB_PRBS_FN(7) BBB_PRBS_FN(9) BBB_PRBS_FN(11) BBB_PRBS_FN(15) BBB_PRBS_FN(20) BBB_PRBS_FN(23) BBB_PRBS_FN(31) }
-#undef BBB_PRBS_FN
-    {
-        static std::mutex mu;
-        static int cached_per_cu[8] = {0};
-        std::lock_guard<std::mutex> g(mu);
-        int &slot = cached_per_cu[ki];
-        if (slot == 0) {
-            if (hipOccupancyMaxActiveBlocksPerMultiprocessor(&per_cu, fn, 64, 0) != hipSuccess || per_cu < 1) per_cu = 4;
-            slot = per_cu;
-        }
-        per_cu = slot;
-    }
-    static const int cap_env = env_knob("BBB_PRBS_WAVES_PER_CU", -1);
-    const int cap = cap_env > 0 ? cap_env : 4;
-    if (per_cu > cap) per_cu = cap;
-    const u64 target_waves = (u64)ncu * (u64)per_cu;
-    u64 rpw = (rows + target_waves - 1) / target_waves;
-    const u64 min_rpw = 8 * (u64)k;
-    if (rpw < min_rpw) rpw = min_rpw;
-    const u64 nblocks = (rows + rpw - 1) / rpw;
-    if (nblocks > 0x7fffffffull) return fail(BBB_EINVAL, "nbits too large");
-    dim3 grid((unsigned)nblocks), block(64);
-#define BBB_PRBS_CASE(KK)                                                                                          \
-    case KK:                                                                                                       \
-        hipLaunchKernelGGL((prbs_check_rev_kernel<KK>), grid, block, 0, st, ki, init_state, first_bit, nbits, nwords, \
-                           rpw, buf, nerr);                                                                        \
+    if (p.nblocks > 0x7fffffffull) return fail(BBB_EINVAL, "nbits too large");
+    dim3 grid((unsigned)p.nblocks), block(64);
+    const int nt_stores = pass == kPrbsFillReadBack ? 1 : 0;
+#define BBB_PRBS_CASE(KK)                                                                                                   \
+    case KK:                                                                                                                \
+        if (pass == kPrbsCheck && rev)                                                                                      \
+            hipLaunchKernelGGL((prbs_check_rev_kernel<KK, WPL>), grid, block, 0, st, ki, init_state, first_bit, nbits, nwords, \
+                               p.lg_w, (u64)p.rows_per_wave, buf, nerr);                                                    \
+        else if (pass == kPrbsCheck)                                                                                        \
+            hipLaunchKernelGGL((prbs_stream_kernel<KK, true, WPL>), grid, block, 0, st, ki, init_state, first_bit, nbits,   \
+                               nwords, p.lg_w, (u64)p.rows_per_wave, buf, nerr, 0);                                         \
+        else                                                                                                                \
+            hipLaunchKernelGGL((prbs_stream_kernel<KK, false, WPL>), grid, block, 0, st, ki, init_state, first_bit, nbits,  \
+                               nwords, p.lg_w, (u64)p.rows_per_wave, buf, nerr, nt_stores);                                 \
         break;
     switch (k) {
         BBB_PRBS_CASE(7) BBB_PRBS_CASE(9) BBB_PRBS_CASE(11) BBB_PRBS_CASE(15)
@@ -458,62 +392,7 @@
     return BBB_OK;
 }
 
-static int prbs_wpl(bool check) {
-    static const int fill = env_knob("BBB_PRBS_FILL_WPL", 1);
-    static const int chk = env_knob("BBB_PRBS_CHECK_WPL", 1);
-    const int v = check ? chk : fill;
-    return v == 1 ? 1 : 2;
-}
-
-template <bool CHECK, int WPL, bool LW>
-static int launch_stream_w(int k, int ki, u64 init_state, u64 first_bit, u64 nbits, u64 *buf, u64 *nerr, hipStream_t st, int nt_stores) {
-    const u64 nwords = (nbits + 63) / 64;
-    const u64 RW = 64 * WPL;
-    const u64 rows = (nwords + RW - 1) / RW;
-    int dev = 0, ncu = 256, per_cu = 4;
-    BBB_HIP(hipGetDevice(&dev));
-    BBB_HIP(hipDeviceGetAttribute(&ncu, hipDeviceAttributeMultiprocessorCount, dev));
-    const void *fn = nullptr;
-#define BBB_PRBS_FN(KK) case KK: fn = (const void *)prbs_stream_kernel<KK, CHECK, WPL, LW>; break;
-    switch (k) { BBB_PRBS_FN(7) BBB_PRBS_FN(9) BBB_PRBS_FN(11) BBB_PRBS_FN(15) BBB_PRBS_FN(20) BBB_PRBS_FN(23) BBB_PRBS_FN(31) }
-#undef BBB_PRBS_FN
-    {
-        static std::mutex mu;
-        static int cached_per_cu[8] = {0};
-        std::lock_guard<std::mutex> g(mu);
-        int &slot = cached_per_cu[ki];
-        if (slot == 0) {
-            if (hipOccupancyMaxActiveBlocksPerMultiprocessor(&per_cu, fn, 64, 0) != hipSuccess || per_cu < 1) per_cu = 4;
-            slot = per_cu;
-        }
-        per_cu = slot;
-    }
-    static const int cap_env = env_knob("BBB_PRBS_WAVES_PER_CU", -1);
-    const int cap = cap_env >= 0 ? cap_env : (CHECK ? 0 : 4);
-    if (cap > 0 && per_cu > cap) per_cu = cap;
-    const u64 target_waves = (u64)ncu * (u64)per_cu;
-    u64 rpw = (rows + target_waves - 1) / target_waves;
-    const u64 min_rpw = 8 * (u64)k;
-    if (rpw < min_rpw) rpw = min_rpw;
-    const u64 nblocks = (rows + rpw - 1) / rpw;
-    if (nblocks > 0x7fffffffull) return fail(BBB_EINVAL, "nbits too large");
-    dim3 grid((unsigned)nblocks), block(64);
-#define BBB_PRBS_CASE(KK)                                                                                       \
-    case KK:                                                                                                    \
-        hipLaunchKernelGGL((prbs_stream_kernel<KK, CHECK, WPL, LW>), grid, block, 0, st, ki, init_state, first_bit, \
-                           nbits, nwords, rpw, buf, nerr, nt_stores);                                           \
-        break;
-    switch (k) {
-        BBB_PRBS_CASE(7) BBB_PRBS_CASE(9) BBB_PRBS_CASE(11) BBB_PRBS_CASE(15)
-        BBB_PRBS_CASE(20) BBB_PRBS_CASE(23) BBB_PRBS_CASE(31)
-    }
-#undef BBB_PRBS_CASE
-    BBB_HIP(hipGetLastError());
-    return BBB_OK;
-}
-
-template <bool CHECK>
-static int launch_stream(int k, u64 init_state, u64 first_bit, u64 nbits, u64 *buf, u64 *nerr, hipStream_t st, int nt_stores = 0) {
+static int launch_stream(int pass, int k, u64 init_state, u64 first_bit, u64 nbits, u64 *buf, u64 *nerr, hipStream_t st) {
     const int ki = k_index(k);
     if (ki < 0) return fail(BBB_EINVAL, "k=" + std::to_string(k) + " invalid for PRBS");
     if (init_state == 0 || init_state >> k) return fail(BBB_EINVAL, "PRBS state must be in [1, 2^k)");
@@ -522,24 +401,21 @@
     if (first_bit + nbits < first_bit) return fail(BBB_EINVAL, "first_bit + nbits overflows");
     int rc = upload_pow_table(k);
     if (rc) return rc;
-    static const int lw_fill = env_knob("BBB_PRBS_FILL_LW", 0);
-    static const int lw_chk = env_knob("BBB_PRBS_CHECK_LW", 0);
-    const bool lw = CHECK ? lw_chk != 0 : lw_fill != 0;
-    static const int rev = env_knob("BBB_PRBS_CHECK_REV", 1);
-    if (CHECK && rev && !lw && prbs_wpl(true) == 1) return launch_check_rev(k, ki, init_state, first_bit, nbits, buf, nerr, st);
-    if (prbs_wpl(CHECK) == 1)
-        return lw ? launch_stream_w<CHECK, 1, true>(k, ki, init_state, first_bit, nbits, buf, nerr, st, nt_stores)
-                  : launch_stream_w<CHECK, 1, false>(k, ki, init_state, first_bit, nbits, buf, nerr, st, nt_stores);
-    return lw ? launch_stream_w<CHECK, 2, true>(k, ki, init_state, first_bit, nbits, buf, nerr, st, nt_stores)
-              : launch_stream_w<CHECK, 2, false>(k, ki, init_state, first_bit, nbits, buf, nerr, st, nt_stores);
+    int dev = 0, ncu = 256;
+    BBB_HIP(hipGetDevice(&dev));
+    BBB_HIP(hipDeviceGetAttribute(&ncu, hipDeviceAttributeMultiprocessorCount, dev));
+    const PrbsPartition p = prbs_partition(k, nbits, pass, ncu);
+    const int rev = env_knob("BBB_PRBS_CHECK_REV", 1);
+    return p.wpl == 1 ? launch_prbs<1>(pass, rev != 0, p, k, ki, init_state, first_bit, nbits, buf, nerr, st)
+                      : launch_prbs<2>(pass, rev != 0, p, k, ki, init_state, first_bit, nbits, buf, nerr, st);
 }
 
 int prbs_fill_launch(int k, uint64_t init_state, uint64_t first_bit, uint64_t nbits, uint64_t *dst, hipStream_t st, int nt_stores) {
-    return launch_stream<false>(k, init_state, first_bit, nbits, (u64 *)dst, nullptr, st, nt_stores);
+    return launch_stream(nt_stores ? kPrbsFillReadBack : kPrbsFill, k, init_state, first_bit, nbits, (u64 *)dst, nullptr, st);
 }
 int prbs_check_launch(int k, uint64_t init_state, uint64_t first_bit, uint64_t nbits, const uint64_t *src,
                       uint64_t *nerr_dev, hipStream_t st) {
-    return launch_stream<true>(k, init_state, first_bit, nbits, (u64 *)const_cast<uint64_t *>(src), (u64 *)nerr_dev, st);
+    return launch_stream(kPrbsCheck, k, init_state, first_bit, nbits, (u64 *)const_cast<uint64_t *>(src), (u64 *)nerr_dev, st);
 }
 
 __global__ void __launch_bounds__(256)
diff --git a/basebandboard_amd/csrc/prbs_partition.hpp b/basebandboard_amd/csrc/prbs_partition.hpp
--- /dev/null
+++ b/basebandboard_amd/csrc/prbs_partition.hpp
@@ -0,0 +1,46 @@
+#pragma once
+#include "bbb_common.hpp"
+
+namespace bbb {
+
+enum PrbsPass { kPrbsFill = 0, kPrbsCheck = 1, kPrbsFillReadBack = 2 };
+
+struct PrbsPartition {
+    int wpl;
+    unsigned lg_w;
+    uint64_t rows_per_wave;
+    uint64_t nblocks;
+};
+
+inline PrbsPartition prbs_partition(int k, uint64_t nbits, int pass, int ncu) {
+    const int want_fill = env_knob("BBB_PRBS_FILL_W", 256), wpl_fill = env_knob("BBB_PRBS_FILL_WPL", 1);
+    const int want_rb = env_knob("BBB_PRBS_FILL_RB_W", 256), wpl_rb = env_knob("BBB_PRBS_FILL_RB_WPL", 2);
+    const int want_chk = env_knob("BBB_PRBS_CHECK_W", 1024), wpl_chk = env_knob("BBB_PRBS_CHECK_WPL", 1);
+    const int contiguous = env_knob("BBB_PRBS_CONTIGUOUS", 0), per_cu = env_knob("BBB_PRBS_WAVES_PER_CU", 4);
+    PrbsPartition p;
+    p.wpl = (pass == kPrbsCheck ? wpl_chk : pass == kPrbsFillReadBack ? wpl_rb : wpl_fill) == 2 ? 2 : 1;
+    const uint64_t rw = 64ull * (uint64_t)p.wpl;
+    const uint64_t nwords = nbits / 64 + (nbits % 64 != 0);
+    const uint64_t rows = nwords / rw + (nwords % rw != 0);
+    if (contiguous) {
+        const uint64_t target = (uint64_t)ncu * (uint64_t)(per_cu > 0 ? per_cu : 4);
+        uint64_t rpw = (rows + target - 1) / target;
+        if (rpw < 8ull * (uint64_t)k) rpw = 8ull * (uint64_t)k;
+        p.lg_w = 0;
+        p.rows_per_wave = rpw;
+        p.nblocks = (rows + rpw - 1) / rpw;
+        return p;
+    }
+    uint64_t want = (uint64_t)(pass == kPrbsCheck ? want_chk : pass == kPrbsFillReadBack ? want_rb : want_fill);
+    const uint64_t resident = 8ull * (uint64_t)ncu;
+    if (want > resident) want = resident;
+    const uint64_t fit = rows / (2ull * (uint64_t)k);
+    if (want > fit) want = fit;
+    p.lg_w = 0;
+    while ((2ull << p.lg_w) <= want) p.lg_w++;
+    p.rows_per_wave = 0;
+    p.nblocks = rows < (1ull << p.lg_w) ? rows : (1ull << p.lg_w);
+    return p;
+}
+
+}
diff --git a/basebandboard_amd/prbs.py b/basebandboard_amd/prbs.py
--- a/basebandboard_amd/prbs.py
+++ b/basebandboard_amd/prbs.py
@@ -14,6 +14,16 @@
 def _check_k(k):
     if k not in TAPS.keys():
         raise ValueError("k={} invalid for PRBS".format(k))
+
+
+PASS_FILL, PASS_CHECK, PASS_FILL_READ_BACK = 0, 1, 2
+
+
+def partition_info(k, nbits, which=PASS_FILL, device=-1):
+    w, rw = C.c_uint32(), C.c_uint32()
+    _lib.check(_lib.lib().bbb_prbs_partition_info(int(k), int(nbits), int(which), int(device), C.byref(w), C.byref(rw)),
+               "bbb_prbs_partition_info")
+    return w.value, rw.value
 
 
 class PRBS:
diff --git a/experiments/prbs_sweep.py b/experiments/prbs_sweep.py
--- a/experiments/prbs_sweep.py
+++ b/experiments/prbs_sweep.py
@@ -1,28 +1,59 @@
-import os, subprocess, sys, json
-if len(sys.argv) > 1:
-    import torch, ctypes as C
-    sys.path.insert(0, os.path.dirname(os.path.dirname(os.path.abspath(__file__))))
-    import basebandboard_amd as bbb
-    bbb._lib.select_build("experiments")
-    nbits = 10_000_000_000
-    p = bbb.PRBS(31); det = bbb.PRBSErrorDetector(31)
-    buf = torch.empty((nbits + 63)//64, dtype=torch.int64, device="cuda")
-    p.generate(nbits, out=buf); n0 = det.count_errors(buf, nbits)
-    torch.cuda.synchronize()
-    e = [torch.cuda.Event(enable_timing=True) for _ in range(3)]
-    g = c = 0.0
-    for _ in range(5):
-        e[0].record(); p.generate(nbits, out=buf); e[1].record(); n = det.count_errors(buf, nbits); e[2].record()
-        torch.cuda.synchronize(); g += e[0].elapsed_time(e[1]); c += e[1].elapsed_time(e[2])
-    print(json.dumps({"cfg": sys.argv[1], "errors": n0, "gen_TBs": nbits/8*5/g/1e9, "chk_TBs": nbits/8*5/c/1e9}))
+import ctypes as C
+import itertools
+import json
+import os
+import sys
+
+sys.path.insert(0, os.path.dirname(os.path.dirname(os.path.abspath(__file__))))
+import torch
+from basebandboard_amd import _lib
+
+_lib.select_build("experiments")
+L = _lib.lib()
+rounds = int(sys.argv[1]) if len(sys.argv) > 1 else 3
+dev = torch.device("cuda", 0)
+sp = C.c_void_p(torch.cuda.current_stream(dev).cuda_stream)
+ev = lambda: torch.cuda.Event(enable_timing=True)
+nbits = 10_000_000_000
+pbuf = torch.empty((nbits + 63) // 64, dtype=torch.int64, device=dev)
+cnt = torch.zeros(1, dtype=torch.int64, device=dev)
+fill = lambda: _lib.check(L.bbb_prbs_fill(31, 1, 0, nbits, C.c_void_p(pbuf.data_ptr()), 0, sp), "fill")
+check = lambda: _lib.check(L.bbb_prbs_check_dev(31, 1, 0, nbits, C.c_void_p(pbuf.data_ptr()), C.c_void_p(cnt.data_ptr()), 0, sp), "check")
+fill_rb = lambda: _lib.check(L.bbb_prbs_fill_hint(31, 1, 0, nbits, C.c_void_p(pbuf.data_ptr()), 1, 0, sp), "fill_hint")
+
+
+def knobs(fill_w, fill_wpl, rb_w, rb_wpl, chk_w, chk_wpl):
+    return {"BBB_PRBS_FILL_W": fill_w, "BBB_PRBS_FILL_WPL": fill_wpl, "BBB_PRBS_FILL_RB_W": rb_w, "BBB_PRBS_FILL_RB_WPL": rb_wpl,
+            "BBB_PRBS_CHECK_W": chk_w, "BBB_PRBS_CHECK_WPL": chk_wpl}
+
+
+settings = [("contiguous", {"BBB_PRBS_CONTIGUOUS": 1})]
+if len(sys.argv) > 2:
+    for (fw, fl), (rw, rl), cw in itertools.product(((256, 1), (128, 1), (128, 2)), ((256, 2), (256, 1), (128, 2)), (1024, 2048)):
+        settings.append((f"fill W={fw} lanes={8 * fl}B  read-back fill W={rw} lanes={8 * rl}B  check W={cw} lanes=8B", knobs(fw, fl, rw, rl, cw, 1)))
 else:
-    def run(tag, **kv):
-        env = dict(os.environ, **{k: str(v) for k, v in kv.items()})
-        subprocess.run([sys.executable, __file__, tag + " " + " ".join(f"{k[9:]}={v}" for k, v in kv.items())], env=env)
-    for cap in (0, 4, 8):
-        for wpl in (1, 2):
-            for lw in (0, 1):
-                if wpl == 2 and lw == 0:
-                    continue
-                run("FILL ", BBB_PRBS_FILL_WPL=wpl, BBB_PRBS_FILL_LW=lw, BBB_PRBS_WAVES_PER_CU=cap)
-                run("CHECK", BBB_PRBS_CHECK_WPL=wpl, BBB_PRBS_CHECK_LW=lw, BBB_PRBS_WAVES_PER_CU=cap)
+    for fw, fl, cw, cl in itertools.product((256, 512, 1024), (1, 2), (1024, 2048), (1, 2)):
+        settings.append((f"fill W={fw} lanes={8 * fl}B  check W={cw} lanes={8 * cl}B", knobs(fw, fl, fw, fl, cw, cl)))
+
+reps = 3
+for r in range(rounds):
+    for name, envs in settings:
+        for k in [k for k in os.environ if k.startswith("BBB_PRBS")]:
+            del os.environ[k]
+        os.environ.update({k: str(v) for k, v in envs.items()})
+        fill_rb(); check()
+        torch.cuda.synchronize()
+        fh = ch = f = c = c2 = 0.0
+        for _ in range(reps):
+            e = [ev() for _ in range(3)]
+            e[0].record(); fill_rb(); e[1].record(); check(); e[2].record()
+            torch.cuda.synchronize()
+            fh += e[0].elapsed_time(e[1]) / reps; ch += e[1].elapsed_time(e[2]) / reps
+        for _ in range(reps):
+            e = [ev() for _ in range(4)]
+            e[0].record(); fill(); e[1].record(); check(); e[2].record(); check(); e[3].record()
+            torch.cuda.synchronize()
+            f += e[0].elapsed_time(e[1]) / reps; c += e[1].elapsed_time(e[2]) / reps; c2 += e[2].elapsed_time(e[3]) / reps
+        print(json.dumps({"round": r, "setting": name, "loopback_ms": round(fh + ch, 4), "hinted_fill_ms": round(fh, 4),
+                          "check_after_hinted_fill_ms": round(ch, 4), "fill_ms": round(f, 4), "check_after_fill_ms": round(c, 4),
+                          "check_clean_ms": round(c2, 4), "errors": int(cnt.item())}), flush=True)
diff --git a/include/bbb.h b/include/bbb.h
--- a/include/bbb.h
+++ b/include/bbb.h
@@ -74,6 +74,10 @@
                        const uint64_t *src_packed_dev, uint64_t *nerr_dev, int device,
                        void *hip_stream);
 int bbb_prbs_state_at(int k, uint64_t init_state, uint64_t nbits, uint64_t *state);
+#define BBB_PRBS_PASS_FILL 0
+#define BBB_PRBS_PASS_CHECK 1
+#define BBB_PRBS_PASS_FILL_READ_BACK 2
+int bbb_prbs_partition_info(int k, uint64_t nbits, int pass, int device, uint32_t *waves, uint32_t *row_words);
 
 int bbb_prbs_detector_run(int k, const uint8_t *bits_dev, uint64_t nstreams, uint64_t n,
                           uint8_t *err_dev, uint8_t *reload_dev, int device, void *hip_stream);
```

Result: no change. 957.4 (-1.0%).
